# Jerrypiglet/monosdf

Measured on AMD Instinct MI355X. Metric: rays/sec fwd+bwd, 1024 rays x 98 samples, 8x256 SDF MLP, higher is better.
Workload: dtype f32; 1 GPU; configs[1]: 1024 rays x 98 samples per GPU, ImplicitNetwork 8x256 + RenderingNetwork 289-256-256-3, error-bounded sampler, random-init weights (density beta 0.1), training step = fwd + loss + bwd + Adam, a different one of 8 ray batches every step; rays_per_gpu=1024, samples_per_ray=98, ray_batches=8, matrix_core=fp32

## Files before the change

include/monosdf_hip.h:

```cpp
#ifndef MONOSDF_HIP_H
#define MONOSDF_HIP_H

#include <stdint.h>
#include "monosdf_plan.h"

#ifdef __cplusplus
extern "C" {
#endif

#define MSDF_OK 0
#define MSDF_ERR_ARG 1
#define MSDF_ERR_LAUNCH 2
#define MSDF_ERR_UNSUPPORTED 3

#define MSDF_ABI_VERSION 8
int msdf_abi_version(void);

int msdf_hash_encode_forward(const float* inputs, const float* embeddings, const int* offsets, float* outputs,
                             uint32_t B, uint32_t D, uint32_t C, uint32_t L, float S, uint32_t H,
                             int calc_grad_inputs, float* dy_dx, void* stream);
int msdf_hash_encode_backward(const float* grad, const float* inputs, const float* embeddings, const int* offsets,
                              float* grad_embeddings, uint32_t B, uint32_t D, uint32_t C, uint32_t L, float S,
                              uint32_t H, int calc_grad_inputs, const float* dy_dx, float* grad_inputs,
                              void* stream);
int msdf_hash_encode_second_backward(const float* grad, const float* inputs, const float* embeddings,
                                     const int* offsets, uint32_t B, uint32_t D, uint32_t C, uint32_t L, float S,
                                     uint32_t H, int calc_grad_inputs, const float* dy_dx,
                                     const float* grad_grad_inputs, float* grad_grad, float* grad2_embeddings,
                                     void* stream);

int64_t msdf_hash_scatter_workspace_bytes(uint32_t B, uint32_t C, uint32_t L, uint64_t n_entries);
int msdf_hash_encode_backward_ws(const float* grad, const float* inputs, const float* embeddings, const int* offsets,
                                 float* grad_embeddings, uint32_t B, uint32_t D, uint32_t C, uint32_t L, float S,
                                 uint32_t H, int calc_grad_inputs, const float* dy_dx, float* grad_inputs,
                                 uint64_t n_entries, void* workspace, uint64_t workspace_bytes, void* stream);
int msdf_hash_encode_second_backward_ws(const float* grad, const float* inputs, const float* embeddings,
                                        const int* offsets, uint32_t B, uint32_t D, uint32_t C, uint32_t L, float S,
                                        uint32_t H, int calc_grad_inputs, const float* dy_dx,
                                        const float* grad_grad_inputs, float* grad_grad, float* grad2_embeddings,
                                        uint64_t n_entries, void* workspace, uint64_t workspace_bytes, void* stream);
int msdf_hash_encode_backward_fused(const float* grad_first, const float* grad_second, const float* inputs,
                                    const int* offsets, float* grad_embeddings, uint32_t B, uint32_t D, uint32_t C,
                                    uint32_t L, float S, uint32_t H, const float* grad_grad_inputs,
                                    uint64_t n_entries, void* workspace, uint64_t workspace_bytes, void* stream);
int msdf_hash_encode_backward_fused_out(const float* grad_first, const float* grad_second, const float* inputs,
                                        const int* offsets, float* grad_embeddings, uint32_t B, uint32_t D, uint32_t C,
                                        uint32_t L, float S, uint32_t H, const float* grad_grad_inputs,
                                        uint64_t n_entries, void* workspace, uint64_t workspace_bytes, void* stream);

int msdf_hash_node_forward(const float* x, double divide_factor, float* x01_out, const float* embeddings,
                           const int* offsets, float* feat, uint32_t pitch, uint32_t B, uint32_t C, uint32_t L,
                           float S, uint32_t H, float* dy_dx, void* stream);
int msdf_hash_node_input_gradient(const float* g, uint32_t pitch, const float* dy_dx, uint32_t B, uint32_t C,
                                  uint32_t L, float scale, float* inout, void* stream);
int msdf_hash_node_second_grad(const float* g_a, const float* g_b, uint32_t n_split, float scale, float* gg_out,
                               const float* dy_dx, float* grad_grad, uint32_t pitch, uint32_t B, uint32_t C,
                               uint32_t L, void* stream);
int msdf_hash_transpose(const float* src, float* dst, const float* src2, float* dst2, uint32_t L, uint32_t B,
                        uint32_t C, uint32_t pitch, int to_point_major, void* stream);
int msdf_hash_node_scatter(const float* grad_first, const float* grad_second, uint32_t pitch, const float* inputs,
                           const int* offsets, float* grad_embeddings, uint32_t B, uint32_t C, uint32_t L, float S,
                           uint32_t H, const float* grad_grad_inputs, uint64_t n_entries, void* workspace,
                           uint64_t workspace_bytes, void* stream);

int msdf_pack_weights(const msdf_plan_t* plan, const msdf_packrule_t* rules_dev, const int* maps_dev,
                      const float* flat_w, const float* flat_b, void* wpack, float* bpack, void* stream);

typedef struct {
  const float* v;
  const float* g;
  const float* b;
  int32_t rows, cols;
  int32_t w_off;
  int32_t b_off;
  int32_t row_off;
  int32_t has_g;
} msdf_wn_layer_t;
int msdf_weightnorm_forward(const msdf_wn_layer_t* layers_dev, const int* row_layer_dev, int total_rows,
                            float* flat_w, float* flat_b, float* norms, void* stream);
int msdf_weightnorm_backward(const msdf_wn_layer_t* layers_dev, const int* row_layer_dev, int total_rows,
                             const float* g_flat_w, const float* norms, float* dv_flat, float* dg_rows, void* stream);

int msdf_sdf_forward(const msdf_plan_t* plan, const void* wpack, const float* bpack, const float* x,
                     const float* aux, int P, float clamp_radius, float sphere_scale, float* sdf, void* stream);
int msdf_sdf_forward_if(const msdf_plan_t* plan, const void* wpack, const float* bpack, const float* x,
                        const float* aux, int P, float clamp_radius, float sphere_scale, float* sdf,
                        const uint32_t* run_flag, void* stream);
int msdf_sdf_forward_lm(const msdf_plan_t* plan, const void* wpack, const float* bpack, const float* x,
                        const float* aux, int aux_C, int aux_LC, int P, float clamp_radius, float sphere_scale,
                        float* sdf, const uint32_t* run_flag, void* stream);
int msdf_sdf_forward_save(const msdf_plan_t* plan, const void* wpack, const float* bpack, const float* x,
                          const float* aux, int aux_C, int aux_LC, int P, float clamp_radius, float sphere_scale,
                          float* sdf, const uint32_t* run_flag, float* H, int P_pad, const int32_t* col_slot,
                          int n_cols, int n_slots, uint32_t* h_saved, void* stream);

typedef struct {
  const void* wpack;
  const float* bpack;
  const float* x;
  const float* aux;
  int32_t P, P_pad;
  int32_t n_clamp;
  int32_t n_feat;
  float clamp_radius, sphere_scale;
  float* sdf;
  float* feat;
  float* nrm;
  float* r_aux;
  unsigned char* clamped;
  float* H;
  float* PM;
  float* IN0;
  int32_t save;
  int32_t aux_C;
  int32_t aux_LC;
  float aux_dx_scale;
  const float* dy_dx;
  const int32_t* row_map;
  const uint32_t* smp_flags;
  const uint32_t* h_saved;
  int32_t n_reuse;
  int32_t stage_pad;
  const float* h_stage;
  int32_t wg_first;
} msdf_fg_args_t;
int msdf_sdf_fwd_grad(const msdf_plan_t* plan, const msdf_fg_args_t* args, void* stream);

typedef struct {
  const void* wpack;
  const float* bpack;
  const float* x;
  int32_t P, P_pad;
  int32_t n_feat;
  int32_t n_split;
  const float* g_sdf;
  const float* g_feat;
  const float* g_nrm;
  const float* g_raux;
  const unsigned char* clamped;
  const float* H;
  const float* PM;
  float* QB;
  float* T;
  float* AB;
  float* GSDF;
  float* QLAST;
  float* g_aux;
  const float* g_sdf_b;
  const float* g_nrm_b;
  int32_t aux_C, aux_LC;
  const float* dy_dx;
  float* gg_out;
  float aux_dx_scale;
  int32_t pad_;
  const int32_t* row_map;
} msdf_bw_args_t;
int msdf_sdf_backward(const msdf_plan_t* plan, const msdf_bw_args_t* args, void* stream);

typedef struct {
  const void* wpack;
  const float* bpack;
  const float* x;
  const float* dirs;
  const float* nrm;
  const float* feat;
  const float* code;
  int32_t P, P_pad;
  int32_t spr;
  int32_t save;
  float* rgb;
  float* H;
  float* MISC;
} msdf_color_fwd_args_t;
int msdf_color_forward(const msdf_plan_t* plan, const msdf_color_fwd_args_t* args, void* stream);

typedef struct {
  const void* wpack;
  const float* bpack;
  const float* rgb;
  const float* g_rgb;
  int32_t P, P_pad;
  const float* H;
  float* AB;
  float* g_feat;
  float* g_misc;
  float* g_nrm;
} msdf_color_bwd_args_t;
int msdf_color_backward(const msdf_plan_t* plan, const msdf_color_bwd_args_t* args, void* stream);

int msdf_wgrad(const msdf_wgrad_item_t* items_dev, const int32_t* wg_map_dev, int n_wgs, float* partials,
               int P_pad, int precision , const float* base0, const float* base1 , void* stream);
int msdf_reduce(const msdf_reduce_rule_t* rules_dev, int n_rules, const int* maps_dev, const float* partials,
                float* dst, void* stream);

typedef struct {
  const float* z;
  const float* sdf;
  const float* rgb;
  const float* nrm;
  const float* beta;
  const float* depth_scale;
  int32_t N, S;
  int32_t white_bkgd;
  float bg0, bg1, bg2;
  float* weights;
  float* rgb_values;
  float* depth_values;
  float* normal_map;
  float* wsum;
  const float* pose;
  int32_t pose_stride;
  int32_t depth_scale_stride;
  float* depth_vals;
} msdf_composite_args_t;
int msdf_composite_forward(const msdf_composite_args_t* args, void* stream);

typedef struct {
  const float* z;
  const float* sdf;
  const float* rgb;
  const float* nrm;
  const float* beta;
  const float* depth_scale;
  const float* weights;
  const float* wsum;
  const float* depth_values;
  const float* g_rgb_values;
  const float* g_depth;
  const float* g_normal;
  const float* g_weights;
  int32_t N, S;
  int32_t white_bkgd;
  float bg0, bg1, bg2;
  float* g_sdf;
  float* g_rgb;
  float* g_nrm;
  float* g_beta_part;
  const float* pose;
  int32_t pose_stride;
  int32_t depth_scale_stride;
} msdf_composite_bwd_args_t;
int msdf_composite_backward(const msdf_composite_bwd_args_t* args, void* stream);

int msdf_beta_eff(const float* beta_raw, float beta_min, float* out, void* stream);
int msdf_beta_grad(const float* beta_raw, const float* g_part, int n, float* g_raw, void* stream);

typedef struct {
  const float* rgb;
  const float* nrm;
  const float* depth;
  const float* g1;
  const float* g2;
  int32_t N, M;
  float w_normal, w_depth, w_eik, w_smooth;
  float* g_rgb; float* g_nrm; float* g_depth; float* g_g1; float* g_g2;
  float* partial;
} msdf_probe_loss_args_t;
int msdf_probe_loss(const msdf_probe_loss_args_t* args, void* stream);

typedef struct {
  const float* rgb;
  const float* depth;
  const float* normal;
  const float* sdf;
  const float* grad_theta;
  const float* grad_nei;
  const float* rgb_gt;
  const float* depth_gt;
  const float* normal_gt;
  const float* mask_gt;
  int32_t N, S, E;
  int32_t gamma;
  int32_t scale_invariant;
  float w_eik, w_smooth, w_depth, w_nl1, w_ncos;
  float* mask;
  float* out;
  float* g_rgb; float* g_depth; float* g_normal; float* g_theta; float* g_nei;
} msdf_monosdf_loss_args_t;
int msdf_monosdf_loss(const msdf_monosdf_loss_args_t* args, void* stream);

typedef struct {
  const float* ray_o;
  const float* ray_d;
  int32_t N;
  int32_t M;
  int32_t m_max;
  int32_t n_eval, n_final, n_extra;
  int32_t round_idx, max_rounds;
  int32_t training;
  int32_t beta_iters;
  float near, far, bound;
  float eps, add_tiny;
  float lemma;
  const float* beta0;
  float* z;
  float* sdf;
  float* new_z;
  const float* new_sdf;
  int32_t* new_pos;
  float* pts;
  float* beta;
  uint32_t* flags;
  const float* jitter;
  const float* u_final;
  float* final_z;
  const int64_t* extra_idx;
  const int64_t* eik_idx;
  float* z_out;
  float* z_eik;
  float* pts_out;
  const float* eik_uniform;
  const float* nei_rand;
  float* far_out;
  int32_t* rounds_out;
  float* dbg_dstar;
  float* dbg_err0;
  float* dbg_cdf;
  const float* eik_u;
  int32_t eik_unit;
  int32_t pad_;
  int32_t* row_map;
  uint32_t* h_saved;
} msdf_sampler_args_t;
int msdf_sampler_init(const msdf_sampler_args_t* args, void* stream);
int msdf_sampler_beta(const msdf_sampler_args_t* args, void* stream);
int msdf_sampler_resample(const msdf_sampler_args_t* args, void* stream);
int msdf_sampler_finish(const msdf_sampler_args_t* args, void* stream);

int msdf_sampler_error_bound(const float* z, const float* sdf, const float* dstar, const float* beta,
                             int beta_stride, int N, int M, float* out, void* stream);

int msdf_laplace_density(const float* sdf, const float* beta, int beta_stride, int64_t n, int cols, float* out,
                         void* stream);
int msdf_laplace_density_backward(const float* sdf, const float* beta, int beta_stride, int64_t n, int cols,
                                  const float* g, float* g_sdf, float* g_beta_elem, void* stream);

int msdf_camera_rays(const float* uv, const float* pose, const float* intrinsics, int n, float* ray_dirs,
                     float* ray_dirs_cam, float* cam_loc, void* stream);

int msdf_pixel_rays(const int64_t* ray_idx, int n, const int32_t* frame_list, int n_frames, const float* pose_all,
                    const float* intrinsics_all, int width, int hw, float* ray_dirs, float* ray_dirs_cam,
                    float* cam_loc, float* ray_pose, int32_t* frame_pos, const float* const* gt_src,
                    float* const* gt_dst, const int32_t* gt_channels, int n_gt, void* stream);

int64_t msdf_mc_workspace_bytes(int nx, int ny, int nz);
int msdf_mc_count(const float* vol, int nx, int ny, int nz, float level, void* workspace, int64_t* totals,
                  void* stream);
int msdf_mc_emit(const float* vol, int nx, int ny, int nz, float level, float sx, float sy, float sz,
                 const void* workspace, float* verts, float* normals, int32_t* faces, void* stream);

int msdf_nn_split_count(int64_t n_ref, int64_t n_query, int n_splits);
int64_t msdf_nn_workspace_bytes(int64_t n_ref, int64_t n_query, int n_splits);
int msdf_nn_search(const float* ref, int64_t n_ref, const float* query, int64_t n_query, int n_splits,
                   void* workspace, float* dist, int32_t* idx, void* stream);
int msdf_voxel_keys(const float* points, int64_t n, const float* min_bound, float voxel_size, int64_t* keys,
                    void* stream);
int msdf_voxel_mean(const float* points, const int64_t* order, const int64_t* seg_start, int64_t n, int64_t m,
                    float* out, void* stream);

int msdf_raster_depth(const float* verts, int64_t n_verts, const int32_t* faces, int64_t n_faces, const float* w2c,
                      int n_views, float fx, float fy, float cx, float cy, int height, int width, float znear,
                      float zfar, float pixel_center, float* depth, void* stream);
int msdf_tsdf_integrate(const float* depth, const float* w2c, int n_views, float fx, float fy, float cx, float cy,
                        int height, int width, float ox, float oy, float oz, int i0, int j0, int k0, int nx, int ny,
                        int nz, float voxel_length, float sdf_trunc, float depth_trunc, int resume, float* tsdf,
                        float* weight, void* stream);
int msdf_tsdf_face_keep(const float* verts, int64_t n_verts, const int32_t* faces, int64_t n_faces,
                        const float* weight, int nx, int ny, int nz, uint8_t* keep, void* stream);
int msdf_cull_vertices(const float* verts, int64_t n_verts, const float* w2c, int n_views, float fx, float fy, float cx,
                       float cy, int height, int width, uint8_t* seen, void* stream);

int64_t msdf_dtu_dilate_workspace_bytes(int n_views, int height, int width);
int msdf_dtu_dilate(const uint8_t* masks, int n_views, int height, int width, int radius, void* workspace,
                    uint8_t* out, void* stream);
int msdf_dtu_mask_vertices(const float* verts, int64_t n_verts, const float* proj, int n_views,
                           const uint8_t* dilated, int height, int width, uint8_t* keep, void* stream);
int msdf_dtu_lattice_count(const float* verts, int64_t n_verts, const int32_t* faces, int64_t n_faces,
                           double density, int64_t* counts, void* stream);
int msdf_dtu_lattice_emit(const float* verts, int64_t n_verts, const int32_t* faces, int64_t n_faces, double density,
                          const int64_t* offsets, int64_t n_points, float* out, void* stream);
// ... 13 lines not shown
```

monosdf_amd/_lib.py:

```python
import ctypes as C
import os

_HERE = os.path.dirname(os.path.abspath(__file__))
LIB_PATH = os.environ.get('MONOSDF_HIP_LIB') or os.path.join(_HERE, 'libmonosdf_hip.so')

MAX_LAYERS = 10
MAX_TILES = 17


class Layer(C.Structure):
    _fields_ = [(n, C.c_int32) for n in
                ('kt', 'ot', 'wf_off', 'wb_off', 'bias_off', 'skip_tile', 'hpre', 'qpre', 'abpre',
                 'ktp', 'otp', 'pad_')]


class Plan(C.Structure):
    _fields_ = [(n, C.c_int32) for n in
                ('n_layers', 'e_tiles', 'aux_tiles', 'n_freqs', 'sdf_slot', 'feat_tiles', 'hsum',
                 'qsum', 'absum', 'wsdf_off', 'mode', 'out_act', 'precision', 'out_rows')] + [('layer', Layer * MAX_LAYERS)]


class PackRule(C.Structure):
    _fields_ = [('w_off', C.c_int32), ('b_off', C.c_int32), ('rows', C.c_int32), ('cols', C.c_int32),
                ('rowmap_off', C.c_int32), ('colmap_off', C.c_int32), ('scale', C.c_float),
                ('pad_', C.c_int32)]


class WgradItem(C.Structure):
    _fields_ = [('x', C.c_int64), ('y', C.c_int64), ('v', C.c_int64),
                ('part_off', C.c_int64), ('colsum_off', C.c_int64), ('vrow_off', C.c_int64),
                ('x_ld', C.c_int32), ('y_ld', C.c_int32), ('wx', C.c_int32), ('wy', C.c_int32),
                ('n_splits', C.c_int32), ('bufs', C.c_int32)]


class ReduceRule(C.Structure):
    _fields_ = [('part_off', C.c_int64), ('dst_off', C.c_int64), ('n_blocks', C.c_int32),
                ('wx', C.c_int32), ('wy', C.c_int32), ('rowmap_off', C.c_int32),
                ('colmap_off', C.c_int32), ('dst_ld', C.c_int32), ('fixed_row', C.c_int32),
                ('scale', C.c_float)]


_P = C.c_void_p


class FgArgs(C.Structure):
    _fields_ = [('wpack', _P), ('bpack', _P), ('x', _P), ('aux', _P),
                ('P', C.c_int32), ('P_pad', C.c_int32), ('n_clamp', C.c_int32), ('n_feat', C.c_int32),
                ('clamp_radius', C.c_float), ('sphere_scale', C.c_float),
                ('sdf', _P), ('feat', _P), ('nrm', _P), ('r_aux', _P), ('clamped', _P),
                ('H', _P), ('PM', _P), ('IN0', _P), ('save', C.c_int32), ('aux_C', C.c_int32), ('aux_LC', C.c_int32),
                ('aux_dx_scale', C.c_float), ('dy_dx', _P),
                ('row_map', _P), ('smp_flags', _P), ('h_saved', _P), ('n_reuse', C.c_int32), ('stage_pad', C.c_int32), ('h_stage', _P),
                ('wg_first', C.c_int32)]


class BwArgs(C.Structure):
    _fields_ = [('wpack', _P), ('bpack', _P), ('x', _P),
                ('P', C.c_int32), ('P_pad', C.c_int32), ('n_feat', C.c_int32), ('n_split', C.c_int32),
                ('g_sdf', _P), ('g_feat', _P), ('g_nrm', _P), ('g_raux', _P), ('clamped', _P),
                ('H', _P), ('PM', _P), ('QB', _P), ('T', _P), ('AB', _P), ('GSDF', _P), ('QLAST', _P),
                ('g_aux', _P), ('g_sdf_b', _P), ('g_nrm_b', _P), ('aux_C', C.c_int32), ('aux_LC', C.c_int32),
                ('dy_dx', _P), ('gg_out', _P), ('aux_dx_scale', C.c_float), ('pad_', C.c_int32),
                ('row_map', _P)]


class ColorFwdArgs(C.Structure):
    _fields_ = [('wpack', _P), ('bpack', _P), ('x', _P), ('dirs', _P), ('nrm', _P), ('feat', _P),
                ('code', _P), ('P', C.c_int32), ('P_pad', C.c_int32), ('spr', C.c_int32),
                ('save', C.c_int32), ('rgb', _P), ('H', _P), ('MISC', _P)]


class ColorBwdArgs(C.Structure):
    _fields_ = [('wpack', _P), ('bpack', _P), ('rgb', _P), ('g_rgb', _P),
                ('P', C.c_int32), ('P_pad', C.c_int32), ('H', _P), ('AB', _P), ('g_feat', _P),
                ('g_misc', _P), ('g_nrm', _P)]


class CompositeArgs(C.Structure):
    _fields_ = [('z', _P), ('sdf', _P), ('rgb', _P), ('nrm', _P), ('beta', _P), ('depth_scale', _P),
                ('N', C.c_int32), ('S', C.c_int32), ('white_bkgd', C.c_int32),
                ('bg0', C.c_float), ('bg1', C.c_float), ('bg2', C.c_float),
                ('weights', _P), ('rgb_values', _P), ('depth_values', _P), ('normal_map', _P),
                ('wsum', _P), ('pose', _P), ('pose_stride', C.c_int32), ('depth_scale_stride', C.c_int32),
                ('depth_vals', _P)]


class CompositeBwdArgs(C.Structure):
    _fields_ = [('z', _P), ('sdf', _P), ('rgb', _P), ('nrm', _P), ('beta', _P), ('depth_scale', _P),
                ('weights', _P), ('wsum', _P), ('depth_values', _P), ('g_rgb_values', _P),
                ('g_depth', _P), ('g_normal', _P), ('g_weights', _P),
                ('N', C.c_int32), ('S', C.c_int32), ('white_bkgd', C.c_int32),
                ('bg0', C.c_float), ('bg1', C.c_float), ('bg2', C.c_float),
                ('g_sdf', _P), ('g_rgb', _P), ('g_nrm', _P), ('g_beta_part', _P),
                ('pose', _P), ('pose_stride', C.c_int32), ('depth_scale_stride', C.c_int32)]


class WnLayer(C.Structure):
    _fields_ = [('v', _P), ('g', _P), ('b', _P), ('rows', C.c_int32), ('cols', C.c_int32),
                ('w_off', C.c_int32), ('b_off', C.c_int32), ('row_off', C.c_int32), ('has_g', C.c_int32)]


class ProbeLossArgs(C.Structure):
    _fields_ = [('rgb', _P), ('nrm', _P), ('depth', _P), ('g1', _P), ('g2', _P), ('N', C.c_int32), ('M', C.c_int32),
                ('w_normal', C.c_float), ('w_depth', C.c_float), ('w_eik', C.c_float), ('w_smooth', C.c_float),
                ('g_rgb', _P), ('g_nrm', _P), ('g_depth', _P), ('g_g1', _P), ('g_g2', _P), ('partial', _P)]


class MonoSdfLossArgs(C.Structure):
    _fields_ = [(n, _P) for n in ('rgb', 'depth', 'normal', 'sdf', 'grad_theta', 'grad_nei', 'rgb_gt', 'depth_gt',
                                  'normal_gt', 'mask_gt')] + \
               [(n, C.c_int32) for n in ('N', 'S', 'E', 'gamma', 'scale_invariant')] + \
               [(n, C.c_float) for n in ('w_eik', 'w_smooth', 'w_depth', 'w_nl1', 'w_ncos')] + \
               [(n, _P) for n in ('mask', 'out', 'g_rgb', 'g_depth', 'g_normal', 'g_theta', 'g_nei')]


class SamplerArgs(C.Structure):
    _fields_ = [('ray_o', _P), ('ray_d', _P), ('N', C.c_int32), ('M', C.c_int32), ('m_max', C.c_int32),
                ('n_eval', C.c_int32), ('n_final', C.c_int32), ('n_extra', C.c_int32),
                ('round_idx', C.c_int32), ('max_rounds', C.c_int32), ('training', C.c_int32),
                ('beta_iters', C.c_int32), ('near', C.c_float), ('far', C.c_float), ('bound', C.c_float),
                ('eps', C.c_float), ('add_tiny', C.c_float), ('lemma', C.c_float),
                ('beta0', _P), ('z', _P), ('sdf', _P), ('new_z', _P), ('new_sdf', _P), ('new_pos', _P),
                ('pts', _P), ('beta', _P), ('flags', _P), ('jitter', _P), ('u_final', _P), ('final_z', _P),
                ('extra_idx', _P), ('eik_idx', _P), ('z_out', _P), ('z_eik', _P), ('pts_out', _P),
                ('eik_uniform', _P), ('nei_rand', _P), ('far_out', _P), ('rounds_out', _P),
                ('dbg_dstar', _P), ('dbg_err0', _P), ('dbg_cdf', _P), ('eik_u', _P), ('eik_unit', C.c_int32),
                ('pad_', C.c_int32), ('row_map', _P), ('h_saved', _P)]


_ERR = {1: 'invalid argument', 2: 'kernel launch failed', 3: 'unsupported configuration'}

_SIGNATURES = {
    'msdf_abi_version': [],
    'msdf_hash_encode_forward': [_P, _P, _P, _P, C.c_uint32, C.c_uint32, C.c_uint32, C.c_uint32,
                                 C.c_float, C.c_uint32, C.c_int, _P, _P],
    'msdf_hash_encode_backward': [_P, _P, _P, _P, _P, C.c_uint32, C.c_uint32, C.c_uint32, C.c_uint32,
                                  C.c_float, C.c_uint32, C.c_int, _P, _P, _P],
    'msdf_hash_encode_second_backward': [_P, _P, _P, _P, C.c_uint32, C.c_uint32, C.c_uint32,
                                         C.c_uint32, C.c_float, C.c_uint32, C.c_int, _P, _P, _P, _P, _P],
    'msdf_hash_scatter_workspace_bytes': [C.c_uint32, C.c_uint32, C.c_uint32, C.c_uint64],
    'msdf_hash_encode_backward_ws': [_P, _P, _P, _P, _P, C.c_uint32, C.c_uint32, C.c_uint32, C.c_uint32,
                                     C.c_float, C.c_uint32, C.c_int, _P, _P, C.c_uint64, _P, C.c_uint64, _P],
    'msdf_hash_encode_second_backward_ws': [_P, _P, _P, _P, C.c_uint32, C.c_uint32, C.c_uint32, C.c_uint32,
                                            C.c_float, C.c_uint32, C.c_int, _P, _P, _P, _P, C.c_uint64, _P,
                                            C.c_uint64, _P],
    'msdf_hash_encode_backward_fused': [_P, _P, _P, _P, _P, C.c_uint32, C.c_uint32, C.c_uint32, C.c_uint32,
                                        C.c_float, C.c_uint32, _P, C.c_uint64, _P, C.c_uint64, _P],
    'msdf_hash_encode_backward_fused_out': [_P, _P, _P, _P, _P, C.c_uint32, C.c_uint32, C.c_uint32, C.c_uint32,
                                            C.c_float, C.c_uint32, _P, C.c_uint64, _P, C.c_uint64, _P],
    'msdf_hash_node_forward': [_P, C.c_double, _P, _P, _P, _P, C.c_uint32, C.c_uint32, C.c_uint32, C.c_uint32,
                               C.c_float, C.c_uint32, _P, _P],
    'msdf_hash_node_input_gradient': [_P, C.c_uint32, _P, C.c_uint32, C.c_uint32, C.c_uint32, C.c_float, _P, _P],
    'msdf_hash_node_second_grad': [_P, _P, C.c_uint32, C.c_float, _P, _P, _P, C.c_uint32, C.c_uint32, C.c_uint32,
                                   C.c_uint32, _P],
    'msdf_hash_transpose': [_P, _P, _P, _P, C.c_uint32, C.c_uint32, C.c_uint32, C.c_uint32, C.c_int, _P],
    'msdf_hash_node_scatter': [_P, _P, C.c_uint32, _P, _P, _P, C.c_uint32, C.c_uint32, C.c_uint32, C.c_float,
                               C.c_uint32, _P, C.c_uint64, _P, C.c_uint64, _P],
    'msdf_weightnorm_forward': [_P, _P, C.c_int, _P, _P, _P, _P],
    'msdf_weightnorm_backward': [_P, _P, C.c_int, _P, _P, _P, _P, _P],
    'msdf_pack_weights': [C.POINTER(Plan), _P, _P, _P, _P, _P, _P, _P],
    'msdf_sdf_forward': [C.POINTER(Plan), _P, _P, _P, _P, C.c_int, C.c_float, C.c_float, _P, _P],
    'msdf_sdf_forward_if': [C.POINTER(Plan), _P, _P, _P, _P, C.c_int, C.c_float, C.c_float, _P, _P, _P],
    'msdf_sdf_forward_lm': [C.POINTER(Plan), _P, _P, _P, _P, C.c_int, C.c_int, C.c_int, C.c_float, C.c_float, _P, _P, _P],
    'msdf_sdf_forward_save': [C.POINTER(Plan), _P, _P, _P, _P, C.c_int, C.c_int, C.c_int, C.c_float, C.c_float, _P, _P,
                              _P, C.c_int, _P, C.c_int, C.c_int, _P, _P],
    'msdf_sdf_fwd_grad': [C.POINTER(Plan), C.POINTER(FgArgs), _P],
    'msdf_sdf_backward': [C.POINTER(Plan), C.POINTER(BwArgs), _P],
    'msdf_color_forward': [C.POINTER(Plan), C.POINTER(ColorFwdArgs), _P],
    'msdf_color_backward': [C.POINTER(Plan), C.POINTER(ColorBwdArgs), _P],
    'msdf_wgrad': [_P, _P, C.c_int, _P, C.c_int, C.c_int, _P, _P, _P],
    'msdf_camera_rays': [_P, _P, _P, C.c_int, _P, _P, _P, _P],
    'msdf_pixel_rays': [_P, C.c_int, _P, C.c_int, _P, _P, C.c_int, C.c_int, _P, _P, _P, _P, _P, _P, _P, _P, C.c_int, _P],
    'msdf_monosdf_loss': [C.POINTER(MonoSdfLossArgs), _P],
    'msdf_reduce': [_P, C.c_int, _P, _P, _P, _P],
    'msdf_composite_forward': [C.POINTER(CompositeArgs), _P],
    'msdf_composite_backward': [C.POINTER(CompositeBwdArgs), _P],
    'msdf_beta_eff': [_P, C.c_float, _P, _P],
    'msdf_beta_grad': [_P, _P, C.c_int, _P, _P],
    'msdf_probe_loss': [C.POINTER(ProbeLossArgs), _P],
    'msdf_sampler_init': [C.POINTER(SamplerArgs), _P],
    'msdf_sampler_beta': [C.POINTER(SamplerArgs), _P],
    'msdf_sampler_resample': [C.POINTER(SamplerArgs), _P],
    'msdf_sampler_finish': [C.POINTER(SamplerArgs), _P],
    'msdf_sampler_error_bound': [_P, _P, _P, _P, C.c_int, C.c_int, C.c_int, _P, _P],
    'msdf_laplace_density': [_P, _P, C.c_int, C.c_int64, C.c_int, _P, _P],
    'msdf_laplace_density_backward': [_P, _P, C.c_int, C.c_int64, C.c_int, _P, _P, _P, _P],
    'msdf_mc_workspace_bytes': [C.c_int, C.c_int, C.c_int],
    'msdf_mc_count': [_P, C.c_int, C.c_int, C.c_int, C.c_float, _P, _P, _P],
    'msdf_mc_emit': [_P, C.c_int, C.c_int, C.c_int, C.c_float, C.c_float, C.c_float, C.c_float, _P, _P, _P, _P, _P],
    'msdf_nn_split_count': [C.c_int64, C.c_int64, C.c_int],
    'msdf_nn_workspace_bytes': [C.c_int64, C.c_int64, C.c_int],
    'msdf_nn_search': [_P, C.c_int64, _P, C.c_int64, C.c_int, _P, _P, _P, _P],
    'msdf_voxel_keys': [_P, C.c_int64, _P, C.c_float, _P, _P],
    'msdf_voxel_mean': [_P, _P, _P, C.c_int64, C.c_int64, _P, _P],
    'msdf_raster_depth': [_P, C.c_int64, _P, C.c_int64, _P, C.c_int, C.c_float, C.c_float, C.c_float, C.c_float,
                          C.c_int, C.c_int, C.c_float, C.c_float, C.c_float, _P, _P],
    'msdf_tsdf_integrate': [_P, _P, C.c_int, C.c_float, C.c_float, C.c_float, C.c_float, C.c_int, C.c_int,
                            C.c_float, C.c_float, C.c_float, C.c_int, C.c_int, C.c_int, C.c_int, C.c_int, C.c_int,
                            C.c_float, C.c_float, C.c_float, C.c_int, _P, _P, _P],
    'msdf_tsdf_face_keep': [_P, C.c_int64, _P, C.c_int64, _P, C.c_int, C.c_int, C.c_int, _P, _P],
    'msdf_cull_vertices': [_P, C.c_int64, _P, C.c_int, C.c_float, C.c_float, C.c_float, C.c_float, C.c_int, C.c_int,
                           _P, _P],
    'msdf_dtu_dilate_workspace_bytes': [C.c_int, C.c_int, C.c_int],
    'msdf_dtu_dilate': [_P, C.c_int, C.c_int, C.c_int, C.c_int, _P, _P, _P],
    'msdf_dtu_mask_vertices': [_P, C.c_int64, _P, C.c_int, _P, C.c_int, C.c_int, _P, _P],
    'msdf_dtu_lattice_count': [_P, C.c_int64, _P, C.c_int64, C.c_double, _P, _P],
    'msdf_dtu_lattice_emit': [_P, C.c_int64, _P, C.c_int64, C.c_double, _P, C.c_int64, _P, _P],
    'msdf_dtu_thin_workspace_bytes': [C.c_int64],
    'msdf_dtu_thin_keys': [_P, C.c_int64, C.c_double, C.c_double, C.c_double, C.c_double, _P, _P],
    'msdf_dtu_thin_prepare': [_P, _P, _P, _P, C.c_int64, _P, _P],
    'msdf_dtu_thin_round': [_P, C.c_int64, C.c_double, _P, _P],
    'msdf_dtu_thin_finish': [_P, _P, C.c_int64, _P, _P],
}

ABI_VERSION = 8

_lib = None


def load():
    global _lib
    if _lib is not None:
        return _lib
    if not os.path.exists(LIB_PATH):
        raise RuntimeError(
            'monosdf_amd: %s not found -- build it with `python __graft_entry__.py` or '
            '`make -C monosdf_amd/csrc` (there is no non-HIP fallback)' % LIB_PATH)
    lib = C.CDLL(LIB_PATH)
    for name, argtypes in _SIGNATURES.items():
        fn = getattr(lib, name)
        fn.argtypes = argtypes
        fn.restype = C.c_int64 if name.endswith('_bytes') else C.c_int
    if lib.msdf_abi_version() != ABI_VERSION:
        raise RuntimeError('monosdf_amd: ABI version mismatch, rebuild the library')
    _lib = lib
    return lib
# ... 36 lines not shown
```

monosdf_amd/csrc/composite.hip:

```cpp
#include "common.h"

#define CMP_MAX_PER_LANE 4

__device__ __forceinline__ float wave_incl_scan(float v) {
  const int lane = lane_id();
#pragma unroll
  for (int d = 1; d < 64; d <<= 1) {
    const float o = __shfl_up(v, d, 64);
    if (lane >= d) v += o;
  }
  return v;
}

__device__ __forceinline__ float wave_excl_scan(const float v, float& total) {
  float prev = __shfl_up(v, 1, 64);
  if (lane_id() == 0) prev = 0.f;
  const float ex = wave_incl_scan(prev);
  total = __shfl(ex, 63, 64) + __shfl(v, 63, 64);
  return ex;
}

__device__ __forceinline__ float wave_sum(float v) {
#pragma unroll
  for (int d = 32; d >= 1; d >>= 1) v += __shfl_xor(v, d, 64);
// ... 38 lines not shown
      w = alpha * trans;
      a.weights[(size_t)ray * S + i] = w;
      if (a.depth_vals != nullptr) a.depth_vals[(size_t)ray * S + i] = z[i] * dscale;
      const float* c = a.rgb + ((size_t)ray * S + i) * 3;
      const float* n = a.nrm + ((size_t)ray * S + i) * 3;
      r0 += w * c[0]; r1 += w * c[1]; r2 += w * c[2];
      wz += w * z[i];
      ws += w;
      const float nn = sqrtf(n[0] * n[0] + n[1] * n[1] + n[2] * n[2]) + 1e-6f;
      m0 += w * (n[0] / nn); m1 += w * (n[1] / nn); m2 += w * (n[2] / nn);
    }
    carry += chunk_total;
  }
  r0 = wave_sum(r0); r1 = wave_sum(r1); r2 = wave_sum(r2);
  wz = wave_sum(wz); ws = wave_sum(ws);
  m0 = wave_sum(m0); m1 = wave_sum(m1); m2 = wave_sum(m2);
  if (lane == 0) {
    if (a.white_bkgd) {
      r0 += (1.f - ws) * a.bg0; r1 += (1.f - ws) * a.bg1; r2 += (1.f - ws) * a.bg2;
    }
    a.rgb_values[(size_t)ray * 3 + 0] = r0;
    a.rgb_values[(size_t)ray * 3 + 1] = r1;
    a.rgb_values[(size_t)ray * 3 + 2] = r2;
    a.depth_values[ray] = dscale * (wz / (ws + 1e-8f));
    if (a.pose != nullptr) {
      const float* R = a.pose + (size_t)ray * a.pose_stride;
      const float c0 = R[0] * m0 + R[4] * m1 + R[8] * m2;
      const float c1 = R[1] * m0 + R[5] * m1 + R[9] * m2;
      const float c2 = R[2] * m0 + R[6] * m1 + R[10] * m2;
      m0 = c0; m1 = c1; m2 = c2;
    }
    a.normal_map[(size_t)ray * 3 + 0] = m0;
    a.normal_map[(size_t)ray * 3 + 1] = m1;
    a.normal_map[(size_t)ray * 3 + 2] = m2;
    a.wsum[ray] = ws;
  }
}

typedef msdf_composite_bwd_args_t CompositeBwdArgs;

__device__ __forceinline__ float wave_excl_suffix(const float v, float& total) {
  const int lane = lane_id();
  float s = __shfl_down(v, 1, 64);
  if (lane == 63) s = 0.f;
#pragma unroll
  for (int d = 1; d < 64; d <<= 1) {
    const float o = __shfl_down(s, d, 64);
    if (lane + d < 64) s += o;
  }
  total = __shfl(s, 0, 64) + __shfl(v, 0, 64);
  return s;
}

__global__ void __launch_bounds__(256)
msdf_composite_backward_k(const CompositeBwdArgs a) {
  const int ray = blockIdx.x * 4 + (threadIdx.x >> 6);
  if (ray >= a.N) return;
  const int lane = lane_id();
  const int S = a.S;
  const float beta = a.beta[0];
  const float* z = a.z + (size_t)ray * S;
  const float* sd = a.sdf + (size_t)ray * S;
  const float ws = a.wsum[ray];
  const float ds = a.depth_scale[(size_t)ray * (a.depth_scale_stride > 0 ? a.depth_scale_stride : 1)];
  float gR0 = 0.f, gR1 = 0.f, gR2 = 0.f, gD = 0.f, gM0 = 0.f, gM1 = 0.f, gM2 = 0.f;
  if (a.g_rgb_values) {
    gR0 = a.g_rgb_values[(size_t)ray * 3 + 0];
    gR1 = a.g_rgb_values[(size_t)ray * 3 + 1];
    gR2 = a.g_rgb_values[(size_t)ray * 3 + 2];
  }
  if (a.g_depth) gD = a.g_depth[ray];
  if (a.g_normal) {
    gM0 = a.g_normal[(size_t)ray * 3 + 0];
    gM1 = a.g_normal[(size_t)ray * 3 + 1];
    gM2 = a.g_normal[(size_t)ray * 3 + 2];
    if (a.pose != nullptr) {
      const float* R = a.pose + (size_t)ray * a.pose_stride;
      const float w0 = R[0] * gM0 + R[1] * gM1 + R[2] * gM2;
      const float w1 = R[4] * gM0 + R[5] * gM1 + R[6] * gM2;
      const float w2 = R[8] * gM0 + R[9] * gM1 + R[10] * gM2;
      gM0 = w0; gM1 = w1; gM2 = w2;
    }
  }
  const float inv = 1.0f / (ws + 1e-8f);
  const float wz_over = (ds != 0.f) ? a.depth_values[ray] / ds : 0.f;
  float bg_term = 0.f;
  if (a.white_bkgd) bg_term = -(gR0 * a.bg0 + gR1 * a.bg1 + gR2 * a.bg2);

  float fe_[CMP_MAX_PER_LANE], tr_[CMP_MAX_PER_LANE], wb_[CMP_MAX_PER_LANE], dist_[CMP_MAX_PER_LANE];
  float carry = 0.f;
  const int nchunk = (S + 63) >> 6;
#pragma unroll
  for (int ch = 0; ch < CMP_MAX_PER_LANE; ++ch) {
    fe_[ch] = tr_[ch] = wb_[ch] = dist_[ch] = 0.f;
    if (ch < nchunk) {
      const int i = ch * 64 + lane;
      const bool ok = i < S;
      float fe = 0.f, dist = 0.f;
      if (ok) {
        const float zi = z[i];
        dist = (i + 1 < S) ? (z[i + 1] - zi) : 1e10f;
        fe = dist * laplace_density(sd[i], beta);
      }
      float chunk_total;
      const float ex = wave_excl_scan(fe, chunk_total);
      if (ok) {
        const float excl = carry + ex;
        const float trans = expf(-excl);
        const float w = a.weights[(size_t)ray * S + i];
        const float* c = a.rgb + ((size_t)ray * S + i) * 3;
        const float* n = a.nrm + ((size_t)ray * S + i) * 3;
        const float nl = sqrtf(n[0] * n[0] + n[1] * n[1] + n[2] * n[2]);
        const float nn = nl + 1e-6f;
        const float gdot = gM0 * n[0] + gM1 * n[1] + gM2 * n[2];
        float wbar = gR0 * c[0] + gR1 * c[1] + gR2 * c[2] + gD * ds * (z[i] - wz_over) * inv + gdot / nn + bg_term;
        if (a.g_weights) wbar += a.g_weights[(size_t)ray * S + i];
        float* gc = a.g_rgb + ((size_t)ray * S + i) * 3;
        gc[0] = w * gR0; gc[1] = w * gR1; gc[2] = w * gR2;
        float* gn = a.g_nrm + ((size_t)ray * S + i) * 3;
        const float k = (nl > 0.f) ? gdot / (nl * nn * nn) : 0.f;
        gn[0] = w * (gM0 / nn - n[0] * k);
        gn[1] = w * (gM1 / nn - n[1] * k);
        gn[2] = w * (gM2 / nn - n[2] * k);
        fe_[ch] = fe; tr_[ch] = trans; wb_[ch] = wbar; dist_[ch] = dist;
      }
      carry += chunk_total;
    }
  }
  float after = 0.f;
  float gbeta = 0.f;
#pragma unroll
  for (int ch = CMP_MAX_PER_LANE - 1; ch >= 0; --ch) {
    if (ch < nchunk) {
      const int i = ch * 64 + lane;
      const bool ok = i < S;
      const float fe = fe_[ch], trans = tr_[ch], wbar = wb_[ch];
      const float efe = expf(-fe);
      const float alpha = 1.0f - efe;
      const float cbar = ok ? (-wbar * alpha * trans) : 0.f;
      float total;
      const float suffix = wave_excl_suffix(cbar, total);
      if (ok) {
        const float ebar = wbar * trans * efe + suffix + after;
        const float sbar = ebar * dist_[ch];
        const float s = sd[i];
        const float ex = expf(-fabsf(s) / beta);
        a.g_sdf[(size_t)ray * S + i] = sbar * (-0.5f / (beta * beta)) * ex;
        const float sigma = laplace_density(s, beta);
        gbeta += sbar * (-sigma / beta + 0.5f * s * ex / (beta * beta * beta));
      }
      after += total;
    }
  }
  gbeta = wave_sum(gbeta);
  if (lane == 0) a.g_beta_part[ray] = gbeta;
}

__global__ void msdf_beta_eff_k(const float* __restrict__ raw, const float beta_min, float* __restrict__ out) {
  if (threadIdx.x == 0) out[0] = fabsf(raw[0]) + beta_min;
}
__global__ void __launch_bounds__(64)
msdf_beta_grad_k(const float* __restrict__ raw, const float* __restrict__ part, const int n, float* __restrict__ g_raw) {
  float s = 0.f;
  for (int i = threadIdx.x; i < n; i += 64) s += part[i];
  s = wave_sum(s);
  const float r = raw[0];
  if (threadIdx.x == 0) g_raw[0] = ((r > 0.f) ? 1.f : (r < 0.f) ? -1.f : 0.f) * s;
}
extern "C" int msdf_beta_eff(const float* beta_raw, float beta_min, float* out, void* stream) {
  if (beta_raw == nullptr || out == nullptr) return MSDF_ERR_ARG;
  msdf_beta_eff_k<<<1, 64, 0, (hipStream_t)stream>>>(beta_raw, beta_min, out);
  return msdf_check_launch();
}
extern "C" int msdf_beta_grad(const float* beta_raw, const float* g_part, int n, float* g_raw, void* stream) {
  if (beta_raw == nullptr || g_raw == nullptr || n < 0 || (n > 0 && g_part == nullptr)) return MSDF_ERR_ARG;
  msdf_beta_grad_k<<<1, 64, 0, (hipStream_t)stream>>>(beta_raw, g_part, n, g_raw);
  return msdf_check_launch();
}

extern "C" int msdf_composite_forward(const msdf_composite_args_t* a, void* stream) {
  if (a == nullptr || a->N < 0 || a->S < 1 || a->S > 64 * CMP_MAX_PER_LANE) return MSDF_ERR_ARG;
  if (a->N == 0) return MSDF_OK;
  msdf_composite_forward_k<<<(a->N + 3) / 4, 256, 0, (hipStream_t)stream>>>(*a);
  return msdf_check_launch();
}

extern "C" int msdf_composite_backward(const msdf_composite_bwd_args_t* a, void* stream) {
  if (a == nullptr || a->N < 0 || a->S < 1 || a->S > 64 * CMP_MAX_PER_LANE) return MSDF_ERR_ARG;
  if (a->N == 0) return MSDF_OK;
  msdf_composite_backward_k<<<(a->N + 3) / 4, 256, 0, (hipStream_t)stream>>>(*a);
  return msdf_check_launch();
}
```

monosdf_amd/csrc/sampler.hip:

```cpp
#include "common.h"

#define SMP_WAVES 4

__device__ __forceinline__ float smp_scan_incl(float v) {
  const int lane = lane_id();
#pragma unroll
  for (int d = 1; d < 64; d <<= 1) {
    const float o = __shfl_up(v, d, 64);
    if (lane >= d) v += o;
  }
  return v;
}
__device__ __forceinline__ float smp_sum(float v) {
#pragma unroll
  for (int d = 32; d >= 1; d >>= 1) v += __shfl_xor(v, d, 64);
  return v;
}
__device__ __forceinline__ float smp_max(float v) {
#pragma unroll
  for (int d = 32; d >= 1; d >>= 1) v = fmaxf(v, __shfl_xor(v, d, 64));
  return v;
}
__device__ __forceinline__ float smp_density(const float s, const float beta) {
  const float e = expm1f(-fabsf(s) / beta);
  const float sg = (s > 0.f) ? 1.f : (s < 0.f) ? -1.f : 0.f;
  return (1.0f / beta) * (0.5f + 0.5f * sg * e);
}
__device__ __forceinline__ float smp_linspace01(const int j, const int n) {
  const float step = 1.0f / (float)(n - 1);
  return (j < n / 2) ? step * (float)j : 1.0f - step * (float)(n - 1 - j);
}

typedef msdf_sampler_args_t SmpArgs;

__global__ void __launch_bounds__(64 * SMP_WAVES) smp_init_k(const SmpArgs a) {
  const int ray = blockIdx.x * SMP_WAVES + (threadIdx.x >> 6);
  if (ray >= a.N) return;
  const int lane = lane_id();
  if (ray == 0 && a.flags != nullptr)
    for (int i = lane; i < 2 * a.max_rounds; i += 64) a.flags[i] = 0u;
  if (ray == 0 && lane == 0 && a.h_saved != nullptr) a.h_saved[0] = 0u;
  const int n = a.n_eval;
  const float o0 = a.ray_o[ray * 3 + 0], o1 = a.ray_o[ray * 3 + 1], o2 = a.ray_o[ray * 3 + 2];
  const float d0 = a.ray_d[ray * 3 + 0], d1 = a.ray_d[ray * 3 + 1], d2 = a.ray_d[ray * 3 + 2];
  const float ta0 = (-a.bound - o0) / (d0 + 1e-15f), tb0 = (a.bound - o0) / (d0 + 1e-15f);
  const float ta1 = (-a.bound - o1) / (d1 + 1e-15f), tb1 = (a.bound - o1) / (d1 + 1e-15f);
  const float ta2 = (-a.bound - o2) / (d2 + 1e-15f), tb2 = (a.bound - o2) / (d2 + 1e-15f);
  float near_c = fmaxf(fmaxf(fminf(ta0, tb0), fminf(ta1, tb1)), fminf(ta2, tb2));
  float far_c = fminf(fminf(fmaxf(ta0, tb0), fmaxf(ta1, tb1)), fmaxf(ta2, tb2));
  if (far_c < near_c) far_c = 1e9f;
  const float far = (a.bound > 0.f) ? fminf(far_c, a.far) : a.far;
  const float near = a.near;
  float sumsq = 0.f;
  float* zrow = a.z + (size_t)ray * a.m_max;
  auto zu = [&](int k) { const float t = smp_linspace01(k, n); return near * (1.f - t) + far * t; };
  auto zfin = [&](int k) {
    float z = zu(k);
    if (a.jitter != nullptr) {
      const float zl = (k > 0) ? 0.5f * (zu(k) + zu(k - 1)) : zu(0);
      const float zh = (k + 1 < n) ? 0.5f * (zu(k + 1) + zu(k)) : zu(n - 1);
      z = zl + (zh - zl) * a.jitter[(size_t)ray * n + k];
    }
    return z;
  };
  for (int j = lane; j < n; j += 64) {
    const float z = zfin(j);
    zrow[j] = z;
    a.new_z[(size_t)ray * n + j] = z;
    a.new_pos[(size_t)ray * n + j] = j;
    float* p = a.pts + ((size_t)ray * n + j) * 3;
    p[0] = o0 + z * d0; p[1] = o1 + z * d1; p[2] = o2 + z * d2;
    if (j + 1 < n) {
      const float dz = zfin(j + 1) - z;
      sumsq += dz * dz;
    }
  }
  sumsq = smp_sum(sumsq);
  if (lane == 0) {
    a.beta[ray] = sqrtf(a.lemma * sumsq);
    if (a.far_out != nullptr) a.far_out[ray] = far;
  }
}

struct SmpLds {
  float* z; float* sdf; float* dist; float* dstar; float* tmp; float* snew;
};
__device__ __forceinline__ SmpLds smp_lds(float* base, const int m_max, const int n_eval) {
  const int w = threadIdx.x >> 6;
  const int per = 5 * (m_max + 1) + n_eval;
  float* p = base + (size_t)w * per;
  SmpLds l;
  l.z = p; l.sdf = p + (m_max + 1); l.dist = p + 2 * (m_max + 1); l.dstar = p + 3 * (m_max + 1);
  l.tmp = p + 4 * (m_max + 1); l.snew = p + 5 * (m_max + 1);
  return l;
}
__device__ __forceinline__ void smp_sync() {
  __builtin_amdgcn_fence(__ATOMIC_RELEASE, "workgroup");
  __builtin_amdgcn_wave_barrier();
  __builtin_amdgcn_fence(__ATOMIC_ACQUIRE, "workgroup");
}

__device__ __forceinline__ bool smp_round_active(const SmpArgs& a) {
  return a.round_idx == 0 || a.flags[2 * (a.round_idx - 1) + 1] != 0u;
}

__device__ __forceinline__ void smp_load_ray(const SmpArgs& a, const SmpLds& l, const int ray, const bool scatter) {
  const int lane = lane_id();
  const int M = a.M;
  const float* zrow = a.z + (size_t)ray * a.m_max;
  float* srow = a.sdf + (size_t)ray * a.m_max;
  for (int i = lane; i < M; i += 64) { l.z[i] = zrow[i]; l.sdf[i] = srow[i]; }
  smp_sync();
  if (scatter) {
    for (int j = lane; j < a.n_eval; j += 64)
      l.sdf[a.new_pos[(size_t)ray * a.n_eval + j]] = a.new_sdf[(size_t)ray * a.n_eval + j];
    smp_sync();
    for (int i = lane; i < M; i += 64) srow[i] = l.sdf[i];
  }
  for (int i = lane; i + 1 < M; i += 64) {
    const float aa = l.z[i + 1] - l.z[i];
    const float b = fabsf(l.sdf[i]), c = fabsf(l.sdf[i + 1]);
    const bool first = aa * aa + b * b <= c * c;
    const bool second = aa * aa + c * c <= b * b;
    float ds = 0.f;
    if (first) ds = b;
    if (second) ds = c;
    if (!first && !second && (b + c - aa > 0.f)) {
      const float s = (aa + b + c) / 2.0f;
      const float area = s * (s - aa) * (s - b) * (s - c);
      ds = (2.0f * sqrtf(area)) / aa;
    }
    const float s0 = l.sdf[i], s1 = l.sdf[i + 1];
    const float sg0 = (s0 > 0.f) ? 1.f : (s0 < 0.f) ? -1.f : 0.f;
    const float sg1 = (s1 > 0.f) ? 1.f : (s1 < 0.f) ? -1.f : 0.f;
    l.dist[i] = aa;
    const float dsv = (sg0 * sg1 == 1.f) ? ds : 0.f;
    l.dstar[i] = dsv;
    if (scatter && a.dbg_dstar != nullptr) a.dbg_dstar[(size_t)ray * a.m_max + i] = dsv;
  }
  smp_sync();
}

__device__ __forceinline__ float smp_error_bound(const SmpLds& l, const int M, const float beta) {
  const int lane = lane_id();
  float carry_fe = 0.f, carry_err = 0.f, best = -1e30f;
  const float inv4b2 = 1.0f / (4.0f * beta * beta);
  for (int base = 0; base < M - 1; base += 64) {
    const int i = base + lane;
    const bool ok = i < M - 1;
    float fe = 0.f, er = 0.f;
    if (ok) {
      const float d = l.dist[i];
      fe = d * smp_density(l.sdf[i], beta);
      er = expf(-l.dstar[i] / beta) * (d * d) * inv4b2;
    }
    const float fe_incl = smp_scan_incl(fe);
    const float er_incl = smp_scan_incl(er);
    if (ok) {
      const float integral = carry_fe + fe_incl - fe;
      const float errint = carry_err + er_incl;
      const float bound = (fminf(expf(errint), 1.0e6f) - 1.0f) * expf(-integral);
      best = fmaxf(best, bound);
    }
    carry_fe += __shfl(fe_incl, 63, 64);
    carry_err += __shfl(er_incl, 63, 64);
  }
  return smp_max(best);
}

__global__ void __launch_bounds__(64 * SMP_WAVES) smp_beta_k(const SmpArgs a) {
  extern __shared__ float smp_lds_mem[];
  const int ray = blockIdx.x * SMP_WAVES + (threadIdx.x >> 6);
  if (ray >= a.N || !smp_round_active(a)) return;
  const SmpLds l = smp_lds(smp_lds_mem, a.m_max, a.n_eval);
  smp_load_ray(a, l, ray, true);
  const float beta0 = a.beta0[0];
  float beta = a.beta[ray];
  const float e0 = smp_error_bound(l, a.M, beta0);
  if (a.dbg_err0 != nullptr && lane_id() == 0) a.dbg_err0[ray] = e0;
  if (e0 <= a.eps) beta = beta0;
  float lo = beta0, hi = beta;
  const int iters = (e0 <= a.eps) ? 0 : a.beta_iters;
  for (int it = 0; it < iters; ++it) {
    const float mid = (lo + hi) / 2.0f;
    const float e = smp_error_bound(l, a.M, mid);
    if (e <= a.eps) hi = mid;
    if (e > a.eps) lo = mid;
  }
  if (lane_id() == 0) {
    a.beta[ray] = hi;
    atomicMax(a.flags + 2 * a.round_idx, __float_as_uint(hi));
  }
}

__global__ void __launch_bounds__(64 * SMP_WAVES) smp_resample_k(const SmpArgs a) {
  extern __shared__ float smp_lds_mem[];
  const int ray = blockIdx.x * SMP_WAVES + (threadIdx.x >> 6);
  if (ray >= a.N || !smp_round_active(a)) return;
  const int lane = lane_id();
  const int M = a.M;
  const SmpLds l = smp_lds(smp_lds_mem, a.m_max, a.n_eval);
  const float beta0 = a.beta0[0];
  const float maxbeta = __uint_as_float(a.flags[2 * a.round_idx]);
  const bool unconverged = maxbeta > beta0;
  const bool more = unconverged && (a.round_idx + 1 < a.max_rounds);
  if (ray == 0 && lane == 0) a.flags[2 * a.round_idx + 1] = more ? 1u : 0u;
  smp_load_ray(a, l, ray, false);
  const float beta = a.beta[ray];
  const float inv4b2 = 1.0f / (4.0f * beta * beta);

  float carry_fe = 0.f, carry_err = 0.f, psum = 0.f;
  for (int base = 0; base < M; base += 64) {
    const int i = base + lane;
    const bool ok = i < M;
    float fe = 0.f, er = 0.f;
    if (ok) {
      const float d = (i + 1 < M) ? l.dist[i] : 1e10f;
      fe = d * smp_density(l.sdf[i], beta);
      if (more && i + 1 < M) er = expf(-l.dstar[i] / beta) * (l.dist[i] * l.dist[i]) * inv4b2;
    }
    float fprev = __shfl_up(fe, 1, 64);
    if (lane == 0) fprev = 0.f;
    const float fe_excl = smp_scan_incl(fprev);
    const float fe_incl = fe_excl + fe;
    const float er_incl = smp_scan_incl(er);
    if (ok && i + 1 < M) {
      const float trans = expf(-(carry_fe + fe_excl));
      float p;
      if (more) p = (fminf(expf(carry_err + er_incl), 1.0e6f) - 1.0f) * trans + a.add_tiny;
      else p = (1.0f - expf(-fe)) * trans + 1e-5f;
      l.tmp[i] = p;
      psum += p;
    }
    carry_fe += __shfl(fe_incl, 63, 64);
    carry_err += __shfl(er_incl, 63, 64);
  }
  psum = smp_sum(psum);
  smp_sync();
  float carry = 0.f;
  for (int base = 0; base < M - 1; base += 64) {
    const int i = base + lane;
    const float p = (i < M - 1) ? l.tmp[i] / psum : 0.f;
    const float incl = smp_scan_incl(p);
    if (i < M - 1) l.dstar[i + 1] = carry + incl;
    carry += __shfl(incl, 63, 64);
  }
  if (lane == 0) l.dstar[0] = 0.f;
  smp_sync();
  const float* cdf = l.dstar;
  if (a.dbg_cdf != nullptr)
    for (int i = lane; i < M; i += 64) a.dbg_cdf[(size_t)ray * a.m_max + i] = cdf[i];

  const int n_new = more ? a.n_eval : a.n_final;
  for (int j = lane; j < n_new; j += 64) {
    float u;
    if (more || !a.training || a.u_final == nullptr) u = smp_linspace01(j, n_new);
    else u = a.u_final[(size_t)ray * a.n_final + j];
    int lo = 0, hi = M;
    while (lo < hi) {
      const int mid = (lo + hi) >> 1;
      if (cdf[mid] <= u) lo = mid + 1; else hi = mid;
    }
    const int below = max(lo - 1, 0), above = min(lo, M - 1);
    float denom = cdf[above] - cdf[below];
    if (denom < 1e-5f) denom = 1.0f;
    const float t = (u - cdf[below]) / denom;
    const float s = l.z[below] + t * (l.z[above] - l.z[below]);
    l.snew[j] = s;
  }
  smp_sync();

  if (!more) {
    for (int j = lane; j < n_new; j += 64) a.final_z[(size_t)ray * a.n_final + j] = l.snew[j];
    return;
  }
  const float o0 = a.ray_o[ray * 3 + 0], o1 = a.ray_o[ray * 3 + 1], o2 = a.ray_o[ray * 3 + 2];
  const float d0 = a.ray_d[ray * 3 + 0], d1 = a.ray_d[ray * 3 + 1], d2 = a.ray_d[ray * 3 + 2];
  float* zrow = a.z + (size_t)ray * a.m_max;
  float* srow = a.sdf + (size_t)ray * a.m_max;
  for (int i = lane; i < M; i += 64) {
    const float zi = l.z[i];
    int cnt = 0;
    for (int k = 0; k < n_new; ++k) cnt += (l.snew[k] < zi) ? 1 : 0;
    zrow[i + cnt] = zi;
    srow[i + cnt] = l.sdf[i];
  }
  for (int j = lane; j < n_new; j += 64) {
    const float sj = l.snew[j];
    int cnt = 0;
    for (int i = 0; i < M; ++i) cnt += (l.z[i] <= sj) ? 1 : 0;
    for (int k = 0; k < n_new; ++k) cnt += (l.snew[k] < sj || (l.snew[k] == sj && k < j)) ? 1 : 0;
    zrow[cnt] = sj;
    a.new_z[(size_t)ray * a.n_eval + j] = sj;
    a.new_pos[(size_t)ray * a.n_eval + j] = cnt;
    float* p = a.pts + ((size_t)ray * a.n_eval + j) * 3;
    p[0] = o0 + sj * d0; p[1] = o1 + sj * d1; p[2] = o2 + sj * d2;
  }
}

__global__ void __launch_bounds__(64 * SMP_WAVES) smp_finish_k(const SmpArgs a) {
  extern __shared__ float smp_lds_mem[];
  const int ray = blockIdx.x * SMP_WAVES + (threadIdx.x >> 6);
  if (ray >= a.N) return;
  const int lane = lane_id();
  const int S = a.n_final + a.n_extra + 2;
  float* v = smp_lds_mem + (size_t)(threadIdx.x >> 6) * 2 * S;
  float* sorted = v + S;
  const float* zrow = a.z + (size_t)ray * a.m_max;
  int rounds = 1;
  while (rounds < a.max_rounds && a.flags[2 * (rounds - 1) + 1] != 0u) ++rounds;
  const int64_t* extra = a.extra_idx + (size_t)(rounds - 1) * a.n_extra;
  if (a.rounds_out != nullptr && ray == 0 && lane == 0) a.rounds_out[0] = rounds;
  for (int j = lane; j < S; j += 64) {
    float x;
    if (j < a.n_final) x = a.final_z[(size_t)ray * a.n_final + j];
    else if (j == a.n_final) x = a.near;
    else if (j == a.n_final + 1) x = a.far;
    else x = zrow[min((int)extra[j - a.n_final - 2], rounds * a.n_eval - 1)];
    if (x != x) x = INFINITY;
    v[j] = x;
  }
  smp_sync();
  const float o0 = a.ray_o[ray * 3 + 0], o1 = a.ray_o[ray * 3 + 1], o2 = a.ray_o[ray * 3 + 2];
  const float d0 = a.ray_d[ray * 3 + 0], d1 = a.ray_d[ray * 3 + 1], d2 = a.ray_d[ray * 3 + 2];
  for (int j = lane; j < S; j += 64) {
    const float x = v[j];
    int r = 0, rn = 0;
    for (int k = 0; k < S; ++k) {
      const int before = (v[k] < x || (v[k] == x && k < j)) ? 1 : 0;
      r += before;
      rn += (k < a.n_final + 2) ? before : 0;
    }
    sorted[r] = x;
    a.z_out[(size_t)ray * S + r] = x;
    if (a.row_map != nullptr) {
      const int e = j - a.n_final - 2;
      const int er = (e >= 0) ? ray * a.n_extra + e : a.N * a.n_extra + ray * (S - a.n_extra) + rn;
      a.row_map[er] = ray * S + r;
    }
    if (a.pts_out != nullptr) {
      float* p = a.pts_out + ((size_t)ray * S + r) * 3;
      p[0] = o0 + x * d0; p[1] = o1 + x * d1; p[2] = o2 + x * d2;
    }
  }
  smp_sync();
  if (lane == 0) {
    const int idx = (a.eik_idx != nullptr) ? (int)a.eik_idx[ray]
                    : (a.eik_u != nullptr) ? min(S - 1, (int)(a.eik_u[ray] * (float)S)) : 0;
    const float ze = sorted[idx];
    if (a.z_eik != nullptr) a.z_eik[ray] = ze;
    if (a.pts_out != nullptr && a.eik_uniform != nullptr) {
      float* e = a.pts_out + (size_t)a.N * S * 3;
      if (a.row_map != nullptr)
        for (int i = 0; i < 4; ++i) a.row_map[a.N * S + i * a.N + ray] = a.N * S + i * a.N + ray;
      const float od[3] = {o0 + ze * d0, o1 + ze * d1, o2 + ze * d2};
#pragma unroll
      for (int c = 0; c < 3; ++c) {
        float u = a.eik_uniform[(size_t)ray * 3 + c];
        if (a.eik_unit) u = (2.0f * u - 1.0f) * a.bound;
        e[((size_t)ray) * 3 + c] = u;
        e[((size_t)a.N + ray) * 3 + c] = od[c];
        e[((size_t)2 * a.N + ray) * 3 + c] = u + (a.nei_rand[(size_t)ray * 3 + c] - 0.5f) * 0.01f;
        e[((size_t)3 * a.N + ray) * 3 + c] = od[c] + (a.nei_rand[((size_t)a.N + ray) * 3 + c] - 0.5f) * 0.01f;
      }
    }
  }
}

__global__ void __launch_bounds__(64 * SMP_WAVES) smp_error_bound_k(const float* __restrict__ z,
                                                                     const float* __restrict__ sdf,
                                                                     const float* __restrict__ dstar,
                                                                     const float* __restrict__ beta, const int beta_stride,
                                                                     const int N, const int M, float* __restrict__ out) {
  extern __shared__ float smp_lds_mem[];
  const int ray = blockIdx.x * SMP_WAVES + (threadIdx.x >> 6);
  if (ray >= N) return;
  const int lane = lane_id();
  const SmpLds l = smp_lds(smp_lds_mem, M, 0);
  for (int i = lane; i < M; i += 64) { l.z[i] = z[(size_t)ray * M + i]; l.sdf[i] = sdf[(size_t)ray * M + i]; }
  smp_sync();
  for (int i = lane; i + 1 < M; i += 64) {
    l.dist[i] = l.z[i + 1] - l.z[i];
    l.dstar[i] = dstar[(size_t)ray * (M - 1) + i];
  }
  smp_sync();
  const float e = smp_error_bound(l, M, beta[(size_t)ray * beta_stride]);
  if (lane == 0) out[ray] = e;
}

__global__ void __launch_bounds__(256) laplace_density_k(const float* __restrict__ sdf, const float* __restrict__ beta,
                                                         const int beta_stride, const int64_t n, const int cols,
                                                         float* __restrict__ out) {
  for (int64_t i = (int64_t)blockIdx.x * 256 + threadIdx.x; i < n; i += (int64_t)gridDim.x * 256)
    out[i] = smp_density(sdf[i], beta[(i / cols) * beta_stride]);
}
__global__ void __launch_bounds__(256) laplace_density_bwd_k(const float* __restrict__ sdf, const float* __restrict__ beta,
                                                             const int beta_stride, const int64_t n, const int cols,
                                                             const float* __restrict__ g, float* __restrict__ g_sdf,
                                                             float* __restrict__ g_beta_elem) {
  for (int64_t i = (int64_t)blockIdx.x * 256 + threadIdx.x; i < n; i += (int64_t)gridDim.x * 256) {
    const float s = sdf[i], b = beta[(i / cols) * beta_stride], gi = g[i];
    const float a = fabsf(s);
    const float ex = expf(-a / b);
    const float sg = (s > 0.f) ? 1.f : (s < 0.f) ? -1.f : 0.f;
    g_sdf[i] = gi * (1.0f / b) * 0.5f * sg * ex * (-sg / b);
    const float em1 = expm1f(-a / b);
    g_beta_elem[i] = gi * (-(1.0f / (b * b)) * (0.5f + 0.5f * sg * em1) + (1.0f / b) * 0.5f * sg * ex * (a / (b * b)));
  }
}

static int smp_check(const msdf_sampler_args_t* a) {
  if (a == nullptr || a->N < 0 || a->n_eval < 2 || a->m_max < a->n_eval) return MSDF_ERR_ARG;
  return MSDF_OK;
}
static size_t smp_lds_bytes(const msdf_sampler_args_t* a) {
  return (size_t)SMP_WAVES * (5 * (a->m_max + 1) + a->n_eval) * sizeof(float);
}
template <typename K>
static int smp_launch(K kernel, const msdf_sampler_args_t* a, size_t lds, void* stream) {
  if (a->N == 0) return MSDF_OK;
  if (lds > 160 * 1024) return MSDF_ERR_UNSUPPORTED;
  if (lds > 48 * 1024 &&
      hipFuncSetAttribute((const void*)kernel, hipFuncAttributeMaxDynamicSharedMemorySize, (int)lds) != hipSuccess)
    return MSDF_ERR_LAUNCH;
  kernel<<<(a->N + SMP_WAVES - 1) / SMP_WAVES, 64 * SMP_WAVES, lds, (hipStream_t)stream>>>(*a);
  return msdf_check_launch();
}

extern "C" int msdf_sampler_init(const msdf_sampler_args_t* a, void* stream) {
  if (smp_check(a)) return MSDF_ERR_ARG;
  return smp_launch(smp_init_k, a, 0, stream);
}
static int smp_round_check(const msdf_sampler_args_t* a) {
  return a->flags == nullptr || a->round_idx < 0 || a->round_idx >= a->max_rounds || a->M > a->m_max || a->M < 2;
}
extern "C" int msdf_sampler_beta(const msdf_sampler_args_t* a, void* stream) {
  if (smp_check(a) || smp_round_check(a)) return MSDF_ERR_ARG;
  return smp_launch(smp_beta_k, a, smp_lds_bytes(a), stream);
}
extern "C" int msdf_sampler_resample(const msdf_sampler_args_t* a, void* stream) {
  if (smp_check(a) || smp_round_check(a) || a->n_final > a->n_eval) return MSDF_ERR_ARG;
  return smp_launch(smp_resample_k, a, smp_lds_bytes(a), stream);
}
extern "C" int msdf_sampler_finish(const msdf_sampler_args_t* a, void* stream) {
  if (smp_check(a) || a->flags == nullptr || (a->extra_idx == nullptr && a->n_extra > 0) ||
      a->m_max < a->n_eval * a->max_rounds)
    return MSDF_ERR_ARG;
  const size_t lds = (size_t)SMP_WAVES * 2 * (a->n_final + a->n_extra + 2) * sizeof(float);
  return smp_launch(smp_finish_k, a, lds, stream);
}

extern "C" int msdf_sampler_error_bound(const float* z, const float* sdf, const float* dstar, const float* beta,
                                        int beta_stride, int N, int M, float* out, void* stream) {
  if (N < 0 || M < 2 || (beta_stride != 0 && beta_stride != 1)) return MSDF_ERR_ARG;
  if (N == 0) return MSDF_OK;
  const size_t lds = (size_t)SMP_WAVES * 5 * (M + 1) * sizeof(float);
  if (lds > 160 * 1024) return MSDF_ERR_UNSUPPORTED;
  if (lds > 48 * 1024 && hipFuncSetAttribute((const void*)smp_error_bound_k,
                                             hipFuncAttributeMaxDynamicSharedMemorySize, (int)lds) != hipSuccess)
    return MSDF_ERR_LAUNCH;
  smp_error_bound_k<<<(N + SMP_WAVES - 1) / SMP_WAVES, 64 * SMP_WAVES, lds, (hipStream_t)stream>>>(
      z, sdf, dstar, beta, beta_stride, N, M, out);
  return msdf_check_launch();
}

static int dens_grid(int64_t n) { return (int)((n + 255) / 256 < 2048 ? (n + 255) / 256 : 2048); }
extern "C" int msdf_laplace_density(const float* sdf, const float* beta, int beta_stride, int64_t n, int cols,
                                    float* out, void* stream) {
  if (n < 0 || cols < 1 || (beta_stride != 0 && beta_stride != 1)) return MSDF_ERR_ARG;
  if (n == 0) return MSDF_OK;
  laplace_density_k<<<dens_grid(n), 256, 0, (hipStream_t)stream>>>(sdf, beta, beta_stride, n, cols, out);
  return msdf_check_launch();
}
extern "C" int msdf_laplace_density_backward(const float* sdf, const float* beta, int beta_stride, int64_t n, int cols,
                                             const float* g, float* g_sdf, float* g_beta_elem, void* stream) {
  if (n < 0 || cols < 1 || (beta_stride != 0 && beta_stride != 1)) return MSDF_ERR_ARG;
  if (n == 0) return MSDF_OK;
  laplace_density_bwd_k<<<dens_grid(n), 256, 0, (hipStream_t)stream>>>(sdf, beta, beta_stride, n, cols, g, g_sdf,
                                                                     g_beta_elem);
  return msdf_check_launch();
}
```

monosdf_amd/csrc/sdf_kernels.h:

```cpp
#pragma once
#include "mlp_core.h"

struct PointCtx {
  int pt;
  int ptc;
  bool valid;
  int q;
  float x0, x1, x2;
};

template <class Core>
__device__ __forceinline__ int eval_wg(const int wg_first = 0) {
  int w = (int)blockIdx.x;
  if constexpr (Core::ROW_MAP) {
    if (wg_first > 0) {
      w += wg_first;
      if (w >= (int)gridDim.x) w -= (int)gridDim.x;
    }
  }
  return w;
}

template <class Core>
__device__ __forceinline__ PointCtx load_point(const float* __restrict__ x, const int P,
// ... 402 lines not shown
  if (nl >= 2) {
    const msdf_layer_t L = plan.layer[nl - 2];
    const float* Hl = REUSE ? a.h_stage + srow(L) : a.H + row(L);
    float* Pl = a.PM + row(L);
    const int otl = L.ot - 1;
    v4f hh[MT];
#pragma unroll
    for (int t = 0; t < MT; ++t) hh[t] = *(const v4f*)(Hl + 16 * (t < otl ? t : otl));
#pragma unroll
    for (int t = 0; t < MT; ++t) {
      if (t == 0 || t < L.ot) {
        if constexpr (REUSE) *(v4f*)(a.H + row(L) + 16 * t) = hh[t];
        scale_by_sigmoid(hh[t], acc[t]);
        if (a.save) *(v4f*)(Pl + 16 * t) = acc[t];
      }
    }
  }
  for (int l = nl - 2; l >= 0; --l) {
    const msdf_layer_t L = plan.layer[l];
#pragma unroll
    for (int t = 0; t < MT; ++t) in[t] = (t < L.ot) ? acc[t] : V4ZERO;
    zero_tiles(acc);
    const msdf_layer_t Lp = plan.layer[l > 0 ? l - 1 : 0];
    Core::gemm(L.otp, acc, in, L.kt, (const wvec*)a.wpack + L.wb_off, lds,
               GradSweepHooks<REUSE>(REUSE ? a.h_stage + srow(Lp) : a.H + row(Lp), a.H + row(Lp), a.PM + row(Lp),
                                     l > 0 ? Lp.ot : 0, a.save != 0));
    if (l == 0) take_input_grad(0);
    else if (L.skip_tile >= 0) take_input_grad(L.skip_tile);
  }
  if (Core::AUX_LEVEL_MAJOR && a.dy_dx != nullptr && plan.aux_tiles > 0) {
    float m0, m1, m2;
    aux_jacobian_transpose(a.dy_dx, av, plan.aux_tiles, r_aux, c.ptc, c.q, m0, m1, m2);
    n0 = __fadd_rn(n0, __fmul_rn(sum_over_quarters(m0), a.aux_dx_scale));
    n1 = __fadd_rn(n1, __fmul_rn(sum_over_quarters(m1), a.aux_dx_scale));
    n2 = __fadd_rn(n2, __fmul_rn(sum_over_quarters(m2), a.aux_dx_scale));
  }
  bool is_clamped = false;
  if (a.clamp_radius > 0.f && c.pt < a.n_clamp) {
    const float nx = sqrtf(c.x0 * c.x0 + c.x1 * c.x1 + c.x2 * c.x2);
    const float sph = a.sphere_scale * (a.clamp_radius - nx);
    if (sph < sdf) {
      is_clamped = true;
      sdf = sph;
      const float inv = -a.sphere_scale / nx;
      n0 = c.x0 * inv; n1 = c.x1 * inv; n2 = c.x2 * inv;
    }
  }
  if (c.valid) {
    if (c.q == 0) {
      a.sdf[c.pt] = sdf;
      a.nrm[(size_t)c.pt * 3 + 0] = n0;
      a.nrm[(size_t)c.pt * 3 + 1] = n1;
      a.nrm[(size_t)c.pt * 3 + 2] = n2;
      a.clamped[c.pt] = is_clamped ? 1 : 0;
    }
    if (a.r_aux != nullptr) {
#pragma unroll
      for (int t = 0; t < 2; ++t)
        if (t < plan.aux_tiles) {
          v4f v = r_aux[t];
          if (is_clamped) v = V4ZERO;
          aux_store_tile<Core::AUX_LEVEL_MAJOR>(a.r_aux, av, plan.aux_tiles, t, c.pt, c.q, v);
        }
    }
  }
}

typedef msdf_bw_args_t BwArgs;

template <bool LM>
__device__ __forceinline__ void load_rbar(v4f (&rbar)[5], const msdf_plan_t& plan, const BwArgs& a,
                                          const PointCtx& c, const bool live, const float gn0, const float gn1,
                                          const float gn2) {
  pe_jacobian(rbar, c.x0, c.x1, c.x2, plan.n_freqs, gn0, gn1, gn2);
  rbar[3] = rbar[4] = V4ZERO;
  if (LM && a.dy_dx != nullptr && live) {
    const AuxView av = {a.aux_C, a.aux_LC, a.P};
    const float g0 = __fmul_rn(gn0, a.aux_dx_scale), g1 = __fmul_rn(gn1, a.aux_dx_scale), g2 = __fmul_rn(gn2, a.aux_dx_scale);
#pragma unroll
    for (int t = 0; t < 2; ++t)
      if (t < plan.aux_tiles) rbar[3 + t] = aux_jacobian_tile(a.dy_dx, av, t, c.pt, c.q, g0, g1, g2);
  } else if (a.g_raux != nullptr && live) {
    const AuxView av = {a.aux_C, a.aux_LC, a.P};
#pragma unroll
    for (int t = 0; t < 2; ++t)
      if (t < plan.aux_tiles) rbar[3 + t] = aux_load_tile<LM>(a.g_raux, av, plan.aux_tiles, t, c.pt, c.q);
  }
}

template <class Core>
__device__ __forceinline__ void sdf_backward_body(const msdf_plan_t& plan, const BwArgs& a, void* lds) {
  typedef typename Core::wvec wvec;
  const PointCtx c = load_point<Core>(a.x, a.P, a.row_map);
  const int nl = plan.n_layers;
  const size_t Pp = (size_t)a.P_pad;
  const bool live = c.valid && !(a.clamped != nullptr && a.clamped[c.ptc]);
  float gs = 0.f, gn0 = 0.f, gn1 = 0.f, gn2 = 0.f;
  if (live) {
    const bool first = c.pt < a.n_split;
    const float* gsp = first ? a.g_sdf : a.g_sdf_b;
    const float* gnp = first ? a.g_nrm : a.g_nrm_b;
    const size_t j = first ? (size_t)c.pt : (size_t)(c.pt - a.n_split);
    if (gsp) gs = gsp[j];
    if (gnp) {
      gn0 = gnp[j * 3 + 0];
      gn1 = gnp[j * 3 + 1];
      gn2 = gnp[j * 3 + 2];
    }
  }
  if (c.q == 0) a.GSDF[c.pt] = gs;
  if (Core::AUX_LEVEL_MAJOR && a.gg_out != nullptr && c.valid && c.q == 0) {
    float r0 = 0.f, r1 = 0.f, r2 = 0.f;
    const bool first = c.pt < a.n_split;
    const float* gnp = first ? a.g_nrm : a.g_nrm_b;
    if (gnp != nullptr) {
      const size_t j = first ? (size_t)c.pt : (size_t)(c.pt - a.n_split);
      r0 = gnp[j * 3 + 0]; r1 = gnp[j * 3 + 1]; r2 = gnp[j * 3 + 2];
    }
    a.gg_out[(size_t)c.pt * 3 + 0] = __fmul_rn(r0, a.aux_dx_scale);
    a.gg_out[(size_t)c.pt * 3 + 1] = __fmul_rn(r1, a.aux_dx_scale);
    a.gg_out[(size_t)c.pt * 3 + 2] = __fmul_rn(r2, a.aux_dx_scale);
  }
  const int in0_tiles = plan.e_tiles + plan.aux_tiles;

  v4f in[MT], acc[MT];
  {
    v4f rbar[5];
    load_rbar<Core::AUX_LEVEL_MAJOR>(rbar, plan, a, c, live, gn0, gn1, gn2);
    place_tiles(in, 0, rbar, in0_tiles);
  }

  for (int l = 0; l < nl - 1; ++l) {
    const msdf_layer_t L = plan.layer[l];
    if (L.skip_tile >= 0) {
      v4f rbar[5];
      load_rbar<Core::AUX_LEVEL_MAJOR>(rbar, plan, a, c, live, gn0, gn1, gn2);
      place_tiles(in, L.skip_tile, rbar, in0_tiles);
    }
    float* Ql = lane_row(a.QB, L.qpre, Pp, c.pt, L.kt, c.q);
#pragma unroll
    for (int t = 0; t < MT; ++t)
      if (t < L.kt) *(v4f*)(Ql + 16 * t) = in[t];
    zero_tiles(acc);
    const float* Hl = lane_row(a.H, L.hpre, Pp, c.pt, L.ot, c.q);
    Core::gemm(L.ktp, acc, in, L.ot, (const wvec*)a.wpack + L.wf_off, lds, SweepUpHooks(Hl, L.ot));
#pragma unroll
    for (int t = 0; t < MT; ++t) in[t] = (t < L.ot) ? acc[t] : V4ZERO;
  }
  const msdf_layer_t LL = plan.layer[nl - 1];
  {
    float* Ql = lane_row(a.QLAST, 0, 0, c.pt, LL.kt, c.q);
#pragma unroll
    for (int t = 0; t < MT; ++t)
      if (t < LL.kt) *(v4f*)(Ql + 16 * t) = in[t];
  }

  const bool has_feat = (a.g_feat != nullptr) && c.valid && c.pt < a.n_feat;
  {
    float* ABl = lane_row(a.AB, LL.abpre, Pp, c.pt, LL.ot, c.q);
    const float* gf = a.g_feat + (size_t)(has_feat ? c.pt : 0) * (16 * plan.feat_tiles) + 4 * c.q;
    const int ftl = plan.feat_tiles - 1;
#pragma unroll
    for (int t = 0; t < MT; ++t) {
      v4f v = V4ZERO;
      if (a.g_feat != nullptr && ftl >= 0) v = *(const v4f*)(gf + 16 * (t < ftl ? t : ftl));
      if (!has_feat || t >= plan.feat_tiles) v = V4ZERO;
      if (t == plan.feat_tiles && c.q == 0) v.x = gs;
      in[t] = v;
    }
#pragma unroll
    for (int t = 0; t < MT; ++t)
// ... 36 lines not shown
```

monosdf_amd/csrc/sdf_mlp.hip:

```cpp
#include "mlp_launch.h"

__global__ void __launch_bounds__(256) msdf_pack_kernel(const msdf_plan_t plan,
                                                        const msdf_packrule_t* __restrict__ rules,
                                                        const int* __restrict__ maps,
                                                        const float* __restrict__ flat_w,
                                                        const float* __restrict__ flat_b,
                                                        v4f* __restrict__ wpack, float* __restrict__ bpack) {
  const int l = blockIdx.y;
  const int which = blockIdx.z;
  const msdf_layer_t L = plan.layer[l];
  const msdf_packrule_t R = rules[l];
  const int* rowmap = maps + R.rowmap_off;
  const int* colmap = maps + R.colmap_off;
  const float* W = flat_w + R.w_off;
  const int stride = gridDim.x * blockDim.x;
  const int t0 = blockIdx.x * blockDim.x + threadIdx.x;
  if (which < 2) {
    const int n_rt = which == 0 ? L.ot : L.kt;
    const int n_kt = which == 0 ? L.kt : L.ot;
    const int ktp = which == 0 ? L.ktp : L.otp;
    const int off = which == 0 ? L.wf_off : L.wb_off;
    const int total = ((n_rt + 1) & ~1) * ktp * 64;
    for (int i = t0; i < total; i += stride) {
      const int lane = i & 63;
      const int blk = i >> 6;
      const int kt = blk % ktp, rt = blk / ktp;
      const int rslot = 16 * rt + (lane & 15);
      v4f v;
#pragma unroll
      for (int r = 0; r < 4; ++r) {
        const int kslot = 16 * kt + 4 * (lane >> 4) + r;
        float w = 0.f;
        if (rt < n_rt && kt < n_kt) {
          const int row = which == 0 ? rowmap[rslot] : rowmap[kslot];
          const int col = which == 0 ? colmap[kslot] : colmap[rslot];
          if (row >= 0 && col >= 0) w = R.scale * W[(size_t)row * R.cols + col];
        }
        v[r] = w;
      }
      wpack[off + i] = v;
    }
  } else {
    pack_bias_rows(plan, l, R, rowmap, colmap, W, flat_b, bpack, t0, stride);
  }
}

__global__ void __launch_bounds__(CoreF32::THREADS, CoreF32::WGS_PER_CU)
msdf_sdf_forward_k(const msdf_plan_t plan, const v4f* __restrict__ wpack, const float* __restrict__ bpack,
                   const float* __restrict__ x, const float* __restrict__ aux, const AuxView av, const int P,
                   const float clamp_radius, const float sphere_scale, float* __restrict__ sdf_out,
                   const uint32_t* __restrict__ run_flag) {
  extern __shared__ v4f lds[];
  if (run_flag != nullptr && *run_flag == 0u) return;
  sdf_forward_body<CoreF32>(plan, wpack, bpack, x, aux, av, P, clamp_radius, sphere_scale, sdf_out, lds);
}

__global__ void __launch_bounds__(CoreF32::THREADS, CoreF32::WGS_PER_CU)
msdf_sdf_forward_save_k(const msdf_plan_t plan, const v4f* __restrict__ wpack, const float* __restrict__ bpack,
                        const float* __restrict__ x, const float* __restrict__ aux, const AuxView av, const int P,
                        const float clamp_radius, const float sphere_scale, float* __restrict__ sdf_out,
                        const uint32_t* __restrict__ run_flag, const HSaveArgs hs, uint32_t* __restrict__ h_saved) {
  extern __shared__ v4f lds[];
  if (run_flag != nullptr && *run_flag == 0u) return;
  if (blockIdx.x == 0 && threadIdx.x == 0) *h_saved = 1u;
  sdf_forward_body<CoreF32, true>(plan, wpack, bpack, x, aux, av, P, clamp_radius, sphere_scale, sdf_out, lds, hs);
}

__global__ void __launch_bounds__(CoreF32::THREADS, CoreF32::WGS_PER_CU)
msdf_sdf_fwd_grad_k(const msdf_plan_t plan, const FgArgs a) {
  extern __shared__ v4f lds[];
  if (sdf_fwd_grad_reuses<CoreF32>(plan, a)) sdf_fwd_grad_body<CoreF32, true>(plan, a, lds);
  else sdf_fwd_grad_body<CoreF32>(plan, a, lds);
}

__global__ void __launch_bounds__(CoreF32::THREADS, CoreF32::WGS_PER_CU)
msdf_sdf_backward_k(const msdf_plan_t plan, const BwArgs a) {
  extern __shared__ v4f lds[];
  sdf_backward_body<CoreF32>(plan, a, lds);
}

static auto pack_kernel(CoreF32) { return msdf_pack_kernel; }
static auto forward_kernel(CoreF32) { return msdf_sdf_forward_k; }
static auto fwd_grad_kernel(CoreF32) { return msdf_sdf_fwd_grad_k; }
static auto backward_kernel(CoreF32) { return msdf_sdf_backward_k; }
template <int NS> static auto pack_kernel(CoreB16N<NS>) { return msdf_pack_b16_kernel<NS>; }
template <int NS> static auto forward_kernel(CoreB16N<NS>) { return msdf_sdf_forward_b16_k<NS>; }
template <int NS> static auto fwd_grad_kernel(CoreB16N<NS>) { return msdf_sdf_fwd_grad_b16_k<NS>; }
template <int NS> static auto backward_kernel(CoreB16N<NS>) { return msdf_sdf_backward_b16_k<NS>; }

extern "C" int msdf_abi_version(void) { return MSDF_ABI_VERSION; }

extern "C" int msdf_pack_weights(const msdf_plan_t* plan, const msdf_packrule_t* rules_dev, const int* maps_dev,
                                 const float* flat_w, const float* flat_b, void* wpack, float* bpack,
                                 void* stream) {
  if (plan == nullptr || plan->n_layers < 1 || plan->n_layers > MSDF_MAX_LAYERS) return MSDF_ERR_ARG;
  return mlp_with_core(plan, [&](auto core) {
    typedef typename decltype(core)::wvec wvec;
    const dim3 grid(32, plan->n_layers, 3);
    pack_kernel(core)<<<grid, 256, 0, (hipStream_t)stream>>>(*plan, rules_dev, maps_dev, flat_w, flat_b, (wvec*)wpack,
                                                             bpack);
    return msdf_check_launch();
  });
}

static bool aux_layout_ok(const msdf_plan_t* plan, const int aux_C, const int aux_LC) {
  if (aux_C == 0) return true;
  return aux_C == 2 && aux_LC > 0 && (aux_LC % aux_C) == 0 &&
         aux_LC <= 16 * plan->aux_tiles;
}

static bool padded_ok(const int P, const int P_pad) { return P_pad >= P && (P_pad % CoreF32::PTS_PER_WG) == 0; }

extern "C" int msdf_sdf_forward_lm(const msdf_plan_t* plan, const void* wpack, const float* bpack, const float* x,
                                   const float* aux, int aux_C, int aux_LC, int P, float clamp_radius,
                                   float sphere_scale, float* sdf, const uint32_t* run_flag, void* stream) {
  if (plan == nullptr || P < 0) return MSDF_ERR_ARG;
  if (P == 0) return MSDF_OK;
  if (plan->aux_tiles > 0 && aux == nullptr) return MSDF_ERR_ARG;
  if (!aux_layout_ok(plan, aux_C, aux_LC)) return MSDF_ERR_ARG;
  return mlp_with_core(plan, [&](auto core) {
    typedef decltype(core) Core;
    if (!Core::AUX_LEVEL_MAJOR && aux_C != 0) return MSDF_ERR_UNSUPPORTED;
    const AuxView av = {aux_C, aux_LC, P};
    return mlp_launch<Core>(forward_kernel(core), (P + Core::PTS_PER_WG - 1) / Core::PTS_PER_WG, stream, *plan,
                            (const typename Core::wvec*)wpack, bpack, x, aux, av, P, clamp_radius, sphere_scale, sdf,
                            run_flag);
  });
}

extern "C" int msdf_sdf_forward_save(const msdf_plan_t* plan, const void* wpack, const float* bpack, const float* x,
                                     const float* aux, int aux_C, int aux_LC, int P, float clamp_radius,
                                     float sphere_scale, float* sdf, const uint32_t* run_flag, float* H, int P_pad,
                                     const int32_t* col_slot, int n_cols, int n_slots, uint32_t* h_saved,
                                     void* stream) {
  if (plan == nullptr || P < 0 || H == nullptr || col_slot == nullptr || h_saved == nullptr) return MSDF_ERR_ARG;
  if (plan->precision != MSDF_PRECISION_F32) return MSDF_ERR_UNSUPPORTED;
  if (n_cols < 1 || n_slots < 1 || n_slots > n_cols || (P % n_cols) != 0 || !padded_ok(0, P_pad) ||
      (int64_t)(P / n_cols) * n_slots > (int64_t)P_pad)
    return MSDF_ERR_ARG;
  if (P == 0) return MSDF_OK;
  if (plan->aux_tiles > 0 && aux == nullptr) return MSDF_ERR_ARG;
  if (!aux_layout_ok(plan, aux_C, aux_LC)) return MSDF_ERR_ARG;
  const AuxView av = {aux_C, aux_LC, P};
  const HSaveArgs hs = {H, P_pad, col_slot, n_cols, n_slots};
  return mlp_launch<CoreF32>(msdf_sdf_forward_save_k, (P + CoreF32::PTS_PER_WG - 1) / CoreF32::PTS_PER_WG, stream, *plan,
                             (const v4f*)wpack, bpack, x, aux, av, P, clamp_radius, sphere_scale, sdf, run_flag, hs,
                             h_saved);
}

extern "C" int msdf_sdf_forward_if(const msdf_plan_t* plan, const void* wpack, const float* bpack, const float* x,
                                   const float* aux, int P, float clamp_radius, float sphere_scale, float* sdf,
                                   const uint32_t* run_flag, void* stream) {
  return msdf_sdf_forward_lm(plan, wpack, bpack, x, aux, 0, 0, P, clamp_radius, sphere_scale, sdf, run_flag, stream);
}

extern "C" int msdf_sdf_forward(const msdf_plan_t* plan, const void* wpack, const float* bpack, const float* x,
                                const float* aux, int P, float clamp_radius, float sphere_scale, float* sdf,
                                void* stream) {
  return msdf_sdf_forward_if(plan, wpack, bpack, x, aux, P, clamp_radius, sphere_scale, sdf, nullptr, stream);
}

extern "C" int msdf_sdf_fwd_grad(const msdf_plan_t* plan, const msdf_fg_args_t* a, void* stream) {
  if (plan == nullptr || a == nullptr || a->P < 0) return MSDF_ERR_ARG;
  if (a->P == 0) return MSDF_OK;
  if (!padded_ok(a->P, a->P_pad)) return MSDF_ERR_ARG;
  if (plan->aux_tiles > 0 && a->aux == nullptr) return MSDF_ERR_ARG;
  if (!aux_layout_ok(plan, a->aux_C, a->aux_LC)) return MSDF_ERR_ARG;
  if (a->dy_dx != nullptr && (a->aux_C != 2 || a->r_aux == nullptr)) return MSDF_ERR_ARG;
  if (a->n_reuse < 0 || (a->n_reuse % CoreF32::PTS_PER_WG) != 0 || a->n_reuse > a->P) return MSDF_ERR_ARG;
  if (a->n_reuse > 0 && (a->row_map == nullptr || a->n_reuse > a->n_feat || a->h_stage == nullptr ||
                         a->stage_pad < a->n_reuse))
    return MSDF_ERR_ARG;
  if (a->wg_first < 0 || a->wg_first >= a->P_pad / CoreF32::PTS_PER_WG) return MSDF_ERR_ARG;
  return mlp_with_core(plan, [&](auto core) {
    typedef decltype(core) Core;
    if (!Core::AUX_LEVEL_MAJOR && (a->aux_C != 0 || a->dy_dx != nullptr)) return MSDF_ERR_UNSUPPORTED;
    if (!Core::ROW_MAP && a->wg_first != 0) return MSDF_ERR_UNSUPPORTED;
    return mlp_launch<Core>(fwd_grad_kernel(core), a->P_pad / Core::PTS_PER_WG, stream, *plan, *a);
  });
}

extern "C" int msdf_sdf_backward(const msdf_plan_t* plan, const msdf_bw_args_t* a, void* stream) {
  if (plan == nullptr || a == nullptr || a->P < 0) return MSDF_ERR_ARG;
  if (a->P == 0) return MSDF_OK;
  if (!padded_ok(a->P, a->P_pad)) return MSDF_ERR_ARG;
  if (!aux_layout_ok(plan, a->aux_C, a->aux_LC)) return MSDF_ERR_ARG;
  if (a->dy_dx != nullptr && a->aux_C != 2) return MSDF_ERR_ARG;
  return mlp_with_core(plan, [&](auto core) {
    typedef decltype(core) Core;
    if (!Core::AUX_LEVEL_MAJOR && (a->aux_C != 0 || a->dy_dx != nullptr)) return MSDF_ERR_UNSUPPORTED;
    return mlp_launch<Core>(backward_kernel(core), a->P_pad / Core::PTS_PER_WG, stream, *plan, *a);
  });
}
```

monosdf_amd/csrc/weightnorm.hip:

```cpp
#include "common.h"

__device__ __forceinline__ float wn_wave_sum(float v) {
#pragma unroll
  for (int d = 32; d >= 1; d >>= 1) v += __shfl_xor(v, d, 64);
  return v;
}

__global__ void __launch_bounds__(256)
msdf_weightnorm_forward_k(const msdf_wn_layer_t* __restrict__ layers, const int* __restrict__ row_layer,
                          const int total_rows, float* __restrict__ flat_w, float* __restrict__ flat_b,
                          float* __restrict__ norms) {
  const int row_g = blockIdx.x * 4 + (threadIdx.x >> 6);
  if (row_g >= total_rows) return;
  const int lane = lane_id();
  const msdf_wn_layer_t L = layers[row_layer[row_g]];
  const int r = row_g - L.row_off;
  const float* v = L.v + (size_t)r * L.cols;
  float* w = flat_w + L.w_off + (size_t)r * L.cols;
  float scale = 1.0f;
  if (L.has_g) {
    float ss = 0.f;
    for (int c = lane; c < L.cols; c += 64) ss += v[c] * v[c];
    const float n = sqrtf(wn_wave_sum(ss));
    scale = L.g[r] / n;
    if (lane == 0) norms[row_g] = n;
  }
  for (int c = lane; c < L.cols; c += 64) w[c] = v[c] * scale;
  if (lane == 0) flat_b[L.b_off + r] = L.b[r];
}

__global__ void __launch_bounds__(256)
msdf_weightnorm_backward_k(const msdf_wn_layer_t* __restrict__ layers, const int* __restrict__ row_layer,
                           const int total_rows, const float* __restrict__ g_flat_w,
                           const float* __restrict__ norms, float* __restrict__ dv_flat,
                           float* __restrict__ dg_rows) {
  const int row_g = blockIdx.x * 4 + (threadIdx.x >> 6);
  if (row_g >= total_rows) return;
  const int lane = lane_id();
  const msdf_wn_layer_t L = layers[row_layer[row_g]];
  const int r = row_g - L.row_off;
  const float* v = L.v + (size_t)r * L.cols;
  const float* dw = g_flat_w + L.w_off + (size_t)r * L.cols;
  float* dv = dv_flat + L.w_off + (size_t)r * L.cols;
  if (!L.has_g) {
    for (int c = lane; c < L.cols; c += 64) dv[c] = dw[c];
    if (lane == 0) dg_rows[row_g] = 0.f;
    return;
  }
  float dot = 0.f;
  for (int c = lane; c < L.cols; c += 64) dot += dw[c] * v[c];
  dot = wn_wave_sum(dot);
  const float n = norms[row_g];
  const float g = L.g[r];
  const float a = g / n, bq = g * dot / (n * n * n);
  for (int c = lane; c < L.cols; c += 64) dv[c] = a * dw[c] - bq * v[c];
  if (lane == 0) dg_rows[row_g] = dot / n;
}

extern "C" int msdf_weightnorm_forward(const msdf_wn_layer_t* layers_dev, const int* row_layer_dev, int total_rows,
                                       float* flat_w, float* flat_b, float* norms, void* stream) {
  if (total_rows < 0) return MSDF_ERR_ARG;
  if (total_rows == 0) return MSDF_OK;
  msdf_weightnorm_forward_k<<<(total_rows + 3) / 4, 256, 0, (hipStream_t)stream>>>(layers_dev, row_layer_dev, total_rows,
                                                                                    flat_w, flat_b, norms);
  return msdf_check_launch();
}

extern "C" int msdf_weightnorm_backward(const msdf_wn_layer_t* layers_dev, const int* row_layer_dev, int total_rows,
                                        const float* g_flat_w, const float* norms, float* dv_flat, float* dg_rows,
                                        void* stream) {
  if (total_rows < 0) return MSDF_ERR_ARG;
  if (total_rows == 0) return MSDF_OK;
  msdf_weightnorm_backward_k<<<(total_rows + 3) / 4, 256, 0, (hipStream_t)stream>>>(
      layers_dev, row_layer_dev, total_rows, g_flat_w, norms, dv_flat, dg_rows);
  return msdf_check_launch();
}
```

monosdf_amd/model/network.py:

```python
import math

import os

import numpy as np
import torch
import torch.nn as nn

from .. import ops, plan as planlib
from ..hashencoder.hashgrid import HashEncoder
from .density import LaplaceDensity
from .ray_sampler import ErrorBoundSampler


class WNLinear(nn.Module):

    def __init__(self, in_dim, out_dim, init_fn=None, weight_norm=True):
        super().__init__()
        lin = nn.Linear(in_dim, out_dim)
        if init_fn is not None:
            init_fn(lin)
        self.in_features, self.out_features = in_dim, out_dim
        self.has_weight_norm = weight_norm
        self.bias = nn.Parameter(lin.bias.data.clone())
        if weight_norm:
# ... 48 lines not shown
        wpack, bpack = fused.pack(flat_w, flat_b)
        return fused, flat_w, flat_b, wpack, bpack

    def share(self, device):
        object.__setattr__(self, '_shared', None)
        object.__setattr__(self, '_shared', self.packed(device))

    def unshare(self):
        object.__setattr__(self, '_shared', None)


def _geometric_init(l, num_layers, dims, skip_in, multires, bias, inside_outside, out_dim):
    def fn(lin):
        if l == num_layers - 2:
            if not inside_outside:
                torch.nn.init.normal_(lin.weight, mean=np.sqrt(np.pi) / np.sqrt(dims[l]), std=0.0001)
                torch.nn.init.constant_(lin.bias, -bias)
            else:
                torch.nn.init.normal_(lin.weight, mean=-np.sqrt(np.pi) / np.sqrt(dims[l]), std=0.0001)
                torch.nn.init.constant_(lin.bias, bias)
        elif multires > 0 and l == 0:
            torch.nn.init.constant_(lin.bias, 0.0)
            torch.nn.init.constant_(lin.weight[:, 3:], 0.0)
            torch.nn.init.normal_(lin.weight[:, :3], 0.0, np.sqrt(2) / np.sqrt(out_dim))
        elif multires > 0 and l in skip_in:
            torch.nn.init.constant_(lin.bias, 0.0)
            torch.nn.init.normal_(lin.weight, 0.0, np.sqrt(2) / np.sqrt(out_dim))
            torch.nn.init.constant_(lin.weight[:, -(dims[0] - 3):], 0.0)
        else:
            torch.nn.init.constant_(lin.bias, 0.0)
            torch.nn.init.normal_(lin.weight, 0.0, np.sqrt(2) / np.sqrt(out_dim))
    return fn


class _SdfBase(_FusedNet):

    supports_bf16x3 = True

    def _make_layers(self, dims, geometric_init, bias, skip_in, weight_norm, multires, inside_outside):
        self.num_layers = len(dims)
        self.skip_in = tuple(skip_in)
        self.dims = list(dims)
        for l in range(self.num_layers - 1):
            out_dim = dims[l + 1] - dims[0] if (l + 1) in self.skip_in else dims[l + 1]
            init = _geometric_init(l, self.num_layers, dims, self.skip_in, multires, bias, inside_outside,
                                   out_dim) if geometric_init else None
            setattr(self, 'lin%d' % l, WNLinear(dims[l], out_dim, init, weight_norm))

    def _build_plan(self):
        shapes = [(l.out_features, l.in_features) for l in self._layers()]
        return planlib.build_sdf_plan(shapes, self.skip_in, self.multires, self.aux_cols, self.aux_active,
                                      self.feature_vector_size)

    def evaluate(self, x, n_clamp, n_feat, save=None, split=None, reuse=None):
        if save is None:
            save = torch.is_grad_enabled()
        x = x.detach()
        fused, flat_w, flat_b, wpack, bpack = self.packed(x.device)
        ns = x.shape[0] if split is None else int(split)
        if self.aux_active and ops.HASH_SCATTER == 'binned' and self.encoding.level_dim > 1:
            enc = self.encoding
            sdf, _, feat, nrm, nrm_b = ops.GridSdfFunction.apply(
                x, enc.embeddings, enc.offsets, flat_w, flat_b, wpack, bpack, fused, enc.kernel_dims, int(n_clamp),
                int(n_feat), self.sphere_scale, bool(save), ns, float(self.divide_factor))
            feat = self._trim_features(feat)
            return (sdf, feat, nrm) if split is None else (sdf, feat, nrm, nrm_b)
        aux, handle = None, None
        if self.aux_active:
            aux, handle = self.encoding.encode_with_jacobian((x / self.divide_factor + 1.0) / 2.0)
            aux = self._pad_aux(aux)
        radius = self.sdf_bounding_sphere if self.clamps else 0.0
        sdf, _, feat, nrm, nrm_b, r_aux = ops.SdfMlpFunction.apply(
            x, aux, flat_w, flat_b, wpack, bpack, fused, int(n_clamp), int(n_feat), radius, self.sphere_scale,
            bool(save), ns, reuse)
        if self.aux_active:
            r_aux = r_aux[:, :self.aux_cols]
            through_grid = self.encoding.input_gradient(handle, r_aux) * (0.5 / self.divide_factor)
            nrm = nrm + through_grid[:ns]
            nrm_b = nrm_b + through_grid[ns:]
        feat = self._trim_features(feat)
        if split is None:
            return sdf, feat, nrm
        return sdf, feat, nrm, nrm_b

    def _trim_features(self, feat):
        F = self.feature_vector_size
        return feat if feat.shape[1] == F else feat[:, :F]

    def _pad_aux(self, aux):
        pad = (-aux.shape[1]) % 16
        if pad:
            aux = torch.nn.functional.pad(aux, (0, pad))
        return aux.contiguous()

    def gradient_sdf(self, x):
        return self.evaluate(x, 0, 0)[2]

    def get_outputs(self, x):
        P = x.shape[0]
        return self.evaluate(x, P, P)

    def raw_sdf(self, x):
        with torch.no_grad():
            return self._sdf_only(x, clamp=False)[:, 0]

    def sdf_reuse(self, device, N, S, n_extra, n_eik, save):
        fused = self.packed(device)[0]
        if fused.precision != 'fp32' or self.aux_active or N <= 0 or n_extra <= 0:
            return None
        return ops.SdfReuse(fused, N, S, n_extra, n_eik, save, device)

    def _sdf_only(self, x, run_flag=None, clamp=True, save_for=None):
        fused, _, _, wpack, bpack = self.packed(x.device)
        if save_for is not None:
            reuse, col_slot, n_cols = save_for
            radius = self.sdf_bounding_sphere if (self.clamps and clamp) else 0.0
            return ops.sdf_forward_save(fused, wpack, bpack, x.detach(), radius, self.sphere_scale, run_flag, reuse,
                                        col_slot, n_cols)
        aux, aux_lm = None, None
        if self.aux_active:
            enc = self.encoding
            if x.shape[-1] == 3 and x.dim() == 2:
                aux, aux_lm = ops.hash_node_features(
                    x, self.divide_factor, enc.embeddings, enc.offsets, enc.kernel_dims, 16 * fused.plan.aux_tiles,
                    level_major=(fused.precision == 'fp32'))
            else:
                with torch.no_grad():
                    aux = self._pad_aux(enc((x / self.divide_factor).detach(), calc_grad_inputs=False))
        radius = self.sdf_bounding_sphere if (self.clamps and clamp) else 0.0
        return ops.sdf_forward_nograd(fused, wpack, bpack, x.detach(), aux, radius, self.sphere_scale, run_flag, aux_lm)


class ImplicitNetwork(_SdfBase):
    def __init__(self, feature_vector_size, sdf_bounding_sphere, d_in, d_out, dims, geometric_init=True,
                 bias=1.0, skip_in=(), weight_norm=True, multires=0, sphere_scale=1.0, inside_outside=False):
# ... 103 lines not shown
        else:
            dirs = view_dirs
        code = None
        if self.per_image_code:
            n_rays = P // samples_per_ray
            if not if_pixel_input:
                code = self.embeddings[indices].expand(n_rays, -1)
            else:
                code = self.embeddings[indices]
                if code.shape[0] != n_rays:
                    code = code.unsqueeze(1).expand(-1, n_rays // code.shape[0], -1).flatten(0, 1)
            code = code.contiguous()
        fused, flat_w, flat_b, wpack, bpack = self.packed(points.device)
        rgb = ops.ColorMlpFunction.apply(points, dirs, normals, feature_vectors, code, flat_w, flat_b, wpack, bpack,
                                         fused, int(samples_per_ray), torch.is_grad_enabled())
        return {'rgb': rgb}


class MonoSDFNetwork(nn.Module):
    def __init__(self, conf, if_hdr=False):
        super().__init__()
        self.feature_vector_size = conf.get_int('feature_vector_size')
        self.scene_bounding_sphere = conf.get_float('scene_bounding_sphere', default=1.0)
        self.white_bkgd = conf.get_bool('white_bkgd', default=False)
        self.register_buffer('bg_color', torch.tensor(conf.get_list('bg_color', default=[1.0, 1.0, 1.0])).float(),
                             persistent=False)
        self.if_hdr = if_hdr
        Grid_MLP = conf.get_bool('Grid_MLP', default=False)
        self.Grid_MLP = Grid_MLP
        sphere = 0.0 if self.white_bkgd else self.scene_bounding_sphere
        cls = ImplicitNetworkGrid if Grid_MLP else ImplicitNetwork
        self.implicit_network = cls(self.feature_vector_size, sphere, **conf.get_config('implicit_network'))
        self.rendering_network = RenderingNetwork(self.feature_vector_size, **conf.get_config('rendering_network'),
                                                  if_hdr=self.if_hdr)
        self.spec = False
        self.density = LaplaceDensity(**conf.get_config('density'))
        self.ray_sampler = ErrorBoundSampler(self.scene_bounding_sphere, **conf.get_config('ray_sampler'))
        self._noise = None
        env = os.environ.get('MSDF_SPECULATE_ROUNDS', '1')
        self.speculate_rounds = False if env == '0' else ('all' if env == 'all' else True)

    def set_precision(self, precision):
        self.implicit_network.set_precision(precision)
        self.rendering_network.set_precision(precision)
        return self

    def _bg_list(self):
        bg = getattr(self, '_bg_cache', None)
        if bg is None:
            bg = [float(v) for v in self.bg_color.tolist()]
            object.__setattr__(self, '_bg_cache', bg)
        return bg

    def _rays(self, input_dict, if_pixel_input):
        if not if_pixel_input:
            uv, pose, intrinsics = input_dict['uv'], input_dict['pose'], input_dict['intrinsics']
            if uv.shape[0] != 1:
                raise NotImplementedError('image mode renders one image (one pose) per call, as the runner does')
            ray_dirs, ray_dirs_tmp, cam_loc = ops.camera_rays(uv[0], pose[0], intrinsics[0])
            ray_dirs, ray_dirs_tmp = ray_dirs.unsqueeze(0), ray_dirs_tmp.unsqueeze(0)
        else:
            ray_dirs = input_dict['ray_dirs'].unsqueeze(0)
            cam_loc = input_dict['ray_cam_loc']
            ray_dirs_tmp = input_dict['ray_dirs_tmp'].unsqueeze(0)
        return ray_dirs, cam_loc, ray_dirs_tmp

    def forward(self, input_dict, indices, if_pixel_input=False):
        ray_dirs, cam_loc, ray_dirs_tmp = self._rays(input_dict, if_pixel_input)
        depth_scale = ray_dirs_tmp[0, :, 2:]
        batch_size, num_pixels, _ = ray_dirs.shape
        ray_dirs = ray_dirs.reshape(-1, 3).contiguous()
        cam_loc = cam_loc.contiguous()
        device = ray_dirs.device
        noise = self._noise or {}
        net = self.implicit_network
        beta = ops.effective_beta(self.density.beta, self.density.beta_min_f)
        net.share(device)
        self.rendering_network.share(device)
        try:
            pose = input_dict['ray_pose'] if if_pixel_input else input_dict['pose'][:1]
            K = self.ray_sampler.max_total_iters
            mode = self.speculate_rounds
            guess = 0 if not mode else (K if mode == 'all' else min(K, self.ray_sampler.guess_rounds()))
            for attempt in (guess, K if guess else 0):
                smp = self.ray_sampler
                reuse = net.sdf_reuse(device, ray_dirs.shape[0], smp.N_samples + smp.N_samples_extra + 2,
                                      smp.N_samples_extra, 4 * ray_dirs.shape[0] if self.training else 0,
                                      torch.is_grad_enabled())
                z_vals, z_samples_eik, x_all = self.ray_sampler.sample(ray_dirs, cam_loc, self, speculate=attempt,
                                                                      beta0=beta, sdf_reuse=reuse)
                N, S = z_vals.shape
                P = N * S
                points_flat = x_all[:P]
                sdf, feature_vectors, gradients_sdf, grad_eik = net.evaluate(x_all, P, P, save=torch.is_grad_enabled(),
                                                                                split=P, reuse=reuse)
                rgb_flat = self.rendering_network(points_flat, gradients_sdf, ray_dirs, feature_vectors, indices,
                                                  if_pixel_input=if_pixel_input, samples_per_ray=S)['rgb']
                rgb = rgb_flat.reshape(-1, S, 3)
                weights, rgb_values, depth_values, normal_map, depth_vals = ops.CompositeFunction.apply(
                    z_vals, sdf, rgb_flat, gradients_sdf, beta, depth_scale, self.white_bkgd,
                    self._bg_list(), pose, self.density.beta, True)
                if attempt == 0 or attempt == K or self.ray_sampler.confirm():
                    break
        finally:
            net.unshare()
            self.rendering_network.unshare()

        output = {
            'rgb': rgb,
            'rgb_values': rgb_values,
            'depth_values': depth_values,
            'z_vals': z_vals,
            'depth_vals': depth_vals,
            'sdf': sdf.reshape(z_vals.shape),
            'weights': weights,
        }
        if self.training:
            output['grad_theta'], output['grad_theta_nei'] = ops.SplitRowsFunction.apply(grad_eik,
                                                                                          grad_eik.shape[0] // 2)
        output['normal_map'] = normal_map
        return output

    def volume_rendering(self, z_vals, sdf):
        N, S = z_vals.shape
        zeros = torch.zeros(N * S, 3, device=z_vals.device)
        ones = torch.ones(N, device=z_vals.device)
        return ops.CompositeFunction.apply(z_vals, sdf, zeros, zeros, self.density.get_beta(), ones, False,
                                           [0.0, 0.0, 0.0])[0]
```

monosdf_amd/model/ray_sampler.py:

```python
import ctypes as C

import torch

from .. import _lib


class RaySampler:
    def __init__(self, near, far):
        self.near, self.far = near, far


def _need_gpu(t):
    if not t.is_cuda:
        raise RuntimeError('monosdf_amd: the samplers run on the GPU only (no CPU fallback)')
    return t.detach().float().contiguous()


class UniformSampler(RaySampler):

    def __init__(self, scene_bounding_sphere, near, N_samples, take_sphere_intersection=False, far=-1):
        super().__init__(near, 2.0 * scene_bounding_sphere * 1.75 if far == -1 else far)
        self.N_samples = N_samples
        self.scene_bounding_sphere = scene_bounding_sphere
        self.take_sphere_intersection = take_sphere_intersection

    def get_z_vals(self, ray_dirs, cam_loc, model, jitter=None):
        ray_dirs, cam_loc = _need_gpu(ray_dirs), _need_gpu(cam_loc)
        dev = ray_dirs.device
        N, n = ray_dirs.shape[0], self.N_samples
        f32 = dict(device=dev, dtype=torch.float32)
        if model.training and jitter is None:
            jitter = torch.rand(N, n, **f32)
        z = torch.empty(N, n, **f32)
        far = torch.empty(N, 1, **f32)
        scratch = torch.empty(N * n * 5 + N, **f32)
        a = _lib.SamplerArgs()
        a.ray_o, a.ray_d, a.N = cam_loc.data_ptr(), ray_dirs.data_ptr(), N
        a.M, a.m_max, a.n_eval, a.n_final, a.n_extra = n, n, n, 0, 0
        a.max_rounds = 1
        a.near, a.far = float(self.near), float(self.far)
        a.bound = float(self.scene_bounding_sphere) if self.take_sphere_intersection else 0.0
        a.lemma = 1.0
        a.z, a.new_z = z.data_ptr(), scratch.data_ptr()
        a.new_pos = scratch.data_ptr() + 4 * N * n
        a.pts, a.beta = scratch.data_ptr() + 8 * N * n, scratch.data_ptr() + 20 * N * n
        a.jitter = _need_gpu(jitter).data_ptr() if jitter is not None else None
        a.far_out = far.data_ptr()
        _lib.call('msdf_sampler_init', C.byref(a), _lib.stream_ptr())
        self._keep = (jitter, scratch)
        return z, torch.full((N, 1), float(self.near), **f32), far


class ErrorBoundSampler(RaySampler):
    def __init__(self, scene_bounding_sphere, near, N_samples, N_samples_eval, N_samples_extra, eps, beta_iters,
                 max_total_iters, inverse_sphere_bg=False, N_samples_inverse_sphere=0, add_tiny=1.0e-6):
        super().__init__(near, 2.0 * scene_bounding_sphere * 1.75)
        if inverse_sphere_bg:
# ... 67 lines not shown
        key = (str(dev), n_eval, K, n_extra)
        if key not in self._eval_columns:
            rows = [torch.linspace(0, n_eval * (k + 1) - 1, n_extra).long() for k in range(K)]
            slots = self.column_slots(rows[0], n_eval)
            self._eval_columns[key] = (torch.stack(rows).to(dev), slots.to(dev) if slots is not None else None)
        return self._eval_columns[key]

    @property
    def last_rounds(self):
        self._resolve()
        return self._last_rounds

    @last_rounds.setter
    def last_rounds(self, value):
        self._resolve()
        self._last_rounds = int(value)

    def _resolve(self):
        if self._pending is None:
            return True
        ev, host, k, which = self._pending
        self._pending = None
        ev.synchronize()
        ran = 1
        while ran <= k and int(host[2 * (ran - 1) + 1]):
            ran += 1
        if ran > k:
            self.stats['repeats'] += 1
            self._note_rounds(k + 1, which)
            self._miss[which] = self.HISTORY
            return False
        self.stats['idle_rounds'] += k - ran
        self._note_rounds(ran, which)
        return True

    def confirm(self):
        if self._pending is None or self._pending[2] >= self.max_total_iters:
            return True
        return self._resolve()

    HISTORY = 32

    def _note_rounds(self, rounds, which=0):
        self._last_rounds = rounds
        self._hist[which] = (self._hist[which] + [rounds])[-self.HISTORY:]

    def guess_rounds(self):
        which = 1 if self.global_rounds is not None else 0
        if self._miss[which] > 0:
            self._miss[which] -= 1
            return self.max_total_iters
        return max(self._hist[which]) if self._hist[which] else 1

    def sample(self, ray_dirs, cam_loc, model, want_points=True, speculate=0, beta0=None, sdf_reuse=None):
        dev = ray_dirs.device
        ray_dirs, cam_loc = _need_gpu(ray_dirs), _need_gpu(cam_loc)
        self._resolve()
        N = ray_dirs.shape[0]
        n_eval, n_final, n_extra = self.N_samples_eval, self.N_samples, self.N_samples_extra
        K = self.max_total_iters
        m_max = n_eval * K
        S = n_final + n_extra + 2
        noise = getattr(model, '_noise', None) or {}
        training = bool(model.training)
        net = model.implicit_network
        beta0 = (model.density.get_beta() if beta0 is None else beta0).detach().float().reshape(1).contiguous()
        f32 = dict(device=dev, dtype=torch.float32)
        z = torch.empty(N, m_max, **f32)
        sdf = torch.empty(N, m_max, **f32)
        new_z = torch.empty(N, n_eval, **f32)
        new_pos = torch.empty(N, n_eval, device=dev, dtype=torch.int32)
        pts = torch.empty(N * n_eval, 3, **f32)
        beta = torch.empty(N, **f32)
        flags = torch.empty(2 * K, device=dev, dtype=torch.int32)
        final_z = torch.empty(N, n_final, **f32)
        jitter = u_final = nei_drawn = eik_u_drawn = eik_unit_drawn = None
        if training:
            need = [k for k in ('jitter', 'final_u', 'nei_rand', 'eik_idx', 'eik_uniform') if noise.get(k) is None]
            sizes = {'jitter': N * n_eval, 'final_u': N * n_final, 'nei_rand': 6 * N if want_points else 0,
                     'eik_idx': N, 'eik_uniform': 3 * N if want_points else 0}
            pool = torch.rand(sum(sizes[k] for k in need), **f32) if need else None
            drawn, off = {}, 0
            for k in need:
                drawn[k] = pool[off:off + sizes[k]]
                off += sizes[k]
            jitter = noise.get('jitter')
            jitter = drawn['jitter'].view(N, n_eval) if jitter is None else jitter.to(**f32).contiguous()
            u_final = noise.get('final_u')
            u_final = drawn['final_u'].view(N, n_final) if u_final is None else u_final.to(**f32).contiguous()
            nei_drawn = drawn.get('nei_rand')
            eik_u_drawn, eik_unit_drawn = drawn.get('eik_idx'), drawn.get('eik_uniform')
        a = _lib.SamplerArgs()
        a.ray_o, a.ray_d, a.N = cam_loc.data_ptr(), ray_dirs.data_ptr(), N
        a.m_max, a.n_eval, a.n_final, a.n_extra = m_max, n_eval, n_final, n_extra
        a.max_rounds, a.training, a.beta_iters = K, int(training), self.beta_iters
        a.near, a.far, a.bound = float(self.near), float(self.far), float(self.scene_bounding_sphere)
        a.eps, a.add_tiny, a.lemma = float(self.eps), float(self.add_tiny), self._lemma
        a.beta0, a.z, a.sdf = beta0.data_ptr(), z.data_ptr(), sdf.data_ptr()
        a.new_z, a.new_pos, a.pts, a.beta = new_z.data_ptr(), new_pos.data_ptr(), pts.data_ptr(), beta.data_ptr()
        a.flags = flags.data_ptr()
        a.jitter = jitter.data_ptr() if jitter is not None else None
        a.u_final = u_final.data_ptr() if u_final is not None else None
        a.final_z = final_z.data_ptr()
        extra_idx = col_slot = None
        if sdf_reuse is not None:
            assert want_points and (sdf_reuse.N, sdf_reuse.S, sdf_reuse.n_extra) == (N, S, n_extra)
            assert sdf_reuse.P == N * S + (4 * N if training else 0)
            sdf_reuse.flags = flags
            sdf_reuse.round_pts = pts
            a.row_map, a.h_saved = sdf_reuse.row_map.data_ptr(), sdf_reuse.h_saved.data_ptr()
            if sdf_reuse.n_reuse > 0 and speculate in (0, 1):
                extra_idx, col_slot = self._extra_columns(training, noise, dev, want_slots=True)
        st = _lib.stream_ptr()
        a.M = n_eval
        _lib.call('msdf_sampler_init', C.byref(a), st)
        z_out = z_eik = x_all = eik_idx = None

        def prepare_finish():
            nonlocal z_out, z_eik, x_all, extra_idx, eik_idx
            eik_idx = noise.get('eik_idx')
            a.eik_u, a.eik_unit = None, 0
            if eik_idx is None and eik_u_drawn is not None:
                a.eik_idx, a.eik_u = None, eik_u_drawn.data_ptr()
            else:
                if eik_idx is None:
                    eik_idx = torch.randint(S, (N,), device=dev)
                eik_idx = eik_idx.to(device=dev, dtype=torch.int64).contiguous()
                a.eik_idx = eik_idx.data_ptr()
            z_out = torch.empty(N, S, **f32)
            z_eik = torch.empty(N, 1, **f32)
            a.z_out, a.z_eik, a.pts_out = z_out.data_ptr(), z_eik.data_ptr(), None
            if want_points:
                n_eik = 4 * N if training else 0
                x_all = torch.empty(N * S + n_eik, 3, **f32)
                a.pts_out = x_all.data_ptr()
                if training:
                    R = self.scene_bounding_sphere
                    eik_uniform = noise.get('eik_uniform')
                    if eik_uniform is None and eik_unit_drawn is not None and eik_unit_drawn.numel() == 3 * N:
                        eik_uniform, a.eik_unit = eik_unit_drawn.view(N, 3), 1
                    else:
                        eik_uniform = (torch.empty(N, 3, **f32).uniform_(-R, R) if eik_uniform is None
                                       else eik_uniform.to(**f32).contiguous())
                    nei = noise.get('nei_rand')
                    nei = nei_drawn.view(2 * N, 3) if nei is None else nei.to(**f32).contiguous()
                    a.eik_uniform, a.nei_rand = eik_uniform.data_ptr(), nei.data_ptr()
                    self._keep = (eik_uniform, nei)
            if extra_idx is None:
                extra_idx = self._extra_columns(training, noise, dev)[0]
            a.extra_idx = extra_idx.data_ptr()

        group = self.global_rounds
        which = 1 if group is not None else 0
        rounds = 0
        with torch.no_grad():
            while True:
                run_flag = flags.data_ptr() + 4 * (2 * rounds - 1) if (speculate > 0 and rounds > 0) else None
                save_for = (sdf_reuse, col_slot, n_eval) if (rounds == 0 and col_slot is not None) else None
                new_sdf = net._sdf_only(pts, run_flag=run_flag, save_for=save_for)
                a.new_sdf = new_sdf.data_ptr()
                a.M, a.round_idx = n_eval * (rounds + 1), rounds
                _lib.call('msdf_sampler_beta', C.byref(a), st)
                if group is not None:
                    import torch.distributed as dist
                    dist.all_reduce(flags[2 * rounds:2 * rounds + 1], op=dist.ReduceOp.MAX,
                                    group=None if group is True else group)
                _lib.call('msdf_sampler_resample', C.byref(a), st)
                if rounds == 0:
                    prepare_finish()
                rounds += 1
                if speculate > 0:
                    more = rounds < min(speculate, K)
                else:
                    more = bool(flags[2 * rounds - 1].item())
                if not more:
                    break
        self._pending = None
        self.stats['calls'] += 1
        if speculate > 0:
            host = torch.empty(flags.shape, dtype=flags.dtype, pin_memory=True)
            host.copy_(flags, non_blocking=True)
            ev = torch.cuda.Event()
            ev.record()
            self._pending = (ev, host, rounds, which)
        else:
            self._note_rounds(rounds, which)
        _lib.call('msdf_sampler_finish', C.byref(a), st)
        return z_out, z_eik, x_all
```

monosdf_amd/ops.py:

```python
import collections
import ctypes as C

import numpy as np
import torch

from . import _lib, parallel, plan as planlib


def _need_cuda(t, name):
    if not t.is_cuda:
        raise RuntimeError('monosdf_amd: %s must be a GPU tensor (the HIP path has no CPU fallback)' % name)
    if t.dtype != torch.float32:
        raise RuntimeError('monosdf_amd: %s must be float32' % name)
    return t.contiguous()


def _pad64(n):
    return (n + 63) // 64 * 64


def _cont(t):
    return None if t is None else t.contiguous()


# ... 12 lines not shown
_PENDING = []
USE_SIDE_STREAM = _os.environ.get('MSDF_SIDE_STREAM', '1') != '0'
COLOR_WGRAD_EARLY = _os.environ.get('MSDF_COLOR_WGRAD_EARLY', '1') != '0'
FUSE_JACOBIAN = _os.environ.get('MSDF_FUSE_JACOBIAN', '1') != '0'


def _side_stream(device):
    key = torch.device(device).index if torch.device(device).index is not None else torch.cuda.current_device()
    if key not in _SIDE_STREAMS:
        _SIDE_STREAMS[key] = torch.cuda.Stream(device=key)
    return _SIDE_STREAMS[key]


def start_side_work(device):
    if not _DEFERRED:
        return
    main, side = torch.cuda.current_stream(), _side_stream(device)
    side.wait_stream(main)
    with torch.cuda.stream(side):
        for launch in _DEFERRED:
            launch(side)
        done = torch.cuda.Event()
        done.record(side)
    _DEFERRED.clear()
    _PENDING.append(done)


def join_side_work():
    if _DEFERRED:
        cur = torch.cuda.current_stream()
        for launch in _DEFERRED:
            launch(cur)
        _DEFERRED.clear()
    if _PENDING:
        cur = torch.cuda.current_stream()
        for ev in _PENDING:
            cur.wait_event(ev)
        _PENDING.clear()


class FusedMlp:

    def __init__(self, mlp_plan, device, precision='fp32'):
        if precision not in PRECISIONS:
            raise ValueError('monosdf_amd: precision must be one of %s, got %r' % (PRECISIONS, precision))
        self.mp = mlp_plan
        self.device = device
        self.precision = precision
        self.plan = mlp_plan.plan if precision == 'fp32' else mlp_plan.build_b16(_PLANES[precision])
        self.rules_dev = torch.from_numpy(mlp_plan.rules_np).to(device)
        self.maps_dev = torch.from_numpy(mlp_plan.maps_np).to(device)
        self._wgrad_cache = {}

    def pack(self, flat_w, flat_b):
        mp = self.mp
        flat_w = _need_cuda(flat_w.detach(), 'weights')
        flat_b = _need_cuda(flat_b.detach(), 'biases')
        assert flat_w.numel() == mp.n_w and flat_b.numel() == mp.n_b
        units16 = mp.wpack_f4 if self.precision == 'fp32' else mp.wpack16_units(_PLANES[self.precision])
        wpack = torch.empty(units16 * 4 + 4 * 17 * 64 * 4, device=self.device, dtype=torch.float32)
        bpack = torch.empty(mp.bpack_f + 64, device=self.device, dtype=torch.float32)
        _lib.call('msdf_pack_weights', C.byref(self.plan), _lib.ptr(self.rules_dev), _lib.ptr(self.maps_dev),
                  _lib.ptr(flat_w), _lib.ptr(flat_b), _lib.ptr(wpack), _lib.ptr(bpack), _lib.stream_ptr())
        return wpack, bpack

    def wgrad_program(self, P_pad):
        key = P_pad
        if key not in self._wgrad_cache:
            build = planlib.build_sdf_wgrad if self.mp.kind == 'sdf' else planlib.build_color_wgrad
            program = planlib.uniform_program if self.precision == 'bf16x3' else planlib.balanced_program
            prog = program(build, self.mp, P_pad)
            rules_dev = torch.from_numpy(prog.rules_bytes()).to(self.device)
            wg_map = torch.from_numpy(prog.wg_map()).to(self.device)
            items_dev = torch.from_numpy(prog.items_bytes()).to(self.device)
            full = prog.writes_every_element(self.mp.n_w + self.mp.n_b, self.mp.maps_np)
            self._wgrad_cache[key] = dict(prog=prog, rules=rules_dev, wg_map=wg_map, items=items_dev, full=full)
        return self._wgrad_cache[key]

    def run_wgrad(self, P_pad, base_addr, defer=False):
        ent = self.wgrad_program(P_pad)
        prog = ent['prog']
        items_dev = ent['items']
        bases = [base_addr.get(name) for name in prog.BUFFERS]
        part = torch.empty(prog.part_f + 64, device=self.device, dtype=torch.float32)
        alloc = torch.empty if ent['full'] else torch.zeros
        grad = alloc(self.mp.n_w + self.mp.n_b, device=self.device, dtype=torch.float32)
        wg_map = ent['wg_map']
        held = list(base_addr.values())

        rules_dev = ent['rules']

        def launch(stream=None):
            if stream is not None:
                for t in held + [part, grad, items_dev, wg_map, rules_dev, self.maps_dev]:
                    t.record_stream(stream)
            st = _lib.stream_ptr()
            _lib.call('msdf_wgrad', _lib.ptr(items_dev), _lib.ptr(wg_map), wg_map.numel() // 2,
                      _lib.ptr(part), P_pad, PRECISIONS.index(self.precision), _lib.ptr(bases[0]), _lib.ptr(bases[1]), st)
            _lib.call('msdf_reduce', _lib.ptr(rules_dev), len(prog.rules), _lib.ptr(self.maps_dev),
                      _lib.ptr(part), _lib.ptr(grad), st)

        if defer:
            _DEFERRED.append(launch)
        else:
            launch()
        return grad


class WeightNormTables:

    def __init__(self, shapes, tensors):
        dev = tensors[0].device
        recs, row_layer, w_off, b_off, it = [], [], 0, 0, iter(tensors)
        for i, (rows, cols, has_g) in enumerate(shapes):
            r = _lib.WnLayer()
            v = next(it)
            g = next(it) if has_g else None
            b = next(it)
            r.v, r.g, r.b = v.data_ptr(), _addr(g), b.data_ptr()
            r.rows, r.cols = rows, cols
            r.w_off, r.b_off, r.row_off, r.has_g = w_off, b_off, b_off, int(has_g)
            recs.append(bytes(r))
            row_layer += [i] * rows
            w_off += rows * cols
            b_off += rows
        self.layers_dev = torch.from_numpy(np.frombuffer(b''.join(recs), dtype=np.uint8).copy()).to(dev)
        self.row_layer_dev = torch.tensor(row_layer, dtype=torch.int32, device=dev)
        self.n_w, self.total_rows = w_off, b_off


class WeightNormState:

    def __init__(self):
        self.key, self.cur = None, None

    def tables(self, shapes, tensors):
        key = tuple(t.data_ptr() for t in tensors)
        if key != self.key:
            self.cur = WeightNormTables(shapes, tensors)
            self.key = key
        return self.cur


class FusedWeightNormFunction(torch.autograd.Function):

    @staticmethod
    def forward(ctx, state, shapes, *params):
        st = state.tables(shapes, params)
        dev = params[0].device
        flat_w = torch.empty(st.n_w, device=dev, dtype=torch.float32)
        flat_b = torch.empty(st.total_rows, device=dev, dtype=torch.float32)
        norms = torch.empty(st.total_rows, device=dev, dtype=torch.float32)
        _lib.call('msdf_weightnorm_forward', _lib.ptr(st.layers_dev), _lib.ptr(st.row_layer_dev), st.total_rows,
                  _lib.ptr(flat_w), _lib.ptr(flat_b), _lib.ptr(norms), _lib.stream_ptr())
        ctx.state, ctx.shapes = state, shapes
        ctx.save_for_backward(norms, *params)
        return flat_w, flat_b

    @staticmethod
    @torch.autograd.function.once_differentiable
    def backward(ctx, g_w, g_b):
        norms, *params = ctx.saved_tensors
        shapes = ctx.shapes
        st = ctx.state.tables(shapes, params)
        dev = norms.device
        join_side_work()
        g_w = g_w.contiguous()
        dv = torch.empty(st.n_w, device=dev, dtype=torch.float32)
        dg = torch.empty(st.total_rows, device=dev, dtype=torch.float32)
        _lib.call('msdf_weightnorm_backward', _lib.ptr(st.layers_dev), _lib.ptr(st.row_layer_dev), st.total_rows,
                  _lib.ptr(g_w), _lib.ptr(norms), _lib.ptr(dv), _lib.ptr(dg), _lib.stream_ptr())
        grads, w_off, b_off = [], 0, 0
        for rows, cols, has_g in shapes:
            n = rows * cols
            grads.append(dv[w_off:w_off + n].view(rows, cols))
            if has_g:
                grads.append(dg[b_off:b_off + rows].view(rows, 1))
            grads.append(g_b[b_off:b_off + rows])
            w_off += n
            b_off += rows
        return (None, None) + tuple(grads)


def fused_weight_norm(state, layers):
    params, shapes = [], []
    for l in layers:
        params.append(l.weight_v if l.has_weight_norm else l.weight)
        if l.has_weight_norm:
            params.append(l.weight_g)
        params.append(l.bias)
        shapes.append((l.out_features, l.in_features, bool(l.has_weight_norm)))
    return FusedWeightNormFunction.apply(state, tuple(shapes), *params)


REUSE_SAMPLER_H = _os.environ.get('MSDF_REUSE_SAMPLER_H', '1') != '0'
FG_REUSE_LAST = _os.environ.get('MSDF_FG_REUSE_LAST', '1') != '0'


def _fg_wg_first(reuse):
    return reuse.n_reuse // 64 % (reuse.P_pad // 64) if FG_REUSE_LAST else 0


class SdfReuse:

    def __init__(self, mlp, N, S, n_extra, n_eik, save, device):
        self.mlp, self.N, self.S, self.n_extra, self.save = mlp, N, S, n_extra, bool(save)
        self.P = N * S + n_eik
        self.P_pad = _pad64(max(self.P, 1))
        woff, total = planlib.sdf_workspace(mlp.mp, self.P_pad)
        if not save:
            total = woff['PM']
        self.ws = torch.empty(max(total, 64), device=device, dtype=torch.float32)
        self.stage_pad = _pad64(max(N * n_extra, 1))
        self.stage = torch.empty(mlp.plan.hsum * self.stage_pad, device=device, dtype=torch.float32) \
            if REUSE_SAMPLER_H else None
        self.row_map = torch.empty(max(self.P, 1), device=device, dtype=torch.int32)
        self.h_saved = torch.empty(1, device=device, dtype=torch.int32)
        self.flags = None
        self.round_pts = None
        self.n_split = N * S
        self.n_reuse = (N * n_extra) // 64 * 64 if REUSE_SAMPLER_H else 0


def sdf_forward_save(mlp, wpack, bpack, x, clamp_radius, sphere_scale, run_flag, reuse, col_slot, n_cols):
    x = _need_cuda(x, 'points')
    P = x.shape[0]
    out = torch.empty(P, 1, device=x.device, dtype=torch.float32)
    _lib.call('msdf_sdf_forward_save', C.byref(mlp.plan), _lib.ptr(wpack), _lib.ptr(bpack), _lib.ptr(x), None, 0, 0, P,
              float(clamp_radius), float(sphere_scale), _lib.ptr(out), C.c_void_p(run_flag) if run_flag else None,
              _lib.ptr(reuse.stage), reuse.stage_pad, _lib.ptr(col_slot), int(n_cols), reuse.n_extra,
              _lib.ptr(reuse.h_saved), _lib.stream_ptr())
    return out


def sdf_forward_nograd(mlp, wpack, bpack, x, aux, clamp_radius, sphere_scale, run_flag=None, aux_lm=None):
    x = _need_cuda(x, 'points')
    P = x.shape[0]
    out = torch.empty(P, 1, device=x.device, dtype=torch.float32)
    aC, aLC = aux_lm if aux_lm is not None else (0, 0)
    _lib.call('msdf_sdf_forward_lm', C.byref(mlp.plan), _lib.ptr(wpack), _lib.ptr(bpack),
              _lib.ptr(x), _lib.ptr(aux), int(aC), int(aLC), P, float(clamp_radius), float(sphere_scale), _lib.ptr(out),
              C.c_void_p(run_flag) if run_flag else None, _lib.stream_ptr())
    return out


_SdfState = collections.namedtuple(
    '_SdfState', 'mlp P P_pad n_feat n_split saved has_aux aux_lm aux_shape jac_scale')


def _sdf_fwd_grad(x, aux, wpack, bpack, mlp, n_clamp, n_feat, clamp_radius, sphere_scale, save, n_split=None,
                  aux_lm=None, aux_jac=None, reuse=None):
    mp = mlp.mp
    plan = mlp.plan
    x = _need_cuda(x.detach(), 'points')
    P = x.shape[0]
    P_pad = _pad64(max(P, 1))
    dev = x.device
    has_aux = plan.aux_tiles > 0
    aux = _need_cuda(aux.detach(), 'aux features') if has_aux else None
    woff, total = planlib.sdf_workspace(mp, P_pad)
    if not save:
        total = woff['PM']
    if reuse is not None:
        ns = P if n_split is None else int(n_split)
        if not (mlp.precision == 'fp32' and reuse.mlp is mlp and reuse.P == P and reuse.P_pad == P_pad and
                bool(save) == reuse.save and not has_aux and n_feat == n_clamp == ns == reuse.n_split and
                reuse.n_reuse <= n_feat and reuse.flags is not None):
            raise RuntimeError('monosdf_amd: SdfReuse does not describe this SDF evaluation')
        ws = reuse.ws
    else:
        ws = torch.empty(max(total, 64), device=dev, dtype=torch.float32)
    F = 16 * plan.feat_tiles
    sdf = torch.empty(P, 1, device=dev, dtype=torch.float32)
    feat_full = torch.empty(_pad64(max(n_feat, 1)), F, device=dev, dtype=torch.float32)
    feat_full[n_feat:].zero_()
    feat = feat_full[:n_feat]
    nrm = torch.empty(P, 3, device=dev, dtype=torch.float32)
    aC, aLC = aux_lm if (aux_lm is not None and has_aux) else (0, 0)
    aux_shape = (aLC // aC, P, aC) if aC else (P, 16 * plan.aux_tiles)
    r_aux = torch.empty(*aux_shape, device=dev, dtype=torch.float32) if has_aux else None
    clamped = torch.empty(max(P, 1), device=dev, dtype=torch.uint8)
    a = _lib.FgArgs()
    a.wpack, a.bpack, a.x, a.aux = wpack.data_ptr(), bpack.data_ptr(), x.data_ptr(), _addr(aux)
    a.P, a.P_pad, a.n_clamp, a.n_feat = P, P_pad, n_clamp, n_feat
    a.clamp_radius, a.sphere_scale = float(clamp_radius), float(sphere_scale)
    a.sdf, a.feat, a.nrm, a.r_aux, a.clamped = sdf.data_ptr(), feat.data_ptr(), nrm.data_ptr(), _addr(r_aux), \
        clamped.data_ptr()
    base = ws.data_ptr()
    a.H = base + 4 * woff['H']
    a.PM = base + 4 * woff['PM'] if save else None
    a.IN0 = base + 4 * woff['IN0'] if save else None
    a.save = 1 if save else 0
    a.aux_C, a.aux_LC = int(aC), int(aLC)
    jac_scale = None
    if aux_jac is not None and aC == 2:
        jac_scale = float(aux_jac[1])
        a.dy_dx, a.aux_dx_scale = aux_jac[0].data_ptr(), jac_scale
    saved = (x, ws, clamped, wpack, bpack)
    if reuse is not None:
        a.row_map, a.n_reuse = reuse.row_map.data_ptr(), reuse.n_reuse
        a.smp_flags, a.h_saved = reuse.flags.data_ptr(), reuse.h_saved.data_ptr()
        a.h_stage, a.stage_pad = _addr(reuse.stage), reuse.stage_pad
        a.wg_first = _fg_wg_first(reuse)
        saved += (reuse.row_map,)
    if P > 0:
        _lib.call('msdf_sdf_fwd_grad', C.byref(plan), C.byref(a), _lib.stream_ptr())
    ns = P if n_split is None else int(n_split)
    state = _SdfState(mlp, P, P_pad, n_feat, ns, save, has_aux, (int(aC), int(aLC)), aux_shape, jac_scale)
    return (sdf[:ns], sdf[ns:], feat, nrm[:ns], nrm[ns:], r_aux), saved, state


def _sdf_backward(state, saved, grads, dy_dx=None, gg_out=None, after_sweeps=None):
    if not state.saved:
        raise RuntimeError('monosdf_amd: backward through an inference-mode SDF evaluation')
    x, ws, clamped, wpack, bpack, *row_map = saved
    mlp, P, P_pad = state.mlp, state.P, state.P_pad
    mp = mlp.mp
    dev = x.device
    woff, _ = planlib.sdf_workspace(mp, P_pad)
    g_sdf, g_sdf_b, g_feat, g_nrm, g_nrm_b, g_raux = [_cont(g) for g in grads]
    g_aux = torch.empty(*state.aux_shape, device=dev, dtype=torch.float32) if state.has_aux else None
    b = _lib.BwArgs()
    b.aux_C, b.aux_LC = state.aux_lm
    if state.jac_scale is not None:
        b.dy_dx, b.aux_dx_scale, b.gg_out = dy_dx.data_ptr(), state.jac_scale, _addr(gg_out)
    b.wpack, b.bpack, b.x = wpack.data_ptr(), bpack.data_ptr(), x.data_ptr()
    b.P, b.P_pad, b.n_feat, b.n_split = P, P_pad, state.n_feat, state.n_split
    b.g_sdf, b.g_sdf_b, b.g_nrm, b.g_nrm_b = _addr(g_sdf), _addr(g_sdf_b), _addr(g_nrm), _addr(g_nrm_b)
    b.g_feat = _addr(g_feat) if state.n_feat > 0 else None
    b.g_raux = _addr(g_raux) if state.has_aux else None
    b.clamped = clamped.data_ptr()
    b.row_map = row_map[0].data_ptr() if row_map else None
    base = ws.data_ptr()
    for k in ('H', 'PM', 'QB', 'AB', 'GSDF', 'QLAST'):
        setattr(b, k, base + 4 * woff[k])
    b.g_aux = _addr(g_aux)
    if P > 0:
        _lib.call('msdf_sdf_backward', C.byref(mlp.plan), C.byref(b), _lib.stream_ptr())
        start_side_work(dev)
    if after_sweeps is not None:
        after_sweeps(g_aux)
    grad = mlp.run_wgrad(P_pad, {'ws': ws}) if P > 0 else torch.zeros(mp.n_w + mp.n_b, device=dev)
    return g_aux, grad


class SdfMlpFunction(torch.autograd.Function):

    @staticmethod
    def forward(ctx, x, aux, flat_w, flat_b, wpack, bpack, mlp, n_clamp, n_feat, clamp_radius,
                sphere_scale, save, n_split=None, reuse=None):
        ctx.set_materialize_grads(False)
        outs, saved, ctx.state = _sdf_fwd_grad(x, aux, wpack, bpack, mlp, n_clamp, n_feat, clamp_radius,
                                               sphere_scale, save, n_split, reuse=reuse)
        ctx.save_for_backward(*saved)
        return outs

    @staticmethod
    @torch.autograd.function.once_differentiable
    def backward(ctx, *grads):
        g_aux, grad = _sdf_backward(ctx.state, ctx.saved_tensors, grads)
        n_w = ctx.state.mlp.mp.n_w
        return (None, g_aux, grad[:n_w], grad[n_w:]) + (None,) * 10


def _encode_points(x, divide_factor, embeddings, offsets, enc, pitch, level_major, jacobian):
    x = _need_cuda(x.detach(), 'points')
    emb = _need_cuda(embeddings.detach(), 'embeddings')
    L, Cdim, S, H = enc
    B, D = x.shape
    dev = x.device
    x01 = torch.empty(B, D, device=dev, dtype=torch.float32) if jacobian else None
    outputs = torch.empty(L, B, Cdim, device=dev, dtype=torch.float32)
    dy_dx = torch.empty(B, L * D * Cdim, device=dev, dtype=torch.float32) if jacobian else None
    st = _lib.stream_ptr()
    _lib.call('msdf_hash_node_forward', _lib.ptr(x), float(divide_factor), _lib.ptr(x01), _lib.ptr(emb),
              _lib.ptr(offsets), _lib.ptr(outputs), 0, B, Cdim, L, S, H, _lib.ptr(dy_dx), st)
    if Cdim == 2 and level_major:
        return x, outputs, (Cdim, L * Cdim), x01, dy_dx
    aux = torch.empty(B, pitch, device=dev, dtype=torch.float32)
    _lib.call('msdf_hash_transpose', _lib.ptr(outputs), _lib.ptr(aux), None, None, L, B, Cdim, pitch, 1, st)
    return x, aux, None, x01, dy_dx


class GridSdfFunction(torch.autograd.Function):

    @staticmethod
    def forward(ctx, x, embeddings, offsets, flat_w, flat_b, wpack, bpack, mlp, enc, n_clamp, n_feat, sphere_scale,
                save, n_split, divide_factor):
        ctx.set_materialize_grads(False)
        L, Cdim, S, H = enc
        A = 16 * mlp.plan.aux_tiles
        x, aux, lm, x01, dy_dx = _encode_points(x, divide_factor, embeddings, offsets, enc, A,
                                                mlp.precision == 'fp32', True)
        B = x.shape[0]
        k = 0.5 / divide_factor
        jac = (dy_dx, k) if (lm is not None and FUSE_JACOBIAN) else None
        (sdf_a, sdf_b, feat, nrm_a, nrm_b, r_aux), saved, ctx.state = _sdf_fwd_grad(
            x, aux, wpack, bpack, mlp, n_clamp, n_feat, 0.0, sphere_scale, save, n_split, lm, jac)
        if jac is None:
            assert nrm_a.data_ptr() + 12 * nrm_a.shape[0] == nrm_b.data_ptr() or nrm_b.shape[0] == 0
            _lib.call('msdf_hash_node_input_gradient', _lib.ptr(r_aux), 0 if lm is not None else A, _lib.ptr(dy_dx), B,
                      Cdim, L, float(k), _lib.ptr(nrm_a), _lib.stream_ptr())
        ctx.enc, ctx.k, ctx.n_entries, ctx.lm, ctx.offsets = enc, k, embeddings.shape[0], lm, offsets
        ctx.save_for_backward(x01, dy_dx, r_aux, *saved)
        return sdf_a, sdf_b, feat, nrm_a, nrm_b

    @staticmethod
    @torch.autograd.function.once_differentiable
    def backward(ctx, g_sdf, g_sdf_b, g_feat, g_nrm, g_nrm_b):
        x01, dy_dx, r_aux, *saved = ctx.saved_tensors
        state, (L, Cdim, S, H), k, lm = ctx.state, ctx.enc, ctx.k, ctx.lm
        B, D = x01.shape
        dev = x01.device
        st = _lib.stream_ptr()
        A = 16 * state.mlp.plan.aux_tiles
# ... 69 lines not shown
        woff, total = planlib.color_workspace(mp, P_pad)
        ws = torch.empty(max(total if save else 64, 64), device=dev, dtype=torch.float32)
        rgb = torch.empty(P, 3, device=dev, dtype=torch.float32)
        a = _lib.ColorFwdArgs()
        a.wpack, a.bpack = wpack.data_ptr(), bpack.data_ptr()
        a.x, a.dirs, a.nrm, a.feat = x.data_ptr(), dirs.data_ptr(), nrm.data_ptr(), feat.data_ptr()
        a.code = _addr(code) if has_code else None
        a.P, a.P_pad, a.spr, a.save = P, P_pad, int(spr), 1 if save else 0
        a.rgb = rgb.data_ptr()
        base = ws.data_ptr()
        a.H = base + 4 * woff['H'] if save else None
        a.MISC = base + 4 * woff['MISC'] if save else None
        if P > 0:
            _lib.call('msdf_color_forward', C.byref(plan), C.byref(a), _lib.stream_ptr())
        ctx.cmlp, ctx.P, ctx.P_pad, ctx.saved, ctx.has_code, ctx.spr = cmlp, P, P_pad, save, has_code, spr
        ctx.save_for_backward(rgb, feat, ws, wpack, bpack)
        return rgb

    @staticmethod
    @torch.autograd.function.once_differentiable
    def backward(ctx, g_rgb):
        if not ctx.saved:
            raise RuntimeError('monosdf_amd: backward through an inference-mode colour evaluation')
        rgb, feat, ws, wpack, bpack = ctx.saved_tensors
        cmlp, P, P_pad = ctx.cmlp, ctx.P, ctx.P_pad
        mp = cmlp.mp
        plan = cmlp.plan
        dev = rgb.device
        woff, _ = planlib.color_workspace(mp, P_pad)
        g_rgb = g_rgb.contiguous()
        g_feat = torch.empty_like(feat)
        g_misc = torch.empty(P, 16 * mp.misc_tiles, device=dev, dtype=torch.float32)
        b = _lib.ColorBwdArgs()
        b.wpack, b.bpack, b.rgb, b.g_rgb = wpack.data_ptr(), bpack.data_ptr(), rgb.data_ptr(), g_rgb.data_ptr()
        b.P, b.P_pad = P, P_pad
        base = ws.data_ptr()
        b.H, b.AB = base + 4 * woff['H'], base + 4 * woff['AB']
        b.g_feat, b.g_misc = g_feat.data_ptr(), g_misc.data_ptr()
        g_nrm = torch.empty(P, 3, device=dev, dtype=torch.float32) if plan.mode == 1 else None
        b.g_nrm = _addr(g_nrm)
        if P > 0:
            _lib.call('msdf_color_backward', C.byref(plan), C.byref(b), _lib.stream_ptr())
            grad = cmlp.run_wgrad(P_pad, {'ws': ws, 'feat': feat}, defer=USE_SIDE_STREAM)
            if USE_SIDE_STREAM and COLOR_WGRAD_EARLY:
                start_side_work(dev)
        else:
            grad = torch.zeros(mp.n_w + mp.n_b, device=dev)
        g_code = None
        if ctx.has_code:
            g_code = g_misc[:, 48:].reshape(P // ctx.spr, ctx.spr, -1).sum(1)
        if ctx.feat_cols < g_feat.shape[1]:
            g_feat = g_feat[:, :ctx.feat_cols]
        return (None, None, g_nrm, g_feat, g_code, grad[:mp.n_w], grad[mp.n_w:], None, None, None, None, None)


class CompositeFunction(torch.autograd.Function):

    @staticmethod
    def forward(ctx, z, sdf, rgb, nrm, beta, depth_scale, white_bkgd, bg, pose=None, beta_raw=None,
                want_depth_vals=False):
        ctx.set_materialize_grads(False)
        z = _need_cuda(z.detach(), 'z_vals')
        N, S = z.shape
        ctx.in_shapes = (sdf.shape, rgb.shape, nrm.shape)
        sdf = _need_cuda(sdf.detach(), 'sdf').reshape(N, S)
        rgb = _need_cuda(rgb.detach(), 'rgb').reshape(N, S, 3)
        nrm = _need_cuda(nrm.detach(), 'normals').reshape(N, S, 3)
        beta = _need_cuda(beta.detach(), 'beta').reshape(1)
        ctx.beta_shape = None if beta_raw is None else beta_raw.shape
        raw = beta if beta_raw is None else _need_cuda(beta_raw.detach(), 'beta').reshape(1)
        depth_scale = depth_scale.detach()
        if depth_scale.dim() == 2 and depth_scale.shape[0] == N and depth_scale.shape[1] == 1 and N > 0 \
                and depth_scale.is_cuda and depth_scale.dtype == torch.float32 and depth_scale.stride(1) == 1:
            ds_stride = int(depth_scale.stride(0))
        else:
            depth_scale = _need_cuda(depth_scale, 'depth_scale').reshape(N)
            ds_stride = 1
        dev = z.device
        weights = torch.empty(N, S, device=dev)
        rgb_values = torch.empty(N, 3, device=dev)
        depth_values = torch.empty(N, 1, device=dev)
        normal_map = torch.empty(N, 3, device=dev)
        wsum = torch.empty(max(N, 1), device=dev)
        depth_vals = torch.empty(N, S, device=dev) if want_depth_vals else None
        a = _lib.CompositeArgs()
        a.z, a.sdf, a.rgb, a.nrm = z.data_ptr(), sdf.data_ptr(), rgb.data_ptr(), nrm.data_ptr()
        a.beta, a.depth_scale = beta.data_ptr(), depth_scale.data_ptr()
        a.depth_scale_stride = ds_stride
        a.depth_vals = _addr(depth_vals)
        a.N, a.S, a.white_bkgd = N, S, 1 if white_bkgd else 0
        a.bg0, a.bg1, a.bg2 = [float(v) for v in bg]
        a.weights, a.rgb_values, a.depth_values = weights.data_ptr(), rgb_values.data_ptr(), depth_values.data_ptr()
        a.normal_map, a.wsum = normal_map.data_ptr(), wsum.data_ptr()
        if pose is not None:
            pose = _need_cuda(pose.detach(), 'pose').reshape(-1, 4, 4)
            if pose.shape[0] not in (1, N):
                raise RuntimeError('monosdf_amd: pose must be [1,4,4] or [N,4,4]')
            a.pose, a.pose_stride = pose.data_ptr(), (16 if pose.shape[0] == N and N > 1 else 0)
        else:
            pose = z.new_zeros(1)
            a.pose, a.pose_stride = None, 0
        ctx.has_pose, ctx.pose_stride = a.pose is not None, a.pose_stride
        _lib.call('msdf_composite_forward', C.byref(a), _lib.stream_ptr())
        ctx.save_for_backward(z, sdf, rgb, nrm, beta, depth_scale, weights, wsum, depth_values, pose, raw)
        ctx.white_bkgd, ctx.bg, ctx.ds_stride = white_bkgd, [float(v) for v in bg], ds_stride
        if want_depth_vals:
            ctx.mark_non_differentiable(depth_vals)
            return weights, rgb_values, depth_values, normal_map, depth_vals
        return weights, rgb_values, depth_values, normal_map

    @staticmethod
    @torch.autograd.function.once_differentiable
    def backward(ctx, g_w, g_rgbv, g_depth, g_nmap, g_dvals=None):
        z, sdf, rgb, nrm, beta, depth_scale, weights, wsum, depth_values, pose, raw = ctx.saved_tensors
        N, S = z.shape
        dev = z.device
        g_w, g_rgbv, g_depth, g_nmap = _cont(g_w), _cont(g_rgbv), _cont(g_depth), _cont(g_nmap)
        g_sdf = torch.empty(N, S, device=dev)
        g_rgb = torch.empty(N, S, 3, device=dev)
        g_nrm = torch.empty(N, S, 3, device=dev)
        g_beta_part = torch.empty(max(N, 1), device=dev)
        b = _lib.CompositeBwdArgs()
        b.z, b.sdf, b.rgb, b.nrm = z.data_ptr(), sdf.data_ptr(), rgb.data_ptr(), nrm.data_ptr()
        b.beta, b.depth_scale = beta.data_ptr(), depth_scale.data_ptr()
        b.weights, b.wsum, b.depth_values = weights.data_ptr(), wsum.data_ptr(), depth_values.data_ptr()
        b.g_rgb_values, b.g_depth, b.g_normal, b.g_weights = _addr(g_rgbv), _addr(g_depth), _addr(g_nmap), _addr(g_w)
        b.N, b.S, b.white_bkgd = N, S, 1 if ctx.white_bkgd else 0
        b.bg0, b.bg1, b.bg2 = ctx.bg
        b.g_sdf, b.g_rgb, b.g_nrm, b.g_beta_part = g_sdf.data_ptr(), g_rgb.data_ptr(), g_nrm.data_ptr(), \
            g_beta_part.data_ptr()
        b.pose, b.pose_stride = (pose.data_ptr() if ctx.has_pose else None), ctx.pose_stride
        b.depth_scale_stride = ctx.ds_stride
        _lib.call('msdf_composite_backward', C.byref(b), _lib.stream_ptr())
        sh = ctx.in_shapes
        if ctx.beta_shape is not None:
            g_raw = torch.empty(1, device=dev)
            _lib.call('msdf_beta_grad', _lib.ptr(raw), _lib.ptr(g_beta_part), N, _lib.ptr(g_raw), _lib.stream_ptr())
            return (None, g_sdf.reshape(sh[0]), g_rgb.reshape(sh[1]), g_nrm.reshape(sh[2]), None, None, None, None, None,
                    g_raw.reshape(ctx.beta_shape), None)
        g_beta = g_beta_part[:N].sum().reshape(beta.shape)
        return (None, g_sdf.reshape(sh[0]), g_rgb.reshape(sh[1]), g_nrm.reshape(sh[2]), g_beta, None, None, None, None,
                None, None)


def effective_beta(beta_raw, beta_min):
    raw = _need_cuda(beta_raw.detach(), 'beta').reshape(1)
    out = torch.empty(1, device=raw.device, dtype=torch.float32)
    _lib.call('msdf_beta_eff', _lib.ptr(raw), float(beta_min), _lib.ptr(out), _lib.stream_ptr())
    return out


class LaplaceDensityFunction(torch.autograd.Function):

    @staticmethod
    def forward(ctx, sdf, beta):
        s = _need_cuda(sdf.detach(), 'sdf')
        b = _need_cuda(beta.detach().to(s.device), 'beta').reshape(-1)
        cols = s.shape[-1] if s.dim() > 0 else 1
        rows = s.numel() // max(cols, 1)
        if b.numel() not in (1, rows):
            raise RuntimeError('monosdf_amd: beta must hold one value or one per row of sdf')
        stride = int(b.numel() == rows and rows > 1)
        out = torch.empty_like(s)
        _lib.call('msdf_laplace_density', _lib.ptr(s), _lib.ptr(b), stride, s.numel(), max(cols, 1), _lib.ptr(out),
                  _lib.stream_ptr())
        ctx.save_for_backward(s, b)
        ctx.meta = (stride, cols, beta.shape)
        return out

    @staticmethod
    @torch.autograd.function.once_differentiable
    def backward(ctx, g):
        s, b = ctx.saved_tensors
        stride, cols, beta_shape = ctx.meta
        g = g.contiguous()
        g_sdf, g_be = torch.empty_like(s), torch.empty_like(s)
        _lib.call('msdf_laplace_density_backward', _lib.ptr(s), _lib.ptr(b), stride, s.numel(), max(cols, 1),
                  _lib.ptr(g), _lib.ptr(g_sdf), _lib.ptr(g_be), _lib.stream_ptr())
        g_beta = (g_be.reshape(-1, max(cols, 1)).sum(1) if stride else g_be.sum()).reshape(beta_shape)
        return g_sdf, g_beta


HASH_SCATTER = _os.environ.get('MSDF_HASH_SCATTER', 'binned')
if HASH_SCATTER not in ('binned', 'atomic'):
    raise RuntimeError("monosdf_amd: MSDF_HASH_SCATTER must be 'binned' or 'atomic', got %r (the library's switch for "
                       "the first binned form is MSDF_HASH_BINNED_FORM=1)" % HASH_SCATTER)


def _hash_workspace(B, Cdim, L, embeddings):
    n = _lib.load().msdf_hash_scatter_workspace_bytes(B, Cdim, L, embeddings.shape[0])
# ... 232 lines not shown
```

Measured before the change: 123,300 rays/s.

## Fold small plumbing kernels into neighbouring launches across sampler, composite and weight-norm

Several small launches are merged into larger ones. The sampler's last resample round and its finish step run in one kernel, and beta_eff is computed inside sampler init. The beta gradient reduction moves into the composite backward kernel using a last-block ticket. The two networks' weight packing and weight-norm backward are batched into single calls, and a duplicated normal output is added to the fwd_grad kernel. The aim is to cut kernel-launch count and host overhead per training step, at the cost of more complex kernels, extra LDS for the fused sampler, and a cross-block atomic ticket protocol.

Result: no change. 123,600 rays/s, median of 6 (+0.2%).

```diff
diff --git a/include/monosdf_hip.h b/include/monosdf_hip.h
--- a/include/monosdf_hip.h
+++ b/include/monosdf_hip.h
@@ -65,6 +65,10 @@
 
 int msdf_pack_weights(const msdf_plan_t* plan, const msdf_packrule_t* rules_dev, const int* maps_dev,
                       const float* flat_w, const float* flat_b, void* wpack, float* bpack, void* stream);
+int msdf_pack_weights2(const msdf_plan_t* plan0, const msdf_packrule_t* rules0_dev, const int* maps0_dev,
+                       const float* flat_w0, const float* flat_b0, void* wpack0, float* bpack0,
+                       const msdf_plan_t* plan1, const msdf_packrule_t* rules1_dev, const int* maps1_dev,
+                       const float* flat_w1, const float* flat_b1, void* wpack1, float* bpack1, void* stream);
 
 typedef struct {
   const float* v;
@@ -80,6 +84,9 @@
                             float* flat_w, float* flat_b, float* norms, void* stream);
 int msdf_weightnorm_backward(const msdf_wn_layer_t* layers_dev, const int* row_layer_dev, int total_rows,
                              const float* g_flat_w, const float* norms, float* dv_flat, float* dg_rows, void* stream);
+int msdf_weightnorm_backward2(const msdf_wn_layer_t* layers_dev, const int* row_layer_dev, int total_rows,
+                              const float* g_flat_w0, const float* g_flat_w1, int w_split, const float* norms,
+                              float* dv_flat, float* dg_rows, void* stream);
 
 int msdf_sdf_forward(const msdf_plan_t* plan, const void* wpack, const float* bpack, const float* x,
                      const float* aux, int P, float clamp_radius, float sphere_scale, float* sdf, void* stream);
@@ -123,6 +130,8 @@
   int32_t stage_pad;
   const float* h_stage;
   int32_t wg_first;
+  int32_t n_nrm2;
+  float* nrm2;
 } msdf_fg_args_t;
 int msdf_sdf_fwd_grad(const msdf_plan_t* plan, const msdf_fg_args_t* args, void* stream);
 
@@ -154,6 +163,7 @@
   float aux_dx_scale;
   int32_t pad_;
   const int32_t* row_map;
+  const float* g_nrm2;
 } msdf_bw_args_t;
 int msdf_sdf_backward(const msdf_plan_t* plan, const msdf_bw_args_t* args, void* stream);
 
@@ -239,6 +249,9 @@
   const float* pose;
   int32_t pose_stride;
   int32_t depth_scale_stride;
+  const float* beta_raw;
+  float* g_beta_raw;
+  uint32_t* ticket;
 } msdf_composite_bwd_args_t;
 int msdf_composite_backward(const msdf_composite_bwd_args_t* args, void* stream);
 
@@ -321,11 +334,16 @@
   int32_t pad_;
   int32_t* row_map;
   uint32_t* h_saved;
+  const float* beta_raw;
+  float beta_min;
+  int32_t pad2_;
+  float* beta_eff_out;
 } msdf_sampler_args_t;
 int msdf_sampler_init(const msdf_sampler_args_t* args, void* stream);
 int msdf_sampler_beta(const msdf_sampler_args_t* args, void* stream);
 int msdf_sampler_resample(const msdf_sampler_args_t* args, void* stream);
 int msdf_sampler_finish(const msdf_sampler_args_t* args, void* stream);
+int msdf_sampler_resample_finish(const msdf_sampler_args_t* args, void* stream);
 
 int msdf_sampler_error_bound(const float* z, const float* sdf, const float* dstar, const float* beta,
                              int beta_stride, int N, int M, float* out, void* stream);
diff --git a/monosdf_amd/_lib.py b/monosdf_amd/_lib.py
--- a/monosdf_amd/_lib.py
+++ b/monosdf_amd/_lib.py
@@ -51,7 +51,7 @@
                 ('H', _P), ('PM', _P), ('IN0', _P), ('save', C.c_int32), ('aux_C', C.c_int32), ('aux_LC', C.c_int32),
                 ('aux_dx_scale', C.c_float), ('dy_dx', _P),
                 ('row_map', _P), ('smp_flags', _P), ('h_saved', _P), ('n_reuse', C.c_int32), ('stage_pad', C.c_int32), ('h_stage', _P),
-                ('wg_first', C.c_int32)]
+                ('wg_first', C.c_int32), ('n_nrm2', C.c_int32), ('nrm2', _P)]
 
 
 class BwArgs(C.Structure):
@@ -61,7 +61,7 @@
                 ('H', _P), ('PM', _P), ('QB', _P), ('T', _P), ('AB', _P), ('GSDF', _P), ('QLAST', _P),
                 ('g_aux', _P), ('g_sdf_b', _P), ('g_nrm_b', _P), ('aux_C', C.c_int32), ('aux_LC', C.c_int32),
                 ('dy_dx', _P), ('gg_out', _P), ('aux_dx_scale', C.c_float), ('pad_', C.c_int32),
-                ('row_map', _P)]
+                ('row_map', _P), ('g_nrm2', _P)]
 
 
 class ColorFwdArgs(C.Structure):
@@ -92,7 +92,8 @@
                 ('N', C.c_int32), ('S', C.c_int32), ('white_bkgd', C.c_int32),
                 ('bg0', C.c_float), ('bg1', C.c_float), ('bg2', C.c_float),
                 ('g_sdf', _P), ('g_rgb', _P), ('g_nrm', _P), ('g_beta_part', _P),
-                ('pose', _P), ('pose_stride', C.c_int32), ('depth_scale_stride', C.c_int32)]
+                ('pose', _P), ('pose_stride', C.c_int32), ('depth_scale_stride', C.c_int32),
+                ('beta_raw', _P), ('g_beta_raw', _P), ('ticket', _P)]
 
 
 class WnLayer(C.Structure):
@@ -125,7 +126,8 @@
                 ('extra_idx', _P), ('eik_idx', _P), ('z_out', _P), ('z_eik', _P), ('pts_out', _P),
                 ('eik_uniform', _P), ('nei_rand', _P), ('far_out', _P), ('rounds_out', _P),
                 ('dbg_dstar', _P), ('dbg_err0', _P), ('dbg_cdf', _P), ('eik_u', _P), ('eik_unit', C.c_int32),
-                ('pad_', C.c_int32), ('row_map', _P), ('h_saved', _P)]
+                ('pad_', C.c_int32), ('row_map', _P), ('h_saved', _P),
+                ('beta_raw', _P), ('beta_min', C.c_float), ('pad2_', C.c_int32), ('beta_eff_out', _P)]
 
 
 _ERR = {1: 'invalid argument', 2: 'kernel launch failed', 3: 'unsupported configuration'}
@@ -158,7 +160,9 @@
                                C.c_uint32, _P, C.c_uint64, _P, C.c_uint64, _P],
     'msdf_weightnorm_forward': [_P, _P, C.c_int, _P, _P, _P, _P],
     'msdf_weightnorm_backward': [_P, _P, C.c_int, _P, _P, _P, _P, _P],
+    'msdf_weightnorm_backward2': [_P, _P, C.c_int, _P, _P, C.c_int, _P, _P, _P, _P],
     'msdf_pack_weights': [C.POINTER(Plan), _P, _P, _P, _P, _P, _P, _P],
+    'msdf_pack_weights2': [C.POINTER(Plan), _P, _P, _P, _P, _P, _P, C.POINTER(Plan), _P, _P, _P, _P, _P, _P, _P],
     'msdf_sdf_forward': [C.POINTER(Plan), _P, _P, _P, _P, C.c_int, C.c_float, C.c_float, _P, _P],
     'msdf_sdf_forward_if': [C.POINTER(Plan), _P, _P, _P, _P, C.c_int, C.c_float, C.c_float, _P, _P, _P],
     'msdf_sdf_forward_lm': [C.POINTER(Plan), _P, _P, _P, _P, C.c_int, C.c_int, C.c_int, C.c_float, C.c_float, _P, _P, _P],
@@ -182,6 +186,7 @@
     'msdf_sampler_beta': [C.POINTER(SamplerArgs), _P],
     'msdf_sampler_resample': [C.POINTER(SamplerArgs), _P],
     'msdf_sampler_finish': [C.POINTER(SamplerArgs), _P],
+    'msdf_sampler_resample_finish': [C.POINTER(SamplerArgs), _P],
     'msdf_sampler_error_bound': [_P, _P, _P, _P, C.c_int, C.c_int, C.c_int, _P, _P],
     'msdf_laplace_density': [_P, _P, C.c_int, C.c_int64, C.c_int, _P, _P],
     'msdf_laplace_density_backward': [_P, _P, C.c_int, C.c_int64, C.c_int, _P, _P, _P, _P],
diff --git a/monosdf_amd/csrc/composite.hip b/monosdf_amd/csrc/composite.hip
--- a/monosdf_amd/csrc/composite.hip
+++ b/monosdf_amd/csrc/composite.hip
@@ -114,10 +114,7 @@
   return s;
 }
 
-__global__ void __launch_bounds__(256)
-msdf_composite_backward_k(const CompositeBwdArgs a) {
-  const int ray = blockIdx.x * 4 + (threadIdx.x >> 6);
-  if (ray >= a.N) return;
+__device__ __forceinline__ void composite_backward_ray(const CompositeBwdArgs& a, const int ray) {
   const int lane = lane_id();
   const int S = a.S;
   const float beta = a.beta[0];
@@ -215,7 +212,39 @@
     }
   }
   gbeta = wave_sum(gbeta);
-  if (lane == 0) a.g_beta_part[ray] = gbeta;
+  if (lane == 0) {
+    if (a.ticket != nullptr) __hip_atomic_store(a.g_beta_part + ray, gbeta, __ATOMIC_RELAXED, __HIP_MEMORY_SCOPE_AGENT);
+    else a.g_beta_part[ray] = gbeta;
+  }
+}
+
+template <bool COHERENT>
+__device__ __forceinline__ void beta_grad_wave(const float* __restrict__ raw, const float* part, const int n,
+                                               float* __restrict__ g_raw) {
+  const int lane = lane_id();
+  float s = 0.f;
+  for (int i = lane; i < n; i += 64)
+    s += COHERENT ? __hip_atomic_load(part + i, __ATOMIC_RELAXED, __HIP_MEMORY_SCOPE_AGENT) : part[i];
+  s = wave_sum(s);
+  const float r = raw[0];
+  if (lane == 0) g_raw[0] = ((r > 0.f) ? 1.f : (r < 0.f) ? -1.f : 0.f) * s;
+}
+
+__global__ void __launch_bounds__(256)
+msdf_composite_backward_k(const CompositeBwdArgs a) {
+  const int ray = blockIdx.x * 4 + (threadIdx.x >> 6);
+  if (ray < a.N) composite_backward_ray(a, ray);
+  if (a.ticket == nullptr) return;
+  __shared__ uint32_t last;
+  asm volatile("s_waitcnt vmcnt(0)" ::: "memory");
+  __syncthreads();
+  if (threadIdx.x == 0) {
+    const uint32_t t = __hip_atomic_fetch_add(a.ticket, 1u, __ATOMIC_RELAXED, __HIP_MEMORY_SCOPE_AGENT);
+    last = (t == gridDim.x - 1) ? 1u : 0u;
+    if (last) __hip_atomic_store(a.ticket, 0u, __ATOMIC_RELAXED, __HIP_MEMORY_SCOPE_AGENT);
+  }
+  __syncthreads();
+  if (last && threadIdx.x < 64) beta_grad_wave<true>(a.beta_raw, a.g_beta_part, a.N, a.g_beta_raw);
 }
 
 __global__ void msdf_beta_eff_k(const float* __restrict__ raw, const float beta_min, float* __restrict__ out) {
@@ -223,11 +252,7 @@
 }
 __global__ void __launch_bounds__(64)
 msdf_beta_grad_k(const float* __restrict__ raw, const float* __restrict__ part, const int n, float* __restrict__ g_raw) {
-  float s = 0.f;
-  for (int i = threadIdx.x; i < n; i += 64) s += part[i];
-  s = wave_sum(s);
-  const float r = raw[0];
-  if (threadIdx.x == 0) g_raw[0] = ((r > 0.f) ? 1.f : (r < 0.f) ? -1.f : 0.f) * s;
+  beta_grad_wave<false>(raw, part, n, g_raw);
 }
 extern "C" int msdf_beta_eff(const float* beta_raw, float beta_min, float* out, void* stream) {
   if (beta_raw == nullptr || out == nullptr) return MSDF_ERR_ARG;
@@ -249,6 +274,8 @@
 
 extern "C" int msdf_composite_backward(const msdf_composite_bwd_args_t* a, void* stream) {
   if (a == nullptr || a->N < 0 || a->S < 1 || a->S > 64 * CMP_MAX_PER_LANE) return MSDF_ERR_ARG;
+  if ((a->ticket != nullptr) != (a->beta_raw != nullptr) || (a->ticket != nullptr) != (a->g_beta_raw != nullptr))
+    return MSDF_ERR_ARG;
   if (a->N == 0) return MSDF_OK;
   msdf_composite_backward_k<<<(a->N + 3) / 4, 256, 0, (hipStream_t)stream>>>(*a);
   return msdf_check_launch();
diff --git a/monosdf_amd/csrc/sampler.hip b/monosdf_amd/csrc/sampler.hip
--- a/monosdf_amd/csrc/sampler.hip
+++ b/monosdf_amd/csrc/sampler.hip
@@ -40,6 +40,7 @@
   if (ray == 0 && a.flags != nullptr)
     for (int i = lane; i < 2 * a.max_rounds; i += 64) a.flags[i] = 0u;
   if (ray == 0 && lane == 0 && a.h_saved != nullptr) a.h_saved[0] = 0u;
+  if (ray == 0 && lane == 0 && a.beta_eff_out != nullptr) a.beta_eff_out[0] = fabsf(a.beta_raw[0]) + a.beta_min;
   const int n = a.n_eval;
   const float o0 = a.ray_o[ray * 3 + 0], o1 = a.ray_o[ray * 3 + 1], o2 = a.ray_o[ray * 3 + 2];
   const float d0 = a.ray_d[ray * 3 + 0], d1 = a.ray_d[ray * 3 + 1], d2 = a.ray_d[ray * 3 + 2];
@@ -85,9 +86,17 @@
 struct SmpLds {
   float* z; float* sdf; float* dist; float* dstar; float* tmp; float* snew;
 };
-__device__ __forceinline__ SmpLds smp_lds(float* base, const int m_max, const int n_eval) {
+__host__ __device__ __forceinline__ int smp_lds_per(const int m_max, const int n_eval) { return 5 * (m_max + 1) + n_eval; }
+__host__ __device__ __forceinline__ int smp_fin_off(const int m_max, const int n_eval, const int S) {
+  return (2 * S <= 5 * (m_max + 1)) ? 0 : smp_lds_per(m_max, n_eval);
+}
+__host__ __device__ __forceinline__ int smp_lds_per_fused(const int m_max, const int n_eval, const int S) {
+  const int per = smp_lds_per(m_max, n_eval), fin = smp_fin_off(m_max, n_eval, S) + 2 * S;
+  return per > fin ? per : fin;
+}
+__device__ __forceinline__ SmpLds smp_lds(float* base, const int m_max, const int n_eval, const int stride = 0) {
   const int w = threadIdx.x >> 6;
-  const int per = 5 * (m_max + 1) + n_eval;
+  const int per = stride > 0 ? stride : smp_lds_per(m_max, n_eval);
   float* p = base + (size_t)w * per;
   SmpLds l;
   l.z = p; l.sdf = p + (m_max + 1); l.dist = p + 2 * (m_max + 1); l.dstar = p + 3 * (m_max + 1);
@@ -193,13 +202,9 @@
   }
 }
 
-__global__ void __launch_bounds__(64 * SMP_WAVES) smp_resample_k(const SmpArgs a) {
-  extern __shared__ float smp_lds_mem[];
-  const int ray = blockIdx.x * SMP_WAVES + (threadIdx.x >> 6);
-  if (ray >= a.N || !smp_round_active(a)) return;
+__device__ __forceinline__ bool smp_resample_ray(const SmpArgs& a, const SmpLds& l, const int ray) {
   const int lane = lane_id();
   const int M = a.M;
-  const SmpLds l = smp_lds(smp_lds_mem, a.m_max, a.n_eval);
   const float beta0 = a.beta0[0];
   const float maxbeta = __uint_as_float(a.flags[2 * a.round_idx]);
   const bool unconverged = maxbeta > beta0;
@@ -272,7 +277,7 @@
 
   if (!more) {
     for (int j = lane; j < n_new; j += 64) a.final_z[(size_t)ray * a.n_final + j] = l.snew[j];
-    return;
+    return false;
   }
   const float o0 = a.ray_o[ray * 3 + 0], o1 = a.ray_o[ray * 3 + 1], o2 = a.ray_o[ray * 3 + 2];
   const float d0 = a.ray_d[ray * 3 + 0], d1 = a.ray_d[ray * 3 + 1], d2 = a.ray_d[ray * 3 + 2];
@@ -296,24 +301,26 @@
     float* p = a.pts + ((size_t)ray * a.n_eval + j) * 3;
     p[0] = o0 + sj * d0; p[1] = o1 + sj * d1; p[2] = o2 + sj * d2;
   }
-}
-
-__global__ void __launch_bounds__(64 * SMP_WAVES) smp_finish_k(const SmpArgs a) {
+  return true;
+}
+__global__ void __launch_bounds__(64 * SMP_WAVES) smp_resample_k(const SmpArgs a) {
   extern __shared__ float smp_lds_mem[];
   const int ray = blockIdx.x * SMP_WAVES + (threadIdx.x >> 6);
-  if (ray >= a.N) return;
+  if (ray >= a.N || !smp_round_active(a)) return;
+  smp_resample_ray(a, smp_lds(smp_lds_mem, a.m_max, a.n_eval), ray);
+}
+
+__device__ __forceinline__ void smp_finish_ray(const SmpArgs& a, const int ray, float* v, const int rounds,
+                                               const float* fin) {
   const int lane = lane_id();
   const int S = a.n_final + a.n_extra + 2;
-  float* v = smp_lds_mem + (size_t)(threadIdx.x >> 6) * 2 * S;
   float* sorted = v + S;
   const float* zrow = a.z + (size_t)ray * a.m_max;
-  int rounds = 1;
-  while (rounds < a.max_rounds && a.flags[2 * (rounds - 1) + 1] != 0u) ++rounds;
   const int64_t* extra = a.extra_idx + (size_t)(rounds - 1) * a.n_extra;
   if (a.rounds_out != nullptr && ray == 0 && lane == 0) a.rounds_out[0] = rounds;
   for (int j = lane; j < S; j += 64) {
     float x;
-    if (j < a.n_final) x = a.final_z[(size_t)ray * a.n_final + j];
+    if (j < a.n_final) x = (fin != nullptr) ? fin[j] : a.final_z[(size_t)ray * a.n_final + j];
     else if (j == a.n_final) x = a.near;
     else if (j == a.n_final + 1) x = a.far;
     else x = zrow[min((int)extra[j - a.n_final - 2], rounds * a.n_eval - 1)];
@@ -366,6 +373,30 @@
     }
   }
 }
+__global__ void __launch_bounds__(64 * SMP_WAVES) smp_finish_k(const SmpArgs a) {
+  extern __shared__ float smp_lds_mem[];
+  const int ray = blockIdx.x * SMP_WAVES + (threadIdx.x >> 6);
+  if (ray >= a.N) return;
+  int rounds = 1;
+  while (rounds < a.max_rounds && a.flags[2 * (rounds - 1) + 1] != 0u) ++rounds;
+  const int S = a.n_final + a.n_extra + 2;
+  smp_finish_ray(a, ray, smp_lds_mem + (size_t)(threadIdx.x >> 6) * 2 * S, rounds, nullptr);
+}
+
+__global__ void __launch_bounds__(64 * SMP_WAVES) smp_resample_finish_k(const SmpArgs a) {
+  extern __shared__ float smp_lds_mem[];
+  const int ray = blockIdx.x * SMP_WAVES + (threadIdx.x >> 6);
+  if (ray >= a.N) return;
+  const int S = a.n_final + a.n_extra + 2;
+  const SmpLds l = smp_lds(smp_lds_mem, a.m_max, a.n_eval, smp_lds_per_fused(a.m_max, a.n_eval, S));
+  const bool active = smp_round_active(a);
+  const bool more = active && smp_resample_ray(a, l, ray);
+  int rounds = 1;
+  while (rounds <= a.round_idx && a.flags[2 * (rounds - 1) + 1] != 0u) ++rounds;
+  if (more) ++rounds;
+  smp_sync();
+  smp_finish_ray(a, ray, l.z + smp_fin_off(a.m_max, a.n_eval, S), rounds, (active && !more) ? l.snew : nullptr);
+}
 
 __global__ void __launch_bounds__(64 * SMP_WAVES) smp_error_bound_k(const float* __restrict__ z,
                                                                      const float* __restrict__ sdf,
@@ -428,7 +459,7 @@
 }
 
 extern "C" int msdf_sampler_init(const msdf_sampler_args_t* a, void* stream) {
-  if (smp_check(a)) return MSDF_ERR_ARG;
+  if (smp_check(a) || (a->beta_eff_out != nullptr && a->beta_raw == nullptr)) return MSDF_ERR_ARG;
   return smp_launch(smp_init_k, a, 0, stream);
 }
 static int smp_round_check(const msdf_sampler_args_t* a) {
@@ -442,10 +473,16 @@
   if (smp_check(a) || smp_round_check(a) || a->n_final > a->n_eval) return MSDF_ERR_ARG;
   return smp_launch(smp_resample_k, a, smp_lds_bytes(a), stream);
 }
+static int smp_finish_check(const msdf_sampler_args_t* a) {
+  return a->flags == nullptr || (a->extra_idx == nullptr && a->n_extra > 0) || a->m_max < a->n_eval * a->max_rounds;
+}
+extern "C" int msdf_sampler_resample_finish(const msdf_sampler_args_t* a, void* stream) {
+  if (smp_check(a) || smp_round_check(a) || a->n_final > a->n_eval || smp_finish_check(a)) return MSDF_ERR_ARG;
+  const size_t lds = (size_t)SMP_WAVES * smp_lds_per_fused(a->m_max, a->n_eval, a->n_final + a->n_extra + 2) * sizeof(float);
+  return smp_launch(smp_resample_finish_k, a, lds, stream);
+}
 extern "C" int msdf_sampler_finish(const msdf_sampler_args_t* a, void* stream) {
-  if (smp_check(a) || a->flags == nullptr || (a->extra_idx == nullptr && a->n_extra > 0) ||
-      a->m_max < a->n_eval * a->max_rounds)
-    return MSDF_ERR_ARG;
+  if (smp_check(a) || smp_finish_check(a)) return MSDF_ERR_ARG;
   const size_t lds = (size_t)SMP_WAVES * 2 * (a->n_final + a->n_extra + 2) * sizeof(float);
   return smp_launch(smp_finish_k, a, lds, stream);
 }
diff --git a/monosdf_amd/csrc/sdf_kernels.h b/monosdf_amd/csrc/sdf_kernels.h
--- a/monosdf_amd/csrc/sdf_kernels.h
+++ b/monosdf_amd/csrc/sdf_kernels.h
@@ -478,6 +478,11 @@
       a.nrm[(size_t)c.pt * 3 + 0] = n0;
       a.nrm[(size_t)c.pt * 3 + 1] = n1;
       a.nrm[(size_t)c.pt * 3 + 2] = n2;
+      if (Core::ROW_MAP && a.nrm2 != nullptr && c.pt < a.n_nrm2) {
+        a.nrm2[(size_t)c.pt * 3 + 0] = n0;
+        a.nrm2[(size_t)c.pt * 3 + 1] = n1;
+        a.nrm2[(size_t)c.pt * 3 + 2] = n2;
+      }
       a.clamped[c.pt] = is_clamped ? 1 : 0;
     }
     if (a.r_aux != nullptr) {
@@ -493,6 +498,23 @@
 }
 
 typedef msdf_bw_args_t BwArgs;
+
+template <bool SECOND>
+__device__ __forceinline__ void load_g_nrm(const BwArgs& a, const int pt, float& g0, float& g1, float& g2) {
+  const bool first = pt < a.n_split;
+  const float* gnp = first ? a.g_nrm : a.g_nrm_b;
+  const float* gn2 = (SECOND && first) ? a.g_nrm2 : nullptr;
+  const size_t j = first ? (size_t)pt : (size_t)(pt - a.n_split);
+  g0 = g1 = g2 = 0.f;
+  if (gnp != nullptr) {
+    g0 = gnp[j * 3 + 0]; g1 = gnp[j * 3 + 1]; g2 = gnp[j * 3 + 2];
+    if (gn2 != nullptr) {
+      g0 = __fadd_rn(g0, gn2[j * 3 + 0]); g1 = __fadd_rn(g1, gn2[j * 3 + 1]); g2 = __fadd_rn(g2, gn2[j * 3 + 2]);
+    }
+  } else if (gn2 != nullptr) {
+    g0 = gn2[j * 3 + 0]; g1 = gn2[j * 3 + 1]; g2 = gn2[j * 3 + 2];
+  }
+}
 
 template <bool LM>
 __device__ __forceinline__ void load_rbar(v4f (&rbar)[5], const msdf_plan_t& plan, const BwArgs& a,
@@ -525,24 +547,14 @@
   if (live) {
     const bool first = c.pt < a.n_split;
     const float* gsp = first ? a.g_sdf : a.g_sdf_b;
-    const float* gnp = first ? a.g_nrm : a.g_nrm_b;
     const size_t j = first ? (size_t)c.pt : (size_t)(c.pt - a.n_split);
     if (gsp) gs = gsp[j];
-    if (gnp) {
-      gn0 = gnp[j * 3 + 0];
-      gn1 = gnp[j * 3 + 1];
-      gn2 = gnp[j * 3 + 2];
-    }
+    load_g_nrm<Core::ROW_MAP>(a, c.pt, gn0, gn1, gn2);
   }
   if (c.q == 0) a.GSDF[c.pt] = gs;
   if (Core::AUX_LEVEL_MAJOR && a.gg_out != nullptr && c.valid && c.q == 0) {
-    float r0 = 0.f, r1 = 0.f, r2 = 0.f;
-    const bool first = c.pt < a.n_split;
-    const float* gnp = first ? a.g_nrm : a.g_nrm_b;
-    if (gnp != nullptr) {
-      const size_t j = first ? (size_t)c.pt : (size_t)(c.pt - a.n_split);
-      r0 = gnp[j * 3 + 0]; r1 = gnp[j * 3 + 1]; r2 = gnp[j * 3 + 2];
-    }
+    float r0, r1, r2;
+    load_g_nrm<Core::ROW_MAP>(a, c.pt, r0, r1, r2);
     a.gg_out[(size_t)c.pt * 3 + 0] = __fmul_rn(r0, a.aux_dx_scale);
     a.gg_out[(size_t)c.pt * 3 + 1] = __fmul_rn(r1, a.aux_dx_scale);
     a.gg_out[(size_t)c.pt * 3 + 2] = __fmul_rn(r2, a.aux_dx_scale);
diff --git a/monosdf_amd/csrc/sdf_mlp.hip b/monosdf_amd/csrc/sdf_mlp.hip
--- a/monosdf_amd/csrc/sdf_mlp.hip
+++ b/monosdf_amd/csrc/sdf_mlp.hip
@@ -1,20 +1,27 @@
 #include "mlp_launch.h"
 
-__global__ void __launch_bounds__(256) msdf_pack_kernel(const msdf_plan_t plan,
-                                                        const msdf_packrule_t* __restrict__ rules,
-                                                        const int* __restrict__ maps,
-                                                        const float* __restrict__ flat_w,
-                                                        const float* __restrict__ flat_b,
-                                                        v4f* __restrict__ wpack, float* __restrict__ bpack) {
-  const int l = blockIdx.y;
-  const int which = blockIdx.z;
+struct PackSet {
+  const msdf_packrule_t* rules;
+  const int* maps;
+  const float* flat_w;
+  const float* flat_b;
+  v4f* wpack;
+  float* bpack;
+};
+
+__device__ __forceinline__ void pack_layer_f32(const msdf_plan_t& plan, const PackSet& s, const int l, const int which,
+                                               const int t0, const int stride) {
+  const msdf_packrule_t* __restrict__ rules = s.rules;
+  const int* __restrict__ maps = s.maps;
+  const float* __restrict__ flat_w = s.flat_w;
+  const float* __restrict__ flat_b = s.flat_b;
+  v4f* __restrict__ wpack = s.wpack;
+  float* __restrict__ bpack = s.bpack;
   const msdf_layer_t L = plan.layer[l];
   const msdf_packrule_t R = rules[l];
   const int* rowmap = maps + R.rowmap_off;
   const int* colmap = maps + R.colmap_off;
   const float* W = flat_w + R.w_off;
-  const int stride = gridDim.x * blockDim.x;
-  const int t0 = blockIdx.x * blockDim.x + threadIdx.x;
   if (which < 2) {
     const int n_rt = which == 0 ? L.ot : L.kt;
     const int n_kt = which == 0 ? L.kt : L.ot;
@@ -45,6 +52,24 @@
   }
 }
 
+__global__ void __launch_bounds__(256) msdf_pack_kernel(const msdf_plan_t plan,
+                                                        const msdf_packrule_t* __restrict__ rules,
+                                                        const int* __restrict__ maps,
+                                                        const float* __restrict__ flat_w,
+                                                        const float* __restrict__ flat_b,
+                                                        v4f* __restrict__ wpack, float* __restrict__ bpack) {
+  const PackSet s = {rules, maps, flat_w, flat_b, wpack, bpack};
+  pack_layer_f32(plan, s, blockIdx.y, blockIdx.z, blockIdx.x * blockDim.x + threadIdx.x, gridDim.x * blockDim.x);
+}
+
+__global__ void __launch_bounds__(256) msdf_pack2_kernel(const msdf_plan_t plan0, const PackSet s0,
+                                                         const msdf_plan_t plan1, const PackSet s1) {
+  const int l = blockIdx.y;
+  const int t0 = blockIdx.x * blockDim.x + threadIdx.x, stride = gridDim.x * blockDim.x;
+  if (l < plan0.n_layers) pack_layer_f32(plan0, s0, l, blockIdx.z, t0, stride);
+  else pack_layer_f32(plan1, s1, l - plan0.n_layers, blockIdx.z, t0, stride);
+}
+
 __global__ void __launch_bounds__(CoreF32::THREADS, CoreF32::WGS_PER_CU)
 msdf_sdf_forward_k(const msdf_plan_t plan, const v4f* __restrict__ wpack, const float* __restrict__ bpack,
                    const float* __restrict__ x, const float* __restrict__ aux, const AuxView av, const int P,
@@ -101,6 +126,20 @@
                                                              bpack);
     return msdf_check_launch();
   });
+}
+
+extern "C" int msdf_pack_weights2(const msdf_plan_t* plan0, const msdf_packrule_t* rules0, const int* maps0,
+                                  const float* flat_w0, const float* flat_b0, void* wpack0, float* bpack0,
+                                  const msdf_plan_t* plan1, const msdf_packrule_t* rules1, const int* maps1,
+                                  const float* flat_w1, const float* flat_b1, void* wpack1, float* bpack1, void* stream) {
+  if (plan0 == nullptr || plan0->n_layers < 1 || plan0->n_layers > MSDF_MAX_LAYERS) return MSDF_ERR_ARG;
+  if (plan1 == nullptr || plan1->n_layers < 1 || plan1->n_layers > MSDF_MAX_LAYERS) return MSDF_ERR_ARG;
+  if (plan0->precision != MSDF_PRECISION_F32 || plan1->precision != MSDF_PRECISION_F32) return MSDF_ERR_UNSUPPORTED;
+  const PackSet s0 = {rules0, maps0, flat_w0, flat_b0, (v4f*)wpack0, bpack0};
+  const PackSet s1 = {rules1, maps1, flat_w1, flat_b1, (v4f*)wpack1, bpack1};
+  const dim3 grid(32, plan0->n_layers + plan1->n_layers, 3);
+  msdf_pack2_kernel<<<grid, 256, 0, (hipStream_t)stream>>>(*plan0, s0, *plan1, s1);
+  return msdf_check_launch();
 }
 
 static bool aux_layout_ok(const msdf_plan_t* plan, const int aux_C, const int aux_LC) {
@@ -172,10 +211,11 @@
                          a->stage_pad < a->n_reuse))
     return MSDF_ERR_ARG;
   if (a->wg_first < 0 || a->wg_first >= a->P_pad / CoreF32::PTS_PER_WG) return MSDF_ERR_ARG;
+  if (a->nrm2 != nullptr && (a->n_nrm2 < 0 || a->n_nrm2 > a->P)) return MSDF_ERR_ARG;
   return mlp_with_core(plan, [&](auto core) {
     typedef decltype(core) Core;
     if (!Core::AUX_LEVEL_MAJOR && (a->aux_C != 0 || a->dy_dx != nullptr)) return MSDF_ERR_UNSUPPORTED;
-    if (!Core::ROW_MAP && a->wg_first != 0) return MSDF_ERR_UNSUPPORTED;
+    if (!Core::ROW_MAP && (a->wg_first != 0 || a->nrm2 != nullptr)) return MSDF_ERR_UNSUPPORTED;
     return mlp_launch<Core>(fwd_grad_kernel(core), a->P_pad / Core::PTS_PER_WG, stream, *plan, *a);
   });
 }
@@ -189,6 +229,7 @@
   return mlp_with_core(plan, [&](auto core) {
     typedef decltype(core) Core;
     if (!Core::AUX_LEVEL_MAJOR && (a->aux_C != 0 || a->dy_dx != nullptr)) return MSDF_ERR_UNSUPPORTED;
+    if (!Core::ROW_MAP && a->g_nrm2 != nullptr) return MSDF_ERR_UNSUPPORTED;
     return mlp_launch<Core>(backward_kernel(core), a->P_pad / Core::PTS_PER_WG, stream, *plan, *a);
   });
 }
diff --git a/monosdf_amd/csrc/weightnorm.hip b/monosdf_amd/csrc/weightnorm.hip
--- a/monosdf_amd/csrc/weightnorm.hip
+++ b/monosdf_amd/csrc/weightnorm.hip
@@ -32,6 +32,7 @@
 __global__ void __launch_bounds__(256)
 msdf_weightnorm_backward_k(const msdf_wn_layer_t* __restrict__ layers, const int* __restrict__ row_layer,
                            const int total_rows, const float* __restrict__ g_flat_w,
+                           const float* __restrict__ g_flat_w1, const int w_split,
                            const float* __restrict__ norms, float* __restrict__ dv_flat,
                            float* __restrict__ dg_rows) {
   const int row_g = blockIdx.x * 4 + (threadIdx.x >> 6);
@@ -40,7 +41,7 @@
   const msdf_wn_layer_t L = layers[row_layer[row_g]];
   const int r = row_g - L.row_off;
   const float* v = L.v + (size_t)r * L.cols;
-  const float* dw = g_flat_w + L.w_off + (size_t)r * L.cols;
+  const float* dw = (L.w_off < w_split ? g_flat_w + L.w_off : g_flat_w1 + (L.w_off - w_split)) + (size_t)r * L.cols;
   float* dv = dv_flat + L.w_off + (size_t)r * L.cols;
   if (!L.has_g) {
     for (int c = lane; c < L.cols; c += 64) dv[c] = dw[c];
@@ -72,6 +73,16 @@
   if (total_rows < 0) return MSDF_ERR_ARG;
   if (total_rows == 0) return MSDF_OK;
   msdf_weightnorm_backward_k<<<(total_rows + 3) / 4, 256, 0, (hipStream_t)stream>>>(
-      layers_dev, row_layer_dev, total_rows, g_flat_w, norms, dv_flat, dg_rows);
+      layers_dev, row_layer_dev, total_rows, g_flat_w, nullptr, 0x7fffffff, norms, dv_flat, dg_rows);
   return msdf_check_launch();
 }
+
+extern "C" int msdf_weightnorm_backward2(const msdf_wn_layer_t* layers_dev, const int* row_layer_dev, int total_rows,
+                                         const float* g_flat_w0, const float* g_flat_w1, int w_split,
+                                         const float* norms, float* dv_flat, float* dg_rows, void* stream) {
+  if (total_rows < 0 || w_split < 0 || g_flat_w0 == nullptr || g_flat_w1 == nullptr) return MSDF_ERR_ARG;
+  if (total_rows == 0) return MSDF_OK;
+  msdf_weightnorm_backward_k<<<(total_rows + 3) / 4, 256, 0, (hipStream_t)stream>>>(
+      layers_dev, row_layer_dev, total_rows, g_flat_w0, g_flat_w1, w_split, norms, dv_flat, dg_rows);
+  return msdf_check_launch();
+}
diff --git a/monosdf_amd/model/network.py b/monosdf_amd/model/network.py
--- a/monosdf_amd/model/network.py
+++ b/monosdf_amd/model/network.py
@@ -124,7 +124,7 @@
         return planlib.build_sdf_plan(shapes, self.skip_in, self.multires, self.aux_cols, self.aux_active,
                                       self.feature_vector_size)
 
-    def evaluate(self, x, n_clamp, n_feat, save=None, split=None, reuse=None):
+    def evaluate(self, x, n_clamp, n_feat, save=None, split=None, reuse=None, nrm_twice=False):
         if save is None:
             save = torch.is_grad_enabled()
         x = x.detach()
@@ -136,15 +136,18 @@
                 x, enc.embeddings, enc.offsets, flat_w, flat_b, wpack, bpack, fused, enc.kernel_dims, int(n_clamp),
                 int(n_feat), self.sphere_scale, bool(save), ns, float(self.divide_factor))
             feat = self._trim_features(feat)
-            return (sdf, feat, nrm) if split is None else (sdf, feat, nrm, nrm_b)
+            if split is None:
+                return sdf, feat, nrm
+            return (sdf, feat, nrm, nrm_b, nrm) if nrm_twice else (sdf, feat, nrm, nrm_b)
         aux, handle = None, None
         if self.aux_active:
             aux, handle = self.encoding.encode_with_jacobian((x / self.divide_factor + 1.0) / 2.0)
             aux = self._pad_aux(aux)
         radius = self.sdf_bounding_sphere if self.clamps else 0.0
-        sdf, _, feat, nrm, nrm_b, r_aux = ops.SdfMlpFunction.apply(
+        twice = bool(nrm_twice) and split is not None and fused.precision == 'fp32' and not self.aux_active
+        sdf, _, feat, nrm, nrm_b, r_aux, *nrm2 = ops.SdfMlpFunction.apply(
             x, aux, flat_w, flat_b, wpack, bpack, fused, int(n_clamp), int(n_feat), radius, self.sphere_scale,
-            bool(save), ns, reuse)
+            bool(save), ns, reuse, twice)
         if self.aux_active:
             r_aux = r_aux[:, :self.aux_cols]
             through_grid = self.encoding.input_gradient(handle, r_aux) * (0.5 / self.divide_factor)
@@ -153,6 +156,8 @@
         feat = self._trim_features(feat)
         if split is None:
             return sdf, feat, nrm
+        if nrm_twice:
+            return sdf, feat, nrm, nrm_b, (nrm2[0] if twice else nrm)
         return sdf, feat, nrm, nrm_b
 
     def _trim_features(self, feat):
@@ -362,6 +367,22 @@
             object.__setattr__(self, '_bg_cache', bg)
         return bg
 
+    def _share_weights(self, device):
+        net, col = self.implicit_network, self.rendering_network
+        fa, fb = net._fused(device), col._fused(device)
+        if not (ops.FOLD_PLUMBING and fa.precision == 'fp32' and fb.precision == 'fp32'):
+            net.share(device)
+            col.share(device)
+            return
+        wn = getattr(self, '_wn_state', None)
+        if wn is None:
+            wn = ops.WeightNormState()
+            object.__setattr__(self, '_wn_state', wn)
+        w_a, b_a, w_b, b_b = ops.fused_weight_norm2(wn, net._layers(), col._layers())
+        packs_a, packs_b = ops.pack_weights2(fa, w_a, b_a, fb, w_b, b_b)
+        object.__setattr__(net, '_shared', (fa, w_a, b_a) + packs_a)
+        object.__setattr__(col, '_shared', (fb, w_b, b_b) + packs_b)
+
     def _rays(self, input_dict, if_pixel_input):
         if not if_pixel_input:
             uv, pose, intrinsics = input_dict['uv'], input_dict['pose'], input_dict['intrinsics']
@@ -384,9 +405,14 @@
         device = ray_dirs.device
         noise = self._noise or {}
         net = self.implicit_network
-        beta = ops.effective_beta(self.density.beta, self.density.beta_min_f)
-        net.share(device)
-        self.rendering_network.share(device)
+        fold = ops.FOLD_PLUMBING and self.training and ray_dirs.shape[0] > 0
+        if fold:
+            beta = torch.empty(1, device=device, dtype=torch.float32)
+            beta_eff = (self.density.beta, self.density.beta_min_f, beta)
+        else:
+            beta = ops.effective_beta(self.density.beta, self.density.beta_min_f)
+            beta_eff = None
+        self._share_weights(device)
         try:
             pose = input_dict['ray_pose'] if if_pixel_input else input_dict['pose'][:1]
             K = self.ray_sampler.max_total_iters
@@ -398,13 +424,15 @@
                                       smp.N_samples_extra, 4 * ray_dirs.shape[0] if self.training else 0,
                                       torch.is_grad_enabled())
                 z_vals, z_samples_eik, x_all = self.ray_sampler.sample(ray_dirs, cam_loc, self, speculate=attempt,
-                                                                      beta0=beta, sdf_reuse=reuse)
+                                                                      beta0=beta, sdf_reuse=reuse, beta_eff=beta_eff)
                 N, S = z_vals.shape
                 P = N * S
                 points_flat = x_all[:P]
-                sdf, feature_vectors, gradients_sdf, grad_eik = net.evaluate(x_all, P, P, save=torch.is_grad_enabled(),
-                                                                                split=P, reuse=reuse)
-                rgb_flat = self.rendering_network(points_flat, gradients_sdf, ray_dirs, feature_vectors, indices,
+                twice = ops.FOLD_PLUMBING and torch.is_grad_enabled()
+                sdf, feature_vectors, gradients_sdf, grad_eik, *second = net.evaluate(
+                    x_all, P, P, save=torch.is_grad_enabled(), split=P, reuse=reuse, nrm_twice=twice)
+                gradients_color = second[0] if twice else gradients_sdf
+                rgb_flat = self.rendering_network(points_flat, gradients_color, ray_dirs, feature_vectors, indices,
                                                   if_pixel_input=if_pixel_input, samples_per_ray=S)['rgb']
                 rgb = rgb_flat.reshape(-1, S, 3)
                 weights, rgb_values, depth_values, normal_map, depth_vals = ops.CompositeFunction.apply(
diff --git a/monosdf_amd/model/ray_sampler.py b/monosdf_amd/model/ray_sampler.py
--- a/monosdf_amd/model/ray_sampler.py
+++ b/monosdf_amd/model/ray_sampler.py
@@ -2,7 +2,7 @@
 
 import torch
 
-from .. import _lib
+from .. import _lib, ops
 
 
 class RaySampler:
@@ -176,7 +176,8 @@
             return self.max_total_iters
         return max(self._hist[which]) if self._hist[which] else 1
 
-    def sample(self, ray_dirs, cam_loc, model, want_points=True, speculate=0, beta0=None, sdf_reuse=None):
+    def sample(self, ray_dirs, cam_loc, model, want_points=True, speculate=0, beta0=None, sdf_reuse=None,
+               beta_eff=None):
         dev = ray_dirs.device
         ray_dirs, cam_loc = _need_gpu(ray_dirs), _need_gpu(cam_loc)
         self._resolve()
@@ -188,6 +189,11 @@
         noise = getattr(model, '_noise', None) or {}
         training = bool(model.training)
         net = model.implicit_network
+        if beta_eff is not None and N > 0:
+            beta0 = beta_eff[2]
+            assert beta0.is_cuda and beta0.dtype == torch.float32 and beta0.numel() == 1 and beta0.is_contiguous()
+        else:
+            beta_eff = None
         beta0 = (model.density.get_beta() if beta0 is None else beta0).detach().float().reshape(1).contiguous()
         f32 = dict(device=dev, dtype=torch.float32)
         z = torch.empty(N, m_max, **f32)
@@ -226,6 +232,9 @@
         a.jitter = jitter.data_ptr() if jitter is not None else None
         a.u_final = u_final.data_ptr() if u_final is not None else None
         a.final_z = final_z.data_ptr()
+        if beta_eff is not None:
+            beta_raw = beta_eff[0].detach().float().reshape(1).contiguous()
+            a.beta_raw, a.beta_min, a.beta_eff_out = beta_raw.data_ptr(), float(beta_eff[1]), beta0.data_ptr()
         extra_idx = col_slot = None
         if sdf_reuse is not None:
             assert want_points and (sdf_reuse.N, sdf_reuse.S, sdf_reuse.n_extra) == (N, S, n_extra)
@@ -289,8 +298,11 @@
                     import torch.distributed as dist
                     dist.all_reduce(flags[2 * rounds:2 * rounds + 1], op=dist.ReduceOp.MAX,
                                     group=None if group is True else group)
-                _lib.call('msdf_sampler_resample', C.byref(a), st)
-                if rounds == 0:
+                fused = ops.FOLD_PLUMBING and speculate > 0 and rounds + 1 >= min(speculate, K)
+                if rounds == 0 and fused:
+                    prepare_finish()
+                _lib.call('msdf_sampler_resample_finish' if fused else 'msdf_sampler_resample', C.byref(a), st)
+                if rounds == 0 and not fused:
                     prepare_finish()
                 rounds += 1
                 if speculate > 0:
@@ -303,11 +315,21 @@
         self.stats['calls'] += 1
         if speculate > 0:
             host = torch.empty(flags.shape, dtype=flags.dtype, pin_memory=True)
-            host.copy_(flags, non_blocking=True)
-            ev = torch.cuda.Event()
-            ev.record()
+            if fused and ops.USE_SIDE_STREAM:
+                side = ops._side_stream(dev)
+                side.wait_stream(torch.cuda.current_stream())
+                with torch.cuda.stream(side):
+                    host.copy_(flags, non_blocking=True)
+                    ev = torch.cuda.Event()
+                    ev.record(side)
+                flags.record_stream(side)
+            else:
+                host.copy_(flags, non_blocking=True)
+                ev = torch.cuda.Event()
+                ev.record()
             self._pending = (ev, host, rounds, which)
         else:
             self._note_rounds(rounds, which)
-        _lib.call('msdf_sampler_finish', C.byref(a), st)
+        if not fused:
+            _lib.call('msdf_sampler_finish', C.byref(a), st)
         return z_out, z_eik, x_all
diff --git a/monosdf_amd/ops.py b/monosdf_amd/ops.py
--- a/monosdf_amd/ops.py
+++ b/monosdf_amd/ops.py
@@ -88,7 +88,7 @@
         self.maps_dev = torch.from_numpy(mlp_plan.maps_np).to(device)
         self._wgrad_cache = {}
 
-    def pack(self, flat_w, flat_b):
+    def _pack_buffers(self, flat_w, flat_b):
         mp = self.mp
         flat_w = _need_cuda(flat_w.detach(), 'weights')
         flat_b = _need_cuda(flat_b.detach(), 'biases')
@@ -96,9 +96,15 @@
         units16 = mp.wpack_f4 if self.precision == 'fp32' else mp.wpack16_units(_PLANES[self.precision])
         wpack = torch.empty(units16 * 4 + 4 * 17 * 64 * 4, device=self.device, dtype=torch.float32)
         bpack = torch.empty(mp.bpack_f + 64, device=self.device, dtype=torch.float32)
-        _lib.call('msdf_pack_weights', C.byref(self.plan), _lib.ptr(self.rules_dev), _lib.ptr(self.maps_dev),
-                  _lib.ptr(flat_w), _lib.ptr(flat_b), _lib.ptr(wpack), _lib.ptr(bpack), _lib.stream_ptr())
-        return wpack, bpack
+        return flat_w, flat_b, wpack, bpack
+
+    def _pack_args(self, bufs):
+        return (C.byref(self.plan), _lib.ptr(self.rules_dev), _lib.ptr(self.maps_dev)) + tuple(_lib.ptr(t) for t in bufs)
+
+    def pack(self, flat_w, flat_b):
+        bufs = self._pack_buffers(flat_w, flat_b)
+        _lib.call('msdf_pack_weights', *self._pack_args(bufs), _lib.stream_ptr())
+        return bufs[2], bufs[3]
 
     def wgrad_program(self, P_pad):
         key = P_pad
@@ -141,6 +147,12 @@
         else:
             launch()
         return grad
+
+
+def pack_weights2(mlp_a, flat_w_a, flat_b_a, mlp_b, flat_w_b, flat_b_b):
+    a, b = mlp_a._pack_buffers(flat_w_a, flat_b_a), mlp_b._pack_buffers(flat_w_b, flat_b_b)
+    _lib.call('msdf_pack_weights2', *mlp_a._pack_args(a), *mlp_b._pack_args(b), _lib.stream_ptr())
+    return (a[2], a[3]), (b[2], b[3])
 
 
 class WeightNormTables:
@@ -218,7 +230,7 @@
         return (None, None) + tuple(grads)
 
 
-def fused_weight_norm(state, layers):
+def _wn_params(layers):
     params, shapes = [], []
     for l in layers:
         params.append(l.weight_v if l.has_weight_norm else l.weight)
@@ -226,11 +238,72 @@
             params.append(l.weight_g)
         params.append(l.bias)
         shapes.append((l.out_features, l.in_features, bool(l.has_weight_norm)))
-    return FusedWeightNormFunction.apply(state, tuple(shapes), *params)
+    for p in params:
+        if not p.is_cuda:
+            raise RuntimeError('monosdf_amd: the network parameters must be GPU tensors (the HIP path has no CPU fallback)')
+    return params, tuple(shapes)
+
+
+def fused_weight_norm(state, layers):
+    params, shapes = _wn_params(layers)
+    return FusedWeightNormFunction.apply(state, shapes, *params)
+
+
+class FusedWeightNorm2Function(torch.autograd.Function):
+
+    @staticmethod
+    def forward(ctx, state, shapes_a, shapes_b, *params):
+        shapes = shapes_a + shapes_b
+        st = state.tables(shapes, params)
+        dev = params[0].device
+        flat_w = torch.empty(st.n_w, device=dev, dtype=torch.float32)
+        flat_b = torch.empty(st.total_rows, device=dev, dtype=torch.float32)
+        norms = torch.empty(st.total_rows, device=dev, dtype=torch.float32)
+        _lib.call('msdf_weightnorm_forward', _lib.ptr(st.layers_dev), _lib.ptr(st.row_layer_dev), st.total_rows,
+                  _lib.ptr(flat_w), _lib.ptr(flat_b), _lib.ptr(norms), _lib.stream_ptr())
+        ctx.state, ctx.shapes = state, shapes
+        ctx.split = (sum(r * c for r, c, _ in shapes_a), sum(r for r, _, _ in shapes_a))
+        ctx.save_for_backward(norms, *params)
+        n_w, n_b = ctx.split
+        return flat_w[:n_w], flat_b[:n_b], flat_w[n_w:], flat_b[n_b:]
+
+    @staticmethod
+    @torch.autograd.function.once_differentiable
+    def backward(ctx, g_w_a, g_b_a, g_w_b, g_b_b):
+        norms, *params = ctx.saved_tensors
+        shapes = ctx.shapes
+        st = ctx.state.tables(shapes, params)
+        dev = norms.device
+        n_w, n_b = ctx.split
+        join_side_work()
+        g_w_a, g_w_b = g_w_a.contiguous(), g_w_b.contiguous()
+        dv = torch.empty(st.n_w, device=dev, dtype=torch.float32)
+        dg = torch.empty(st.total_rows, device=dev, dtype=torch.float32)
+        _lib.call('msdf_weightnorm_backward2', _lib.ptr(st.layers_dev), _lib.ptr(st.row_layer_dev), st.total_rows,
+                  _lib.ptr(g_w_a), _lib.ptr(g_w_b), n_w, _lib.ptr(norms), _lib.ptr(dv), _lib.ptr(dg), _lib.stream_ptr())
+        grads, w_off, b_off = [], 0, 0
+        for rows, cols, has_g in shapes:
+            n = rows * cols
+            grads.append(dv[w_off:w_off + n].view(rows, cols))
+            if has_g:
+                grads.append(dg[b_off:b_off + rows].view(rows, 1))
+            grads.append(g_b_a[b_off:b_off + rows] if b_off < n_b else g_b_b[b_off - n_b:b_off - n_b + rows])
+            w_off += n
+            b_off += rows
+        return (None, None, None) + tuple(grads)
+
+
+def fused_weight_norm2(state, layers_a, layers_b):
+    params_a, shapes_a = _wn_params(layers_a)
+    params_b, shapes_b = _wn_params(layers_b)
+    return FusedWeightNorm2Function.apply(state, shapes_a, shapes_b, *params_a, *params_b)
 
 
 REUSE_SAMPLER_H = _os.environ.get('MSDF_REUSE_SAMPLER_H', '1') != '0'
 FG_REUSE_LAST = _os.environ.get('MSDF_FG_REUSE_LAST', '1') != '0'
+
+
+FOLD_PLUMBING = _os.environ.get('MSDF_FOLD_PLUMBING', '1') != '0'
 
 
 def _fg_wg_first(reuse):
@@ -285,7 +358,7 @@
 
 
 def _sdf_fwd_grad(x, aux, wpack, bpack, mlp, n_clamp, n_feat, clamp_radius, sphere_scale, save, n_split=None,
-                  aux_lm=None, aux_jac=None, reuse=None):
+                  aux_lm=None, aux_jac=None, reuse=None, nrm_twice=False):
     mp = mlp.mp
     plan = mlp.plan
     x = _need_cuda(x.detach(), 'points')
@@ -332,6 +405,11 @@
     if aux_jac is not None and aC == 2:
         jac_scale = float(aux_jac[1])
         a.dy_dx, a.aux_dx_scale = aux_jac[0].data_ptr(), jac_scale
+    ns = P if n_split is None else int(n_split)
+    nrm2 = None
+    if nrm_twice:
+        nrm2 = torch.empty(ns, 3, device=dev, dtype=torch.float32)
+        a.nrm2, a.n_nrm2 = nrm2.data_ptr(), ns
     saved = (x, ws, clamped, wpack, bpack)
     if reuse is not None:
         a.row_map, a.n_reuse = reuse.row_map.data_ptr(), reuse.n_reuse
@@ -341,9 +419,9 @@
         saved += (reuse.row_map,)
     if P > 0:
         _lib.call('msdf_sdf_fwd_grad', C.byref(plan), C.byref(a), _lib.stream_ptr())
-    ns = P if n_split is None else int(n_split)
     state = _SdfState(mlp, P, P_pad, n_feat, ns, save, has_aux, (int(aC), int(aLC)), aux_shape, jac_scale)
-    return (sdf[:ns], sdf[ns:], feat, nrm[:ns], nrm[ns:], r_aux), saved, state
+    outs = (sdf[:ns], sdf[ns:], feat, nrm[:ns], nrm[ns:], r_aux)
+    return (outs + (nrm2,) if nrm_twice else outs), saved, state
 
 
 def _sdf_backward(state, saved, grads, dy_dx=None, gg_out=None, after_sweeps=None):
@@ -354,7 +432,7 @@
     mp = mlp.mp
     dev = x.device
     woff, _ = planlib.sdf_workspace(mp, P_pad)
-    g_sdf, g_sdf_b, g_feat, g_nrm, g_nrm_b, g_raux = [_cont(g) for g in grads]
+    g_sdf, g_sdf_b, g_feat, g_nrm, g_nrm_b, g_raux, *g_nrm2 = [_cont(g) for g in grads]
     g_aux = torch.empty(*state.aux_shape, device=dev, dtype=torch.float32) if state.has_aux else None
     b = _lib.BwArgs()
     b.aux_C, b.aux_LC = state.aux_lm
@@ -367,6 +445,7 @@
     b.g_raux = _addr(g_raux) if state.has_aux else None
     b.clamped = clamped.data_ptr()
     b.row_map = row_map[0].data_ptr() if row_map else None
+    b.g_nrm2 = _addr(g_nrm2[0]) if g_nrm2 else None
     base = ws.data_ptr()
     for k in ('H', 'PM', 'QB', 'AB', 'GSDF', 'QLAST'):
         setattr(b, k, base + 4 * woff[k])
@@ -384,10 +463,10 @@
 
     @staticmethod
     def forward(ctx, x, aux, flat_w, flat_b, wpack, bpack, mlp, n_clamp, n_feat, clamp_radius,
-                sphere_scale, save, n_split=None, reuse=None):
+                sphere_scale, save, n_split=None, reuse=None, nrm_twice=False):
         ctx.set_materialize_grads(False)
         outs, saved, ctx.state = _sdf_fwd_grad(x, aux, wpack, bpack, mlp, n_clamp, n_feat, clamp_radius,
-                                               sphere_scale, save, n_split, reuse=reuse)
+                                               sphere_scale, save, n_split, reuse=reuse, nrm_twice=nrm_twice)
         ctx.save_for_backward(*saved)
         return outs
 
@@ -396,7 +475,7 @@
     def backward(ctx, *grads):
         g_aux, grad = _sdf_backward(ctx.state, ctx.saved_tensors, grads)
         n_w = ctx.state.mlp.mp.n_w
-        return (None, g_aux, grad[:n_w], grad[n_w:]) + (None,) * 10
+        return (None, g_aux, grad[:n_w], grad[n_w:]) + (None,) * 11
 
 
 def _encode_points(x, divide_factor, embeddings, offsets, enc, pitch, level_major, jacobian):
@@ -572,6 +651,16 @@
         if ctx.feat_cols < g_feat.shape[1]:
             g_feat = g_feat[:, :ctx.feat_cols]
         return (None, None, g_nrm, g_feat, g_code, grad[:mp.n_w], grad[mp.n_w:], None, None, None, None, None)
+
+
+_BETA_TICKETS = {}
+
+
+def _beta_ticket(device):
+    key = torch.device(device).index if torch.device(device).index is not None else torch.cuda.current_device()
+    if key not in _BETA_TICKETS:
+        _BETA_TICKETS[key] = torch.zeros(1, device=device, dtype=torch.int32)
+    return _BETA_TICKETS[key]
 
 
 class CompositeFunction(torch.autograd.Function):
@@ -651,11 +740,15 @@
             g_beta_part.data_ptr()
         b.pose, b.pose_stride = (pose.data_ptr() if ctx.has_pose else None), ctx.pose_stride
         b.depth_scale_stride = ctx.ds_stride
+        g_raw = torch.empty(1, device=dev) if ctx.beta_shape is not None else None
+        in_launch = g_raw is not None and FOLD_PLUMBING and N > 0
+        if in_launch:
+            b.beta_raw, b.g_beta_raw, b.ticket = raw.data_ptr(), g_raw.data_ptr(), _beta_ticket(dev).data_ptr()
         _lib.call('msdf_composite_backward', C.byref(b), _lib.stream_ptr())
         sh = ctx.in_shapes
         if ctx.beta_shape is not None:
-            g_raw = torch.empty(1, device=dev)
-            _lib.call('msdf_beta_grad', _lib.ptr(raw), _lib.ptr(g_beta_part), N, _lib.ptr(g_raw), _lib.stream_ptr())
+            if not in_launch:
+                _lib.call('msdf_beta_grad', _lib.ptr(raw), _lib.ptr(g_beta_part), N, _lib.ptr(g_raw), _lib.stream_ptr())
             return (None, g_sdf.reshape(sh[0]), g_rgb.reshape(sh[1]), g_nrm.reshape(sh[2]), None, None, None, None, None,
                     g_raw.reshape(ctx.beta_shape), None)
         g_beta = g_beta_part[:N].sum().reshape(beta.shape)
```
